# oscka/rag-llm-k8s

Measured on AMD Instinct MI355X. Metric: end-to-end RAG query p50 latency + gen tokens/sec, Llama-3.1-8B top-k=4, higher is better.
Workload: dtype bf16; 1 GPU; model=Llama-3.1-8B-Instruct, embedder=all-MiniLM-L6-v2, index=FlatL2 10000 vectors (HBM-resident; 10000 embedded chunks), retrieve_k=4, context_k=4, global_batch=32, seq_len=5192, parallelism=dp1

## Files before the change

csrc/kernels/gemm_w4.hip:

```cpp
#include <stdlib.h>

#include <utility>

#include "common.h"
using namespace ragk;

namespace {

constexpr int WBM = 256, WBN = 256, WBK = 64;
constexpr int W4_THREADS = 256;
constexpr int W_TILE_A = WBM * WBK * 2;
constexpr int W_TILE_B = WBN * WBK * 2;
constexpr int W_BUF = W_TILE_A + W_TILE_B;
constexpr int W4_LDS = 2 * W_BUF;
constexpr int WGROUP_M = 8;
constexpr int W4_MIN_KT = 3;

__device__ __forceinline__ int wswz(int row, int chunk) { return chunk ^ ((row >> 1) & 7); }

template <typename F, int... Ms>
__device__ __forceinline__ void static_for_impl(F&& f, std::integer_sequence<int, Ms...>) {
  (f(std::integral_constant<int, Ms>{}), ...);
}
template <int N, typename F>
__device__ __forceinline__ void static_for(F&& f) {
  static_for_impl(f, std::make_integer_sequence<int, N>{});
}

__device__ __forceinline__ int w4_perm(int q) {
  const int j = q >> 4, fh = (q >> 2) & 3, k = q & 3;
  return 32 * (j >> 1) + 8 * fh + 4 * (j & 1) + k;
}

template <bool PERM>
__device__ __forceinline__ void w4_offsets(int ld, int row0, int rows_valid, int wid, int lane, int (&off)[8]) {
#pragma unroll
  for (int i = 0; i < 8; ++i) {
    const int r = (wid * 8 + i) * 8 + (lane >> 3);
    const int c = wswz(r, lane & 7);
    int gr = row0 + (PERM ? (r & ~127) + w4_perm(r & 127) : r);
    gr = gr < rows_valid ? gr : rows_valid - 1;
    off[i] = gr * ld * 2 + c * 16;
  }
}

__device__ __forceinline__ void w4_stage(i32x4 srd, const int (&off)[8], int k0, char* lds, int wid) {
#pragma unroll
  for (int i = 0; i < 8; ++i) blds16(srd, off[i], k0 * 2, lds + (wid * 8 + i) * 1024);
}

__device__ __forceinline__ void w4_barrier() {
  __builtin_amdgcn_sched_barrier(0);
  __builtin_amdgcn_s_barrier();
  __builtin_amdgcn_sched_barrier(0);
}

__device__ __forceinline__ void w4_read(const char* buf, int s, int wr, int wc, int fr, int fh, bf16x8 (&a)[8],
                                        bf16x8 (&b)[8]) {
  const char* sa = buf;
  const char* sb = buf + W_TILE_A;
  const int c = 4 * s + fh;
#pragma unroll
  for (int i = 0; i < 8; ++i) {
    const int R = wr * 128 + 16 * i + fr;
    a[i] = *reinterpret_cast<const bf16x8*>(sa + R * 128 + 16 * wswz(R, c));
  }
#pragma unroll
  for (int j = 0; j < 8; ++j) {
    const int R = wc * 128 + 16 * j + fr;
    b[j] = *reinterpret_cast<const bf16x8*>(sb + R * 128 + 16 * wswz(R, c));
  }
}

__device__ __forceinline__ void w4_mfma(f32x4 (&acc)[8][8], const bf16x8 (&a)[8], const bf16x8 (&b)[8], int m) {
  asm volatile("v_mfma_f32_16x16x32_bf16 %0, %2, %1, %0"
               : "+a"(acc[m >> 3][m & 7])
               : "v"(a[m >> 3]), "v"(b[m & 7])
               : "memory");
}
__device__ __forceinline__ void w4_mfma0(f32x4 (&acc)[8][8], const bf16x8 (&a)[8], const bf16x8 (&b)[8], int m) {
  asm volatile("v_mfma_f32_16x16x32_bf16 %0, %2, %1, 0"
               : "=a"(acc[m >> 3][m & 7])
               : "v"(a[m >> 3]), "v"(b[m & 7])
               : "memory");
}

__device__ __forceinline__ void w4_pin_acc(f32x4 (&acc)[8][8]) {
  asm volatile("s_nop 7\n\ts_nop 7\n\ts_nop 1" ::: "memory");
#pragma unroll
  for (int i = 0; i < 8; ++i)
#pragma unroll
    for (int j = 0; j < 8; ++j) asm volatile("" : "+a"(acc[i][j])::"memory");
}

constexpr bool epi_res(int e) { return e == EPI_RESID || e == EPI_BIAS_RESID; }
constexpr bool epi_bias(int e) {
  return e == EPI_BIAS || e == EPI_BIAS_RESID || e == EPI_BIAS_GELU || e == EPI_BIAS_GELU_TANH;
}

template <int EPI, bool OUT_F32>
constexpr int w4_epi_vmem() {
  if constexpr (EPI == EPI_ROPE_KV) return 63;
  if constexpr (EPI == EPI_SILU_MUL) return 16;
  if constexpr (OUT_F32) return 64 + (epi_res(EPI) ? 64 : 0) + (epi_bias(EPI) ? 8 : 0);
  return 32 + (epi_res(EPI) ? 32 : 0) + (epi_bias(EPI) ? 4 : 0);
}

template <int EPI>
__device__ __forceinline__ float w4_act(float v) {
  if constexpr (EPI == EPI_BIAS_GELU || EPI == EPI_GELU) return gelu_erf(v);
  if constexpr (EPI == EPI_BIAS_GELU_TANH) return gelu_tanh(v);
  return v;
}

__device__ __forceinline__ void unpack4(uint2 v, float (&f)[4]) {
  f[0] = __uint_as_float(v.x << 16);
  f[1] = __uint_as_float(v.x & 0xffff0000u);
  f[2] = __uint_as_float(v.y << 16);
  f[3] = __uint_as_float(v.y & 0xffff0000u);
}

template <int EPI>
__device__ __forceinline__ void w4_epilogue_full_bf16(const f32x4 (&acc)[8][8], int wr, int wc, int fr, int fh,
                                                      int m0, int n0, void* C, int ldc,
                                                      const bf16_t* __restrict__ bias, const bf16_t* resid, int ldr) {
  const int row0 = m0 + wr * 128 + fr;
  bf16_t* Cb = reinterpret_cast<bf16_t*>(C);
  if constexpr (EPI == EPI_SILU_MUL) {
    const int colw = (n0 >> 1) + wc * 64 + 8 * fh;
#pragma unroll
    for (int i = 0; i < 8; ++i) {
#pragma unroll
      for (int p = 0; p < 2; ++p) {
        float o[8];
#pragma unroll
        for (int k = 0; k < 4; ++k) {
          o[k] = silu(acc[i][2 * p][k]) * acc[i][2 * p + 4][k];
          o[4 + k] = silu(acc[i][2 * p + 1][k]) * acc[i][2 * p + 5][k];
        }
        *reinterpret_cast<u32x4*>(Cb + (size_t)(row0 + 16 * i) * ldc + colw + 32 * p) = pack8(o);
        __builtin_amdgcn_sched_barrier(0);
      }
    }
  } else {
    constexpr bool RES = epi_res(EPI), BIAS = epi_bias(EPI);
    const int colw = n0 + wc * 128 + 8 * fh;
    u32x4 bv[BIAS ? 4 : 1];
    if constexpr (BIAS) {
#pragma unroll
      for (int p = 0; p < 4; ++p) bv[p] = *reinterpret_cast<const u32x4*>(bias + colw + 32 * p);
    }
    u32x4 rv[RES ? 32 : 1];
    if constexpr (RES) {
#pragma unroll
      for (int i = 0; i < 8; ++i)
#pragma unroll
        for (int p = 0; p < 4; ++p)
          rv[4 * i + p] = *reinterpret_cast<const u32x4*>(resid + (size_t)(row0 + 16 * i) * ldr + colw + 32 * p);
    }
#pragma unroll
    for (int i = 0; i < 8; ++i) {
#pragma unroll
      for (int p = 0; p < 4; ++p) {
        float o[8];
#pragma unroll
        for (int k = 0; k < 4; ++k) {
          o[k] = acc[i][2 * p][k];
          o[4 + k] = acc[i][2 * p + 1][k];
        }
        if constexpr (BIAS) {
          float b[8];
          unpack8(bv[p], b);
#pragma unroll
          for (int k = 0; k < 8; ++k) o[k] += b[k];
        }
        if constexpr (RES) {
          float r[8];
          unpack8(rv[4 * i + p], r);
#pragma unroll
          for (int k = 0; k < 8; ++k) o[k] += r[k];
        }
#pragma unroll
        for (int k = 0; k < 8; ++k) o[k] = w4_act<EPI>(o[k]);
        *reinterpret_cast<u32x4*>(Cb + (size_t)(row0 + 16 * i) * ldc + colw + 32 * p) = pack8(o);
      }
    }
  }
}

struct RopeKV {
  const int* pos;
  const int* slot;
  const float* cos_t;
  const float* sin_t;
  bf16_t* kc;
  bf16_t* vc;
  int Hq, Hkv, BS;
};

template <bool FULL>
__device__ __forceinline__ void w4_epilogue_rope(const f32x4 (&acc)[8][8], int wr, int wc, int fr, int fh, int m0,
                                                 int n0, bf16_t* C, int ldc, const RopeKV& rk, int M) {
  const int row0 = m0 + wr * 128 + fr;
  const int hd = (n0 + wc * 128) >> 7;
  const int d0 = 8 * fh;
  const bool isq = hd < rk.Hq, isk = !isq && hd < rk.Hq + rk.Hkv, rot = hd < rk.Hq + rk.Hkv;
  const int kvh = isk ? hd - rk.Hq : hd - rk.Hq - rk.Hkv;
  bf16_t* cache = isk ? rk.kc : rk.vc;
  int pos[8], slot[8];
#pragma unroll
  for (int i = 0; i < 8; ++i) {
    const int r = FULL ? row0 + 16 * i : min(row0 + 16 * i, M - 1);
    pos[i] = rk.pos[r];
    slot[i] = rk.slot[r];
  }
#pragma unroll
  for (int i2 = 0; i2 < 8; i2 += 2) {
    u32x4 cv[2][2][2], sv[2][2][2];
#pragma unroll
    for (int u = 0; u < 2; ++u)
#pragma unroll
      for (int p = 0; p < 2; ++p) {
        const float* ct = rk.cos_t + (size_t)pos[i2 + u] * 64 + d0 + 32 * p;
        const float* st = rk.sin_t + (size_t)pos[i2 + u] * 64 + d0 + 32 * p;
        cv[u][p][0] = *reinterpret_cast<const u32x4*>(ct);
        cv[u][p][1] = *reinterpret_cast<const u32x4*>(ct + 4);
        sv[u][p][0] = *reinterpret_cast<const u32x4*>(st);
        sv[u][p][1] = *reinterpret_cast<const u32x4*>(st + 4);
      }
#pragma unroll
    for (int u = 0; u < 2; ++u) {
      const int i = i2 + u;
      const int gr = row0 + 16 * i;
      float o[4][8];
#pragma unroll
      for (int p = 0; p < 4; ++p)
#pragma unroll
        for (int k = 0; k < 4; ++k) {
          o[p][k] = bf2f(f2bf(acc[i][2 * p][k]));
          o[p][4 + k] = bf2f(f2bf(acc[i][2 * p + 1][k]));
        }
      if (rot) {
#pragma unroll
        for (int p = 0; p < 2; ++p)
#pragma unroll
          for (int k = 0; k < 8; ++k) {
            const float c = __uint_as_float(cv[u][p][k >> 2][k & 3]), sn = __uint_as_float(sv[u][p][k >> 2][k & 3]);
            const float x1 = o[p][k], x2 = o[p + 2][k];
            o[p][k] = bf2f(f2bf(bf2f(f2bf(x1 * c)) + bf2f(f2bf(-x2 * sn))));
            o[p + 2][k] = bf2f(f2bf(bf2f(f2bf(x2 * c)) + bf2f(f2bf(x1 * sn))));
          }
      }
      if (FULL || gr < M) {
        bf16_t* crow = C + (size_t)gr * ldc + n0 + wc * 128 + d0;
#pragma unroll
        for (int p = 0; p < 4; ++p) *reinterpret_cast<u32x4*>(crow + 32 * p) = pack8(o[p]);
        const int sl = slot[i];
        if (!isq && sl >= 0) {
          bf16_t* dst = cache + (((size_t)(sl / rk.BS) * rk.Hkv + kvh) * rk.BS + (sl % rk.BS)) * 128 + d0;
#pragma unroll
          for (int p = 0; p < 4; ++p) *reinterpret_cast<u32x4*>(dst + 32 * p) = pack8(o[p]);
        }
      }
    }
  }
}

template <int EPI, bool OUT_F32, bool FULL>
__device__ __forceinline__ void w4_epilogue_reg(const f32x4 (&acc)[8][8], int wr, int wc, int fr, int fh, int m0,
                                                int n0, void* C, int ldc, const bf16_t* __restrict__ bias,
                                                const bf16_t* resid, int ldr, int M, int Nout) {
  const int row0 = m0 + wr * 128 + fr;
  if constexpr (EPI == EPI_SILU_MUL) {
    const int colw = (n0 >> 1) + wc * 64;
#pragma unroll
    for (int i = 0; i < 8; ++i) {
      const int gr = row0 + 16 * i;
#pragma unroll
      for (int j = 0; j < 4; ++j) {
        const int gc = colw + w4_perm(16 * j + 4 * fh);
        if (FULL || (gr < M && gc < Nout)) {
          float o[4];
#pragma unroll
          for (int k = 0; k < 4; ++k) o[k] = silu(acc[i][j][k]) * acc[i][j + 4][k];
          *reinterpret_cast<uint2*>(reinterpret_cast<bf16_t*>(C) + (size_t)gr * ldc + gc) =
              make_uint2(pk2bf(o[0], o[1]), pk2bf(o[2], o[3]));
        }
      }
    }
  } else {
    constexpr bool RES = epi_res(EPI), BIAS = epi_bias(EPI);
    const int colw = n0 + wc * 128;
    uint2 bv[BIAS ? 8 : 1];
    if constexpr (BIAS) {
#pragma unroll
      for (int j = 0; j < 8; ++j) {
        const int gc = colw + w4_perm(16 * j + 4 * fh);
        bv[j] = *reinterpret_cast<const uint2*>(bias + (FULL ? gc : min(gc, Nout - 4)));
      }
    }
    constexpr int RD = BIAS ? 1 : 8;
    uint2 rv[RES ? 8 * RD : 1];
#pragma unroll
    for (int i = 0; i < 8; ++i) {
      const int gr = row0 + 16 * i;
      if constexpr (RES) {
        if (i % RD == 0) {
#pragma unroll
          for (int g = 0; g < RD; ++g)
#pragma unroll
            for (int j = 0; j < 8; ++j) {
              const int grc = FULL ? gr + 16 * g : min(gr + 16 * g, M - 1);
              const int gc = colw + w4_perm(16 * j + 4 * fh);
              rv[8 * g + j] = *reinterpret_cast<const uint2*>(resid + (size_t)grc * ldr + (FULL ? gc : min(gc, Nout - 4)));
            }
        }
      }
#pragma unroll
      for (int j = 0; j < 8; ++j) {
        const int gc = colw + w4_perm(16 * j + 4 * fh);
        if (FULL || (gr < M && gc < Nout)) {
          float o[4];
#pragma unroll
          for (int k = 0; k < 4; ++k) o[k] = acc[i][j][k];
          if constexpr (BIAS) {
            float b[4];
            unpack4(bv[j], b);
#pragma unroll
            for (int k = 0; k < 4; ++k) o[k] += b[k];
          }
          if constexpr (RES) {
            float r[4];
            unpack4(rv[8 * (i % RD) + j], r);
#pragma unroll
            for (int k = 0; k < 4; ++k) o[k] += r[k];
          }
#pragma unroll
          for (int k = 0; k < 4; ++k) o[k] = w4_act<EPI>(o[k]);
          if constexpr (OUT_F32) {
            *reinterpret_cast<f32x4*>(reinterpret_cast<float*>(C) + (size_t)gr * ldc + gc) =
                (f32x4){o[0], o[1], o[2], o[3]};
          } else {
            *reinterpret_cast<uint2*>(reinterpret_cast<bf16_t*>(C) + (size_t)gr * ldc + gc) =
                make_uint2(pk2bf(o[0], o[1]), pk2bf(o[2], o[3]));
          }
        }
      }
    }
  }
}

__device__ __forceinline__ void h_read(bf16x8& d, unsigned addr, int off_imm) {
  asm volatile("ds_read_b128 %0, %1 offset:%2" : "=v"(d) : "v"(addr), "i"(off_imm) : "memory");
}
__device__ __forceinline__ void h_dma(i32x4 srd, int voff, int soff) {
  asm volatile("buffer_load_dwordx4 %0, %1, %2 offen lds" ::"v"(voff), "s"(srd), "s"(soff) : "memory");
}
__device__ __forceinline__ void h_m0_set(unsigned lds) { asm volatile("s_mov_b32 m0, %0" ::"s"(lds) : "memory"); }
__device__ __forceinline__ void h_m0_inc() { asm volatile("s_add_u32 m0, m0, 0x400" ::: "memory"); }

constexpr int H_DX[8] = {22, 25, 28, 31, 34, 52, 55, 58};
constexpr int H_DY[8] = {61, 64, 85, 87, 89, 96, 99, 125};
constexpr int H_RB1[8] = {0, 2, 4, 6, 8, 10, 12, 14};
constexpr int H_RA1[8] = {24, 27, 30, 33, 36, 38, 40, 42};
constexpr int H_RB0[8] = {93, 94, 95, 97, 98, 100, 101, 102};
constexpr int H_RA0[8] = {104, 107, 110, 113, 116, 119, 121, 123};
constexpr int H_VM = 13;

constexpr int h_find(const int (&s)[8], int m) {
  for (int q = 0; q < 8; ++q)
    if (s[q] == m) return q;
  return -1;
}

template <bool ZERO, int VMW, bool F0 = true>
__device__ __forceinline__ void w4_iter_h(char* smem, int g, i32x4 srd_a, i32x4 srd_b, const int (&sa)[8],
                                          const int (&sb)[8], int kst, int wid, const unsigned (&rbA)[2],
                                          const unsigned (&rbB)[2], f32x4 (&acc)[8][8], bf16x8 (&a0)[8],
                                          bf16x8 (&b0)[8], bf16x8 (&a1)[8], bf16x8 (&b1)[8]) {
  static_assert(VMW >= H_VM && VMW <= 63, "vmcnt bound");
  const unsigned cur = (unsigned)(g & 1) * W_BUF, nxt = (unsigned)((g + 1) & 1) * W_BUF;
  const unsigned lds_cur = (unsigned)(unsigned long long)(const __attribute__((address_space(3))) char*)smem + cur;
  const unsigned mX = __builtin_amdgcn_readfirstlane(lds_cur + W_TILE_A + wid * 8192);
  const unsigned mY = __builtin_amdgcn_readfirstlane(lds_cur + wid * 8192);
  const int kb = kst * WBK * 2;
  const unsigned rb1 = rbB[1] + cur, ra1 = rbA[1] + cur, rb0 = rbB[0] + nxt, ra0 = rbA[0] + nxt;
  static_for<128>([&](auto mc) __attribute__((always_inline)) {
    constexpr int m = decltype(mc)::value;
    if constexpr (m == 0) asm volatile("s_waitcnt lgkmcnt(7)" ::: "memory");
    if constexpr (m == 8) asm volatile("s_waitcnt lgkmcnt(10)" ::: "memory");
    if constexpr (m == 16) asm volatile("s_waitcnt lgkmcnt(13)" ::: "memory");
    if constexpr (m == 21 || m == 51) asm volatile("s_waitcnt lgkmcnt(0)" ::: "memory");
    if constexpr (m == 22 || m == 52) w4_barrier();
    if constexpr (m == 92) asm volatile("s_waitcnt vmcnt(%0)" ::"i"(VMW) : "memory");
    if constexpr (m == 93) w4_barrier();
    if constexpr (m < 64) {
      if constexpr (ZERO) w4_mfma0(acc, a0, b0, m);
      else w4_mfma(acc, a0, b0, m);
    } else {
      w4_mfma(acc, a1, b1, m - 64);
    }
    if constexpr (h_find(H_DX, m - 1) >= 0 || h_find(H_DY, m - 1) >= 0) h_m0_inc();
    if constexpr (m == 21) h_m0_set(mX);
    if constexpr (m == 59) h_m0_set(mY);
    constexpr int qx = h_find(H_DX, m), qy = h_find(H_DY, m);
    if constexpr (qx >= 0) h_dma(srd_b, sb[qx], kb);
    if constexpr (qy >= 0) h_dma(srd_a, sa[qy], kb);
    constexpr int r1b = h_find(H_RB1, m), r1a = h_find(H_RA1, m), r0b = h_find(H_RB0, m), r0a = h_find(H_RA0, m);
    if constexpr (r1b >= 0) h_read(b1[r1b], rb1, r1b * 2048);
    if constexpr (r1a >= 0) h_read(a1[r1a], ra1, r1a * 2048);
    if constexpr (F0 && r0b >= 0) h_read(b0[r0b], rb0, r0b * 2048);
    if constexpr (F0 && r0a >= 0) h_read(a0[r0a], ra0, r0a * 2048);
  });
}

__device__ __forceinline__ void w4_read_f0(int g, const unsigned (&rbA)[2], const unsigned (&rbB)[2],
                                           bf16x8 (&a0)[8], bf16x8 (&b0)[8]) {
  const unsigned buf = (unsigned)(g & 1) * W_BUF;
  const unsigned rb0 = rbB[0] + buf, ra0 = rbA[0] + buf;
  static_for<8>([&](auto jc) __attribute__((always_inline)) {
    constexpr int j = decltype(jc)::value;
    h_read(b0[j], rb0, j * 2048);
  });
  static_for<8>([&](auto ic) __attribute__((always_inline)) {
    constexpr int i = decltype(ic)::value;
    h_read(a0[i], ra0, i * 2048);
  });
}

template <bool MT = false>
__device__ __forceinline__ void w4_origin(int tile, int nwg, int tiles_m, int tiles_n, int& m0, int& n0,
                                          const int* __restrict__ mt = nullptr, int mt_max = 0) {
  const int logical = xcd_remap(tile, nwg);
  const int group = logical / (WGROUP_M * tiles_n);
  const int first_m = group * WGROUP_M;
  const int gm = min(tiles_m - first_m, WGROUP_M);
  const int in_group = logical % (WGROUP_M * tiles_n);
  int mi = first_m + in_group % gm;
  if constexpr (MT) mi = (int)min((unsigned)mt[__builtin_amdgcn_readfirstlane(mi)], (unsigned)mt_max);
  m0 = mi * WBM;
  n0 = (in_group / gm) * WBN;
}

template <int EPI, bool OUT_F32, bool KSPLIT = false, bool MT = false>
__global__ __launch_bounds__(W4_THREADS, 1) void gemm_w4_kernel(const bf16_t* __restrict__ A, int lda,
                                                                const bf16_t* __restrict__ B, int ldb, void* C,
                                                                int ldc, const bf16_t* __restrict__ bias,
                                                                const bf16_t* resid, int ldr, int M, int N, int K,
                                                                int nsplit, RopeKV rk,
                                                                const int* __restrict__ m_tiles, int n_m_tiles) {
  __shared__ __attribute__((aligned(16))) char smem[W4_LDS];
  const int tid = threadIdx.x, lane = tid & 63;
  const int wid = __builtin_amdgcn_readfirstlane(tid >> 6);
  const int wr = wid >> 1, wc = wid & 1;
  const int fr = lane & 15, fh = lane >> 4;
  const int tiles_m = MT ? n_m_tiles : (M + WBM - 1) / WBM, tiles_n = (N + WBN - 1) / WBN;
  const int mt_max = (M + WBM - 1) / WBM - 1;
  const int nwg = tiles_m * tiles_n;
  const int nwt = KSPLIT ? nwg * nsplit : nwg;
  const int nk = K / WBK;
  const int Nout = EPI == EPI_SILU_MUL ? N / 2 : N;
  const i32x4 srd_a = make_srd(A, (unsigned)M * (unsigned)lda * 2u);
  const i32x4 srd_b = make_srd(B, (unsigned)N * (unsigned)ldb * 2u);

  constexpr int EV = w4_epi_vmem<EPI, OUT_F32>();
  constexpr int VMH0 = H_VM + EV > 63 ? 63 : H_VM + EV;
  constexpr bool LATE_F0 = !(EPI == EPI_NONE || EPI == EPI_SILU_MUL || (EPI == EPI_RESID && !OUT_F32));
  static_assert(EPI != EPI_ROPE_KV || (!OUT_F32 && !KSPLIT), "rope epilogue: bf16 output, no split-K");
  static_assert(!MT || EPI == EPI_NONE || ((EPI == EPI_RESID || EPI == EPI_SILU_MUL) && !OUT_F32 && !KSPLIT),
                "M-tile list: none / residual / SiLU*up epilogues and the split-K slabs");

  int tile = blockIdx.x;
  int z = KSPLIT ? tile / nwg : 0;
  int m0, n0;
  w4_origin<MT>(tile - z * nwg, nwg, tiles_m, tiles_n, m0, n0, m_tiles, mt_max);
  int off_a[8], off_b[8];
  w4_offsets<false>(lda, m0, M, wid, lane, off_a);
  w4_offsets<true>(ldb, n0, N, wid, lane, off_b);
  if constexpr (KSPLIT) {
#pragma unroll
    for (int i = 0; i < 8; ++i) {
      off_a[i] += z * K * 2;
      off_b[i] += z * K * 2;
    }
  }
  w4_stage(srd_a, off_a, 0, smem, wid);
  w4_stage(srd_b, off_b, 0, smem + W_TILE_A, wid);
  w4_stage(srd_a, off_a, WBK, smem + W_BUF, wid);
  w4_stage(srd_b, off_b, WBK, smem + W_BUF + W_TILE_A, wid);
  __builtin_amdgcn_s_waitcnt(0x0F70);
  w4_barrier();
  bf16x8 a0[8], b0[8], a1[8], b1[8];
  w4_read(smem, 0, wr, wc, fr, fh, a0, b0);
  __builtin_amdgcn_s_waitcnt(0xC07F);
  __builtin_amdgcn_sched_barrier(0);

  unsigned rbA[2], rbB[2];
  {
    const unsigned l0 = (unsigned)(unsigned long long)(const __attribute__((address_space(3))) char*)smem;
#pragma unroll
    for (int s = 0; s < 2; ++s) {
      const unsigned cs = (unsigned)(((4 * s + fh) ^ ((fr >> 1) & 7)) * 16);
      rbA[s] = l0 + (unsigned)((wr * 128 + fr) * 128) + cs;
      rbB[s] = l0 + W_TILE_A + (unsigned)((wc * 128 + fr) * 128) + cs;
    }
  }

  f32x4 acc[8][8];
  int g = 0;
  for (;;) {
    const int next = tile + (int)gridDim.x;
    const bool has_next = next < nwt;
    w4_iter_h<true, VMH0>(smem, g, srd_a, srd_b, off_a, off_b, 2, wid, rbA, rbB, acc, a0, b0, a1, b1);
    ++g;
    for (int t = 1; t + 2 < nk; ++t, ++g)
      w4_iter_h<false, H_VM>(smem, g, srd_a, srd_b, off_a, off_b, t + 2, wid, rbA, rbB, acc, a0, b0, a1, b1);
    int nm0, nn0;
    const int ntile = has_next ? next : tile;
    const int nz = KSPLIT ? ntile / nwg : 0;
    w4_origin<MT>(ntile - nz * nwg, nwg, tiles_m, tiles_n, nm0, nn0, m_tiles, mt_max);
    {
      int ln;
      asm volatile("v_mbcnt_lo_u32_b32 %0, -1, 0\n\tv_mbcnt_hi_u32_b32 %0, -1, %0" : "=v"(ln));
      w4_offsets<false>(lda, nm0, M, wid, ln, off_a);
      w4_offsets<true>(ldb, nn0, N, wid, ln, off_b);
      if constexpr (KSPLIT) {
#pragma unroll
        for (int i = 0; i < 8; ++i) {
          off_a[i] += nz * K * 2;
          off_b[i] += nz * K * 2;
        }
      }
    }
    w4_iter_h<false, H_VM>(smem, g, srd_a, srd_b, off_a, off_b, 0, wid, rbA, rbB, acc, a0, b0, a1, b1);
    ++g;
    w4_iter_h<false, H_VM, !LATE_F0>(smem, g, srd_a, srd_b, off_a, off_b, 1, wid, rbA, rbB, acc, a0, b0, a1, b1);
    ++g;
    asm volatile("s_waitcnt lgkmcnt(0)" ::: "memory");
    w4_pin_acc(acc);
    void* Cz = KSPLIT ? (void*)(reinterpret_cast<float*>(C) + (size_t)z * M * ldc) : C;
    if constexpr (EPI == EPI_ROPE_KV) {
      if (m0 + WBM <= M) {
        w4_epilogue_rope<true>(acc, wr, wc, fr, fh, m0, n0, reinterpret_cast<bf16_t*>(Cz), ldc, rk, M);
      } else {
        w4_epilogue_rope<false>(acc, wr, wc, fr, fh, m0, n0, reinterpret_cast<bf16_t*>(Cz), ldc, rk, M);
        __builtin_amdgcn_s_waitcnt(0x0F70);
      }
    } else if (m0 + WBM <= M && n0 + WBN <= N) {
      if constexpr (OUT_F32)
        w4_epilogue_reg<EPI, true, true>(acc, wr, wc, fr, fh, m0, n0, Cz, ldc, bias, resid, ldr, M, Nout);
      else
        w4_epilogue_full_bf16<EPI>(acc, wr, wc, fr, fh, m0, n0, Cz, ldc, bias, resid, ldr);
    } else {
      w4_epilogue_reg<EPI, OUT_F32, false>(acc, wr, wc, fr, fh, m0, n0, Cz, ldc, bias, resid, ldr, M, Nout);
      __builtin_amdgcn_s_waitcnt(0x0F70);
    }
    asm volatile("s_nop 7" ::: "memory");
    if (!has_next) {
      __builtin_amdgcn_s_waitcnt(0x0F70);
      asm volatile("s_waitcnt lgkmcnt(0)" ::: "memory");
      break;
    }
    if constexpr (LATE_F0) w4_read_f0(g, rbA, rbB, a0, b0);
    tile = next;
    m0 = nm0;
    n0 = nn0;
    z = nz;
  }
}

static int g_w4_grid = -1;
static int w4_grid(int nwg) {
  if (g_w4_grid < 0) {
    int cus = 0, dev = 0;
    if (hipGetDevice(&dev) != hipSuccess ||
        hipDeviceGetAttribute(&cus, hipDeviceAttributeMultiprocessorCount, dev) != hipSuccess)
      cus = 256;
    g_w4_grid = (cus / 8) * 8;
  }
  return (g_w4_grid == 0 || g_w4_grid >= nwg) ? nwg : g_w4_grid;
}

constexpr bool w4_mt_epi(int e) { return e == EPI_NONE || e == EPI_RESID || e == EPI_SILU_MUL; }

template <int EPI, bool F32>
int launch_w4(const void* A, int lda, const void* B, int ldb, void* C, int ldc, const void* bias, const void* resid,
              int ldr, int M, int N, int K, const int* m_tiles, int n_m_tiles, hipStream_t st) {
  const int tiles_n = (N + WBN - 1) / WBN;
  if (m_tiles) {
    if constexpr (w4_mt_epi(EPI) && !F32) {
      hipLaunchKernelGGL((gemm_w4_kernel<EPI, F32, false, true>), dim3(w4_grid(n_m_tiles * tiles_n)),
                         dim3(W4_THREADS), 0, st, (const bf16_t*)A, lda, (const bf16_t*)B, ldb, C, ldc,
                         (const bf16_t*)bias, (const bf16_t*)resid, ldr, M, N, K, 1, RopeKV{}, m_tiles, n_m_tiles);
      return (int)hipGetLastError();
    } else {
      return (int)hipErrorInvalidValue;
    }
  }
  const int nwg = ((M + WBM - 1) / WBM) * tiles_n;
  hipLaunchKernelGGL((gemm_w4_kernel<EPI, F32>), dim3(w4_grid(nwg)), dim3(W4_THREADS), 0, st, (const bf16_t*)A, lda,
                     (const bf16_t*)B, ldb, C, ldc, (const bf16_t*)bias, (const bf16_t*)resid, ldr, M, N, K, 1,
                     RopeKV{}, nullptr, 0);
  return (int)hipGetLastError();
}

static bool w4_mt_ok(const int* m_tiles, int n_m_tiles, int M) {
  return !m_tiles || (n_m_tiles >= 1 && n_m_tiles <= (M + WBM - 1) / WBM);
}

}

RAGK_API int ragk_gemm_w4_set_grid(int g) {
  g_w4_grid = g < 0 ? -1 : g;
  return 0;
}

RAGK_API int ragk_gemm_w4(const void* A, int lda, const void* B, int ldb, void* C, int ldc, const void* bias,
                          const void* resid, int ldr, int M, int N, int K, int epi, int out_f32, const int* m_tiles,
                          int n_m_tiles, hipStream_t st) {
  if (M <= 0 || N <= 0 || K <= 0 || (m_tiles && n_m_tiles == 0)) return 0;
  if (!w4_mt_ok(m_tiles, n_m_tiles, M)) return (int)hipErrorInvalidValue;
  if (K % WBK != 0 || K / WBK < W4_MIN_KT) return (int)hipErrorInvalidValue;
  const long long rows_b = (epi == EPI_SILU_MUL) ? 2LL * N : (long long)N;
  if ((long long)M * lda * 2 >= (1LL << 31) || rows_b * ldb * 2 >= (1LL << 31))
    return (int)hipErrorInvalidValue;
  if (epi == EPI_SILU_MUL) {
    if (N % 128 != 0 || out_f32) return (int)hipErrorInvalidValue;
    return launch_w4<EPI_SILU_MUL, false>(A, lda, B, ldb, C, ldc, bias, resid, ldr, M, 2 * N, K, m_tiles, n_m_tiles,
                                          st);
  }
  if (N % 8 != 0) return (int)hipErrorInvalidValue;
#define RAGK_W4_CASE(E) \
  case E:               \
    return out_f32 ? launch_w4<E, true>(A, lda, B, ldb, C, ldc, bias, resid, ldr, M, N, K, m_tiles, n_m_tiles, st) \
                   : launch_w4<E, false>(A, lda, B, ldb, C, ldc, bias, resid, ldr, M, N, K, m_tiles, n_m_tiles, st);
  switch (epi) {
    RAGK_W4_CASE(EPI_NONE)
    RAGK_W4_CASE(EPI_BIAS)
    RAGK_W4_CASE(EPI_RESID)
    RAGK_W4_CASE(EPI_BIAS_RESID)
    RAGK_W4_CASE(EPI_BIAS_GELU)
    RAGK_W4_CASE(EPI_GELU)
    RAGK_W4_CASE(EPI_BIAS_GELU_TANH)
    default:
      return (int)hipErrorInvalidValue;
  }
#undef RAGK_W4_CASE
}

RAGK_API int ragk_gemm_w4_splitk(const void* A, int lda, const void* B, int ldb, float* P, int M, int N, int K,
                                 int nsplit, const int* m_tiles, int n_m_tiles, hipStream_t st) {
  if (M <= 0 || N <= 0 || K <= 0 || (m_tiles && n_m_tiles == 0)) return 0;
  if (!w4_mt_ok(m_tiles, n_m_tiles, M)) return (int)hipErrorInvalidValue;
  if (nsplit < 1 || K % nsplit || (K / nsplit) % WBK || (K / nsplit) / WBK < W4_MIN_KT || N % 8 || !P)
    return (int)hipErrorInvalidValue;
  if ((long long)M * lda * 2 >= (1LL << 31) || (long long)N * ldb * 2 >= (1LL << 31)) return (int)hipErrorInvalidValue;
  if (m_tiles) {
    const int nwt = n_m_tiles * ((N + WBN - 1) / WBN) * nsplit;
    hipLaunchKernelGGL((gemm_w4_kernel<EPI_NONE, true, true, true>), dim3(w4_grid(nwt)), dim3(W4_THREADS), 0, st,
                       (const bf16_t*)A, lda, (const bf16_t*)B, ldb, (void*)P, N, nullptr, nullptr, 0, M, N,
                       K / nsplit, nsplit, RopeKV{}, m_tiles, n_m_tiles);
    return (int)hipGetLastError();
  }
  const int nwg = ((M + WBM - 1) / WBM) * ((N + WBN - 1) / WBN);
  hipLaunchKernelGGL((gemm_w4_kernel<EPI_NONE, true, true>), dim3(w4_grid(nwg * nsplit)), dim3(W4_THREADS), 0, st,
                     (const bf16_t*)A, lda, (const bf16_t*)B, ldb, (void*)P, N, nullptr, nullptr, 0, M, N, K / nsplit,
                     nsplit, RopeKV{}, nullptr, 0);
  return (int)hipGetLastError();
}

RAGK_API int ragk_gemm_w4_rope_kv(const void* A, int lda, const void* B, int ldb, void* C, int ldc, int M, int K,
                                  const int* pos, const int* slot, const float* cos_t, const float* sin_t, void* kc,
                                  void* vc, int Hq, int Hkv, int BS, hipStream_t st) {
  if (M <= 0) return 0;
  const int N = (Hq + 2 * Hkv) * 128;
  if (K % WBK != 0 || K / WBK < W4_MIN_KT || Hq < 1 || Hkv < 1 || BS < 1 || N % WBN != 0) return (int)hipErrorInvalidValue;
  if (!pos || !slot || !cos_t || !sin_t || !kc || !vc || ldc % 8 != 0) return (int)hipErrorInvalidValue;
  if ((long long)M * lda * 2 >= (1LL << 31) || (long long)N * ldb * 2 >= (1LL << 31)) return (int)hipErrorInvalidValue;
  const int nwg = ((M + WBM - 1) / WBM) * (N / WBN);
  const RopeKV rk{pos, slot, cos_t, sin_t, (bf16_t*)kc, (bf16_t*)vc, Hq, Hkv, BS};
  hipLaunchKernelGGL((gemm_w4_kernel<EPI_ROPE_KV, false>), dim3(w4_grid(nwg)), dim3(W4_THREADS), 0, st,
                     (const bf16_t*)A, lda, (const bf16_t*)B, ldb, C, ldc, nullptr, nullptr, 0, M, N, K, 1, rk, nullptr, 0);
  return (int)hipGetLastError();
}
```

csrc/kernels/norm.hip:

```cpp
#include <algorithm>

#include "common.h"
#include "kv_fp8.h"
using namespace ragk;

namespace {

constexpr int NT = 256;

__global__ __launch_bounds__(NT) void rmsnorm_kernel(const bf16_t* x, int ldx, bf16_t* resid, int ldr,
                                                     const bf16_t* __restrict__ w, bf16_t* out, int ldo,
                                                     int H, float eps) {
  __shared__ float red[NT / 64];
  const int row = blockIdx.x;
  const bf16_t* xr = x + (size_t)row * ldx;
  bf16_t* rr = resid ? resid + (size_t)row * ldr : nullptr;
  bf16_t* orow = out + (size_t)row * ldo;
  constexpr int MAXV = 4;
  float v[MAXV][8];
  const int nvec = H >> 3;
  float ss = 0.f;
#pragma unroll
  for (int i = 0; i < MAXV; ++i) {
    const int vi = threadIdx.x + i * NT;
    if (vi < nvec) {
      unpack8(*reinterpret_cast<const u32x4*>(xr + vi * 8), v[i]);
      if (rr) {
        float r8[8];
        unpack8(*reinterpret_cast<const u32x4*>(rr + vi * 8), r8);
#pragma unroll
        for (int e = 0; e < 8; ++e) v[i][e] = bf2f(f2bf(v[i][e] + r8[e]));
        *reinterpret_cast<u32x4*>(rr + vi * 8) = pack8(v[i]);
      }
#pragma unroll
      for (int e = 0; e < 8; ++e) ss += v[i][e] * v[i][e];
    }
  }
  ss = block_sum(ss, red);
  const float inv = rsqrtf(ss / (float)H + eps);
#pragma unroll
  for (int i = 0; i < MAXV; ++i) {
    const int vi = threadIdx.x + i * NT;
    if (vi < nvec) {
      float wv[8], o[8];
      unpack8(*reinterpret_cast<const u32x4*>(w + vi * 8), wv);
#pragma unroll
      for (int e = 0; e < 8; ++e) o[e] = wv[e] * bf2f(f2bf(v[i][e] * inv));
      *reinterpret_cast<u32x4*>(orow + vi * 8) = pack8(o);
    }
  }
}

__global__ __launch_bounds__(NT) void layernorm_kernel(const bf16_t* x, int ldx, const bf16_t* resid, int ldr,
                                                       const bf16_t* __restrict__ g, const bf16_t* __restrict__ b,
                                                       bf16_t* out, int ldo, int H, float eps) {
  __shared__ float red[NT / 64];
  const int row = blockIdx.x;
  const bf16_t* xr = x + (size_t)row * ldx;
  constexpr int MAXV = 4;
  float v[MAXV][8];
  const int nvec = H >> 3;
  float s = 0.f;
#pragma unroll
  for (int i = 0; i < MAXV; ++i) {
    const int vi = threadIdx.x + i * NT;
    if (vi < nvec) {
      unpack8(*reinterpret_cast<const u32x4*>(xr + vi * 8), v[i]);
      if (resid) {
        float r8[8];
        unpack8(*reinterpret_cast<const u32x4*>(resid + (size_t)row * ldr + vi * 8), r8);
#pragma unroll
        for (int e = 0; e < 8; ++e) v[i][e] += r8[e];
      }
#pragma unroll
      for (int e = 0; e < 8; ++e) s += v[i][e];
    }
  }
  const float mean = block_sum(s, red) / (float)H;
  float sq = 0.f;
#pragma unroll
  for (int i = 0; i < MAXV; ++i) {
    const int vi = threadIdx.x + i * NT;
    if (vi < nvec)
#pragma unroll
      for (int e = 0; e < 8; ++e) {
        const float d = v[i][e] - mean;
        sq += d * d;
      }
  }
  const float inv = rsqrtf(block_sum(sq, red) / (float)H + eps);
#pragma unroll
  for (int i = 0; i < MAXV; ++i) {
    const int vi = threadIdx.x + i * NT;
    if (vi < nvec) {
      float gv[8], bv[8], o[8];
      unpack8(*reinterpret_cast<const u32x4*>(g + vi * 8), gv);
      unpack8(*reinterpret_cast<const u32x4*>(b + vi * 8), bv);
#pragma unroll
      for (int e = 0; e < 8; ++e) o[e] = (v[i][e] - mean) * inv * gv[e] + bv[e];
      *reinterpret_cast<u32x4*>(out + (size_t)row * ldo + vi * 8) = pack8(o);
    }
  }
}

__global__ __launch_bounds__(NT) void embed_kernel(int* __restrict__ ids, const bf16_t* __restrict__ table,
                                                   bf16_t* out, int H, int vocab, const int* __restrict__ carry,
                                                   const int* __restrict__ prev) {
  const int t = blockIdx.x;
  int id = ids[t];
  if (carry != nullptr) {
    const int c = carry[t];
    if (c >= 0) {
      id = prev[c];
      __syncthreads();
      if (threadIdx.x == 0) ids[t] = id;
    }
  }
  id = id < 0 ? 0 : (id >= vocab ? vocab - 1 : id);
  const u32x4* src = reinterpret_cast<const u32x4*>(table + (size_t)id * H);
  u32x4* dst = reinterpret_cast<u32x4*>(out + (size_t)t * H);
  for (int i = threadIdx.x; i < (H >> 3); i += NT) dst[i] = src[i];
}

__global__ __launch_bounds__(NT) void embed_ln_kernel(const int* __restrict__ ids, const int* __restrict__ pos_ids,
                                                      const bf16_t* __restrict__ word, const bf16_t* __restrict__ pos,
                                                      const bf16_t* __restrict__ type, const bf16_t* __restrict__ g,
                                                      const bf16_t* __restrict__ b, bf16_t* out, int H, float eps,
                                                      int do_ln) {
  __shared__ float red[NT / 64];
  const int t = blockIdx.x;
  const bf16_t* wr = word + (size_t)ids[t] * H;
  const bf16_t* pr = pos + (size_t)pos_ids[t] * H;
  constexpr int MAXV = 4;
  float v[MAXV][8];
  const int nvec = H >> 3;
  float s = 0.f;
#pragma unroll
  for (int i = 0; i < MAXV; ++i) {
    const int vi = threadIdx.x + i * NT;
    if (vi < nvec) {
      float a[8], p[8];
      unpack8(*reinterpret_cast<const u32x4*>(wr + vi * 8), a);
      unpack8(*reinterpret_cast<const u32x4*>(pr + vi * 8), p);
#pragma unroll
      for (int e = 0; e < 8; ++e) v[i][e] = a[e] + p[e];
      if (type) {
        float ty[8];
        unpack8(*reinterpret_cast<const u32x4*>(type + vi * 8), ty);
#pragma unroll
        for (int e = 0; e < 8; ++e) v[i][e] += ty[e];
      }
#pragma unroll
      for (int e = 0; e < 8; ++e) s += v[i][e];
    }
  }
  if (!do_ln) {
#pragma unroll
    for (int i = 0; i < MAXV; ++i) {
      const int vi = threadIdx.x + i * NT;
      if (vi < nvec) *reinterpret_cast<u32x4*>(out + (size_t)t * H + vi * 8) = pack8(v[i]);
    }
    return;
  }
  const float mean = block_sum(s, red) / (float)H;
  float sq = 0.f;
#pragma unroll
  for (int i = 0; i < MAXV; ++i) {
    const int vi = threadIdx.x + i * NT;
    if (vi < nvec)
#pragma unroll
      for (int e = 0; e < 8; ++e) {
        const float d = v[i][e] - mean;
        sq += d * d;
      }
  }
  const float inv = rsqrtf(block_sum(sq, red) / (float)H + eps);
#pragma unroll
  for (int i = 0; i < MAXV; ++i) {
    const int vi = threadIdx.x + i * NT;
    if (vi < nvec) {
      float gv[8], bv[8], o[8];
      unpack8(*reinterpret_cast<const u32x4*>(g + vi * 8), gv);
      unpack8(*reinterpret_cast<const u32x4*>(b + vi * 8), bv);
#pragma unroll
      for (int e = 0; e < 8; ++e) o[e] = (v[i][e] - mean) * inv * gv[e] + bv[e];
      *reinterpret_cast<u32x4*>(out + (size_t)t * H + vi * 8) = pack8(o);
    }
  }
}

__global__ __launch_bounds__(NT) void rope_kv_kernel(bf16_t* qkv, int ld, const int* __restrict__ positions,
                                                     const float* __restrict__ cos_t, const float* __restrict__ sin_t,
                                                     const int* __restrict__ slots, bf16_t* kc, bf16_t* vc, int Hq,
                                                     int Hkv, int D, int BS, int apply_rope) {
  const int t = blockIdx.x;
  const int pos = positions[t];
  const int slot = slots ? slots[t] : -1;
  bf16_t* row = qkv + (size_t)t * ld;
  const int half = D >> 1;
  const int vpr = half >> 3;
  const float* ct = cos_t + (size_t)pos * half;
  const float* st = sin_t + (size_t)pos * half;
  const int nrot = (Hq + Hkv) * vpr;
  for (int i = threadIdx.x; i < nrot; i += NT) {
    const int h = i / vpr, v = i % vpr;
    bf16_t* hp = row + h * D;
    float x1[8], x2[8], o1[8], o2[8];
    unpack8(*reinterpret_cast<const u32x4*>(hp + v * 8), x1);
    unpack8(*reinterpret_cast<const u32x4*>(hp + half + v * 8), x2);
    if (apply_rope) {
#pragma unroll
      for (int e = 0; e < 8; ++e) {
        const float c = ct[v * 8 + e], s = st[v * 8 + e];
        o1[e] = bf2f(f2bf(bf2f(f2bf(x1[e] * c)) + bf2f(f2bf(-x2[e] * s))));
        o2[e] = bf2f(f2bf(bf2f(f2bf(x2[e] * c)) + bf2f(f2bf(x1[e] * s))));
      }
    } else {
#pragma unroll
      for (int e = 0; e < 8; ++e) { o1[e] = x1[e]; o2[e] = x2[e]; }
    }
    const u32x4 p1 = pack8(o1), p2 = pack8(o2);
    if (h < Hq) {
      *reinterpret_cast<u32x4*>(hp + v * 8) = p1;
      *reinterpret_cast<u32x4*>(hp + half + v * 8) = p2;
    } else if (slot >= 0) {
      const int kh = h - Hq;
      bf16_t* dst = kc + (((size_t)(slot / BS) * Hkv + kh) * BS + (slot % BS)) * D;
      *reinterpret_cast<u32x4*>(dst + v * 8) = p1;
      *reinterpret_cast<u32x4*>(dst + half + v * 8) = p2;
      *reinterpret_cast<u32x4*>(hp + v * 8) = p1;
      *reinterpret_cast<u32x4*>(hp + half + v * 8) = p2;
    } else {
      *reinterpret_cast<u32x4*>(hp + v * 8) = p1;
      *reinterpret_cast<u32x4*>(hp + half + v * 8) = p2;
    }
  }
  if (slot >= 0) {
    const int vpd = D >> 3;
    for (int i = threadIdx.x; i < Hkv * vpd; i += NT) {
      const int kh = i / vpd, v = i % vpd;
      const bf16_t* src = row + (Hq + Hkv + kh) * D + v * 8;
      bf16_t* dst = vc + (((size_t)(slot / BS) * Hkv + kh) * BS + (slot % BS)) * D + v * 8;
      *reinterpret_cast<u32x4*>(dst) = *reinterpret_cast<const u32x4*>(src);
    }
  }
}

__global__ __launch_bounds__(NT) void pool_l2norm_kernel(const bf16_t* __restrict__ hidden, int ld,
                                                         const int* __restrict__ cu, float* out, int H, int mode,
                                                         int normalize) {
  __shared__ float red[NT / 64];
  const int b = blockIdx.x;
  const int s0 = cu[b], s1 = cu[b + 1];
  const int len = s1 - s0;
  float ss = 0.f;
  constexpr int MAXC = 8;
  float acc[MAXC];
#pragma unroll
  for (int k = 0; k < MAXC; ++k) acc[k] = 0.f;
  if (mode == 1) {
    for (int t = s0; t < s1; ++t)
#pragma unroll
      for (int k = 0; k < MAXC; ++k) {
        const int c = threadIdx.x + k * NT;
        if (c < H) acc[k] += bf2f(hidden[(size_t)t * ld + c]);
      }
    const float inv = len > 0 ? 1.f / (float)len : 0.f;
#pragma unroll
    for (int k = 0; k < MAXC; ++k) acc[k] *= inv;
  } else {
    const int t = mode == 0 ? s0 : s1 - 1;
#pragma unroll
    for (int k = 0; k < MAXC; ++k) {
      const int c = threadIdx.x + k * NT;
      if (c < H) acc[k] = bf2f(hidden[(size_t)t * ld + c]);
    }
  }
#pragma unroll
  for (int k = 0; k < MAXC; ++k) ss += acc[k] * acc[k];
  float scale = 1.f;
  if (normalize) {
    ss = block_sum(ss, red);
    scale = 1.f / fmaxf(sqrtf(ss), 1e-12f);
  }
#pragma unroll
  for (int k = 0; k < MAXC; ++k) {
    const int c = threadIdx.x + k * NT;
    if (c < H) out[(size_t)b * H + c] = acc[k] * scale;
  }
}

__global__ __launch_bounds__(NT) void silu_mul_kernel(const bf16_t* x, int ldx, bf16_t* out, int ldo, int I) {
  const int t = blockIdx.x;
  for (int v = threadIdx.x; v < (I >> 3); v += NT) {
    float g[8], u[8], o[8];
    unpack8(*reinterpret_cast<const u32x4*>(x + (size_t)t * ldx + v * 8), g);
    unpack8(*reinterpret_cast<const u32x4*>(x + (size_t)t * ldx + I + v * 8), u);
#pragma unroll
    for (int e = 0; e < 8; ++e) o[e] = silu(g[e]) * u[e];
    *reinterpret_cast<u32x4*>(out + (size_t)t * ldo + v * 8) = pack8(o);
  }
}

__global__ __launch_bounds__(NT) void gather_rows_kernel(const bf16_t* x, int ldx, const int* __restrict__ idx,
                                                         bf16_t* out, int ldo, int H) {
  const int i = blockIdx.x;
  const bf16_t* src = x + (size_t)idx[i] * ldx;
  for (int v = threadIdx.x; v < (H >> 3); v += NT)
    *reinterpret_cast<u32x4*>(out + (size_t)i * ldo + v * 8) = *reinterpret_cast<const u32x4*>(src + v * 8);
}



constexpr int PNT = 512;
__global__ __launch_bounds__(PNT) void add_partials_rmsnorm_kernel(const float* __restrict__ P, int S, int M,
                                                                   bf16_t* h, int ldh,
                                                                   const bf16_t* __restrict__ w, bf16_t* out,
                                                                   int ldo, int H, float eps) {
  __shared__ float red[PNT / 64];
  const int row = blockIdx.x;
  bf16_t* hr = h + (size_t)row * ldh;
  constexpr int MAXV = 2;
  float v[MAXV][8];
  const int nvec = H >> 3;
  float ss = 0.f;
  f32x4 pv[MAXV][PSU][2];
  u32x4 hv[MAXV], gv[MAXV];
#pragma unroll
  for (int i = 0; i < MAXV; ++i) {
    const int vi = min((int)threadIdx.x + i * PNT, nvec - 1);
    if (i * PNT < nvec) {
      load_slabs8(P + (size_t)row * H + vi * 8, S, (size_t)M * H, pv[i]);
      hv[i] = *reinterpret_cast<const u32x4*>(hr + vi * 8);
      gv[i] = *reinterpret_cast<const u32x4*>(w + vi * 8);
    }
  }
#pragma unroll
  for (int i = 0; i < MAXV; ++i) {
    const int vi = threadIdx.x + i * PNT;
    if (vi < nvec) {
      float a[8];
      add_slabs8(pv[i], P + (size_t)row * H + vi * 8, S, (size_t)M * H, a);
      unpack8(hv[i], v[i]);
#pragma unroll
      for (int e = 0; e < 8; ++e) v[i][e] = bf2f(f2bf(v[i][e] + bf2f(f2bf(a[e]))));
      *reinterpret_cast<u32x4*>(hr + vi * 8) = pack8(v[i]);
#pragma unroll
      for (int e = 0; e < 8; ++e) ss += v[i][e] * v[i][e];
    }
  }
  ss = block_sum(ss, red);
  const float inv = rsqrtf(ss / (float)H + eps);
#pragma unroll
  for (int i = 0; i < MAXV; ++i) {
    const int vi = threadIdx.x + i * PNT;
    if (vi < nvec) {
      float wv[8], o[8];
      unpack8(gv[i], wv);
#pragma unroll
      for (int e = 0; e < 8; ++e) o[e] = wv[e] * bf2f(f2bf(v[i][e] * inv));
      *reinterpret_cast<u32x4*>(out + (size_t)row * ldo + vi * 8) = pack8(o);
    }
  }
}


__global__ __launch_bounds__(NT) void rope_kv_partials_kernel(const float* __restrict__ P, int S, int T, int ldp,
                                                              bf16_t* q_out, int ldq,
                                                              const int* __restrict__ positions,
                                                              const float* __restrict__ cos_t,
                                                              const float* __restrict__ sin_t,
                                                              const int* __restrict__ slots, bf16_t* kc, bf16_t* vc,
                                                              int Hq, int Hkv, int D, int BS) {
  const int t = blockIdx.x, hg = blockIdx.y, ngroups = gridDim.y;
  const int pos = positions[t];
  const int slot = slots ? slots[t] : -1;
  const size_t slab = (size_t)T * ldp;
  const float* prow = P + (size_t)t * ldp;
  const int half = D >> 1;
  const int vpr = half >> 3;
  const float* ct = cos_t + (size_t)pos * half;
  const float* st = sin_t + (size_t)pos * half;
  const int nh = Hq + 2 * Hkv;
  for (int i = threadIdx.x + hg * NT; i < nh * vpr; i += NT * ngroups) {
    const int hd = i / vpr, v = i % vpr;
    float x1[8], x2[8];
    sum_partials8(prow + hd * D + v * 8, S, slab, x1);
    sum_partials8(prow + hd * D + half + v * 8, S, slab, x2);
    if (hd >= Hq + Hkv) {
      if (slot >= 0) {
        bf16_t* dst = vc + (((size_t)(slot / BS) * Hkv + (hd - Hq - Hkv)) * BS + (slot % BS)) * D;
        *reinterpret_cast<u32x4*>(dst + v * 8) = pack8(x1);
        *reinterpret_cast<u32x4*>(dst + half + v * 8) = pack8(x2);
      }
      continue;
    }
    float o1[8], o2[8];
    rope8(x1, x2, ct + v * 8, st + v * 8, o1, o2);
    if (hd < Hq) {
      bf16_t* qp = q_out + (size_t)t * ldq + hd * D;
      *reinterpret_cast<u32x4*>(qp + v * 8) = pack8(o1);
      *reinterpret_cast<u32x4*>(qp + half + v * 8) = pack8(o2);
    } else if (slot >= 0) {
      bf16_t* dst = kc + (((size_t)(slot / BS) * Hkv + (hd - Hq)) * BS + (slot % BS)) * D;
      *reinterpret_cast<u32x4*>(dst + v * 8) = pack8(o1);
      *reinterpret_cast<u32x4*>(dst + half + v * 8) = pack8(o2);
    }
  }
}

__device__ __forceinline__ size_t kv8_row(int slot, int kh, int Hkv, int BS) {
  return ((size_t)(slot / BS) * Hkv + kh) * BS + (slot % BS);
}

__global__ __launch_bounds__(NT) void rope_kv_fp8_kernel(bf16_t* qkv, int ld, const int* __restrict__ positions,
                                                         const float* __restrict__ cos_t,
                                                         const float* __restrict__ sin_t,
                                                         const int* __restrict__ slots, unsigned char* k8,
                                                         unsigned char* v8, float* ks, float* vs, int Hq, int Hkv,
                                                         int BS) {
  constexpr int D = 128, half = 64, vpr = 8;
  const int t = blockIdx.x;
  const int pos = positions[t];
  const int slot = slots ? slots[t] : -1;
  bf16_t* row = qkv + (size_t)t * ld;
  const float* ct = cos_t + (size_t)pos * half;
  const float* st = sin_t + (size_t)pos * half;
  const int nh = Hq + 2 * Hkv;
  for (int i = threadIdx.x; i < nh * vpr; i += NT) {
    const int h = i / vpr, v = i % vpr;
    bf16_t* hp = row + h * D;
    float x1[8], x2[8], o1[8], o2[8];
    unpack8(*reinterpret_cast<const u32x4*>(hp + v * 8), x1);
    unpack8(*reinterpret_cast<const u32x4*>(hp + half + v * 8), x2);
    if (h >= Hq + Hkv) {
      if (slot >= 0) {
        const size_t r = kv8_row(slot, h - Hq - Hkv, Hkv, BS);
        kv8_store_row128(x1, x2, v, v8 + r * D, vs + r);
      }
      continue;
    }
    rope8(x1, x2, ct + v * 8, st + v * 8, o1, o2);
    *reinterpret_cast<u32x4*>(hp + v * 8) = pack8(o1);
    *reinterpret_cast<u32x4*>(hp + half + v * 8) = pack8(o2);
    if (h >= Hq && slot >= 0) {
      const size_t r = kv8_row(slot, h - Hq, Hkv, BS);
      kv8_store_row128(o1, o2, v, k8 + r * D, ks + r);
    }
  }
}

__global__ __launch_bounds__(NT) void rope_kv_partials_fp8_kernel(const float* __restrict__ P, int S, int T, int ldp,
                                                                  bf16_t* q_out, int ldq,
                                                                  const int* __restrict__ positions,
                                                                  const float* __restrict__ cos_t,
                                                                  const float* __restrict__ sin_t,
                                                                  const int* __restrict__ slots, unsigned char* k8,
                                                                  unsigned char* v8, float* ks, float* vs, int Hq,
                                                                  int Hkv, int BS) {
  constexpr int D = 128, half = 64, vpr = 8;
  const int t = blockIdx.x, hg = blockIdx.y, ngroups = gridDim.y;
  const int pos = positions[t];
  const int slot = slots[t];
  const size_t slab = (size_t)T * ldp;
  const float* prow = P + (size_t)t * ldp;
  const float* ct = cos_t + (size_t)pos * half;
  const float* st = sin_t + (size_t)pos * half;
  const int nh = Hq + 2 * Hkv;
  for (int i = threadIdx.x + hg * NT; i < nh * vpr; i += NT * ngroups) {
    const int hd = i / vpr, v = i % vpr;
    float x1[8], x2[8];
    sum_partials8(prow + hd * D + v * 8, S, slab, x1);
    sum_partials8(prow + hd * D + half + v * 8, S, slab, x2);
    if (hd >= Hq + Hkv) {
      if (slot >= 0) {
        const size_t r = kv8_row(slot, hd - Hq - Hkv, Hkv, BS);
        kv8_store_row128(x1, x2, v, v8 + r * D, vs + r);
      }
      continue;
    }
    float o1[8], o2[8];
    rope8(x1, x2, ct + v * 8, st + v * 8, o1, o2);
    if (hd < Hq) {
      bf16_t* qp = q_out + (size_t)t * ldq + hd * D;
      *reinterpret_cast<u32x4*>(qp + v * 8) = pack8(o1);
      *reinterpret_cast<u32x4*>(qp + half + v * 8) = pack8(o2);
    } else if (slot >= 0) {
      const size_t r = kv8_row(slot, hd - Hq, Hkv, BS);
      kv8_store_row128(o1, o2, v, k8 + r * D, ks + r);
    }
  }
}

}

RAGK_API int ragk_rmsnorm(const void* x, int ldx, void* resid, int ldr, const void* w, void* out, int ldo, int rows,
                          int H, float eps, hipStream_t st) {
  if (rows <= 0) return 0;
  if (H % 8 || H > 8 * NT * 4) return (int)hipErrorInvalidValue;
  hipLaunchKernelGGL(rmsnorm_kernel, dim3(rows), dim3(NT), 0, st, (const bf16_t*)x, ldx, (bf16_t*)resid, ldr,
                     (const bf16_t*)w, (bf16_t*)out, ldo, H, eps);
  return (int)hipGetLastError();
}

RAGK_API int ragk_layernorm(const void* x, int ldx, const void* resid, int ldr, const void* g, const void* b,
                            void* out, int ldo, int rows, int H, float eps, hipStream_t st) {
  if (rows <= 0) return 0;
  if (H % 8 || H > 8 * NT * 4) return (int)hipErrorInvalidValue;
  hipLaunchKernelGGL(layernorm_kernel, dim3(rows), dim3(NT), 0, st, (const bf16_t*)x, ldx, (const bf16_t*)resid,
                     ldr, (const bf16_t*)g, (const bf16_t*)b, (bf16_t*)out, ldo, H, eps);
  return (int)hipGetLastError();
}

RAGK_API int ragk_embed(const int* ids, const void* table, void* out, int T, int H, int vocab, hipStream_t st) {
  if (T <= 0) return 0;
  if (H % 8) return (int)hipErrorInvalidValue;
  hipLaunchKernelGGL(embed_kernel, dim3(T), dim3(NT), 0, st, const_cast<int*>(ids), (const bf16_t*)table,
                     (bf16_t*)out, H, vocab, (const int*)nullptr, (const int*)nullptr);
  return (int)hipGetLastError();
}

RAGK_API int ragk_embed_carry(int* ids, const int* carry, const int* prev, const void* table, void* out, int T,
                              int H, int vocab, hipStream_t st) {
  if (T <= 0) return 0;
  if (H % 8 || !carry || !prev) return (int)hipErrorInvalidValue;
  hipLaunchKernelGGL(embed_kernel, dim3(T), dim3(NT), 0, st, ids, (const bf16_t*)table, (bf16_t*)out, H, vocab,
                     carry, prev);
  return (int)hipGetLastError();
}

RAGK_API int ragk_embed_ln(const int* ids, const int* pos_ids, const void* word, const void* pos, const void* type,
                           const void* g, const void* b, void* out, int T, int H, float eps, int do_ln,
                           hipStream_t st) {
  if (T <= 0) return 0;
  if (H % 8 || H > 8 * NT * 4) return (int)hipErrorInvalidValue;
  hipLaunchKernelGGL(embed_ln_kernel, dim3(T), dim3(NT), 0, st, ids, pos_ids, (const bf16_t*)word,
                     (const bf16_t*)pos, (const bf16_t*)type, (const bf16_t*)g, (const bf16_t*)b, (bf16_t*)out, H,
                     eps, do_ln);
  return (int)hipGetLastError();
}

RAGK_API int ragk_rope_kv(void* qkv, int ld, const int* positions, const float* cos_t, const float* sin_t,
                          const int* slots, void* kc, void* vc, int T, int Hq, int Hkv, int D, int BS,
                          int apply_rope, hipStream_t st) {
  if (T <= 0) return 0;
  if (D % 16) return (int)hipErrorInvalidValue;
  hipLaunchKernelGGL(rope_kv_kernel, dim3(T), dim3(NT), 0, st, (bf16_t*)qkv, ld, positions, cos_t, sin_t, slots,
                     (bf16_t*)kc, (bf16_t*)vc, Hq, Hkv, D, BS, apply_rope);
  return (int)hipGetLastError();
}

RAGK_API int ragk_pool_l2norm(const void* hidden, int ld, const int* cu, float* out, int B, int H, int mode,
                              int normalize, hipStream_t st) {
  if (B <= 0) return 0;
  if (H > 8 * NT) return (int)hipErrorInvalidValue;
  hipLaunchKernelGGL(pool_l2norm_kernel, dim3(B), dim3(NT), 0, st, (const bf16_t*)hidden, ld, cu, out, H, mode,
                     normalize);
  return (int)hipGetLastError();
}

RAGK_API int ragk_silu_mul(const void* x, int ldx, void* out, int ldo, int T, int I, hipStream_t st) {
  if (T <= 0) return 0;
  if (I % 8) return (int)hipErrorInvalidValue;
  hipLaunchKernelGGL(silu_mul_kernel, dim3(T), dim3(NT), 0, st, (const bf16_t*)x, ldx, (bf16_t*)out, ldo, I);
  return (int)hipGetLastError();
}

RAGK_API int ragk_gather_rows(const void* x, int ldx, const int* idx, void* out, int ldo, int n, int H,
                              hipStream_t st) {
  if (n <= 0) return 0;
  if (H % 8) return (int)hipErrorInvalidValue;
  hipLaunchKernelGGL(gather_rows_kernel, dim3(n), dim3(NT), 0, st, (const bf16_t*)x, ldx, idx, (bf16_t*)out, ldo, H);
  return (int)hipGetLastError();
}

RAGK_API int ragk_add_partials_rmsnorm(const float* P, int S, int M, void* h, int ldh, const void* w, void* out,
                                       int ldo, int H, float eps, hipStream_t st) {
  if (M <= 0) return 0;
  if (H % 8 || H > 8 * PNT * 2 || S < 1) return (int)hipErrorInvalidValue;
  hipLaunchKernelGGL(add_partials_rmsnorm_kernel, dim3(M), dim3(PNT), 0, st, P, S, M, (bf16_t*)h, ldh,
                     (const bf16_t*)w, (bf16_t*)out, ldo, H, eps);
  return (int)hipGetLastError();
}

RAGK_API int ragk_rope_kv_partials(const float* P, int S, int T, int ldp, void* q_out, int ldq,
                                   const int* positions, const float* cos_t, const float* sin_t, const int* slots,
                                   void* kc, void* vc, int Hq, int Hkv, int D, int BS, hipStream_t st) {
  if (T <= 0) return 0;
  if (D % 16 || S < 1) return (int)hipErrorInvalidValue;
  const int items = (Hq + 2 * Hkv) * (D / 16);
  const int groups = std::max(1, std::min((items + 63) / 64, std::max(4, (512 + T - 1) / T)));
  hipLaunchKernelGGL(rope_kv_partials_kernel, dim3(T, groups), dim3(NT), 0, st, P, S, T, ldp, (bf16_t*)q_out,
                     ldq, positions, cos_t, sin_t, slots, (bf16_t*)kc, (bf16_t*)vc, Hq, Hkv, D, BS);
  return (int)hipGetLastError();
}

RAGK_API int ragk_rope_kv_fp8(void* qkv, int ld, const int* positions, const float* cos_t, const float* sin_t,
                              const int* slots, void* k8, void* v8, float* ks, float* vs, int T, int Hq, int Hkv,
                              int D, int BS, hipStream_t st) {
  if (T <= 0) return 0;
  if (D != 128 || !positions || !cos_t || !sin_t || (slots && (!k8 || !v8 || !ks || !vs)))
    return (int)hipErrorInvalidValue;
  hipLaunchKernelGGL(rope_kv_fp8_kernel, dim3(T), dim3(NT), 0, st, (bf16_t*)qkv, ld, positions, cos_t, sin_t, slots,
                     (unsigned char*)k8, (unsigned char*)v8, ks, vs, Hq, Hkv, BS);
  return (int)hipGetLastError();
}

RAGK_API int ragk_rope_kv_partials_fp8(const float* P, int S, int T, int ldp, void* q_out, int ldq,
                                       const int* positions, const float* cos_t, const float* sin_t,
                                       const int* slots, void* k8, void* v8, float* ks, float* vs, int Hq, int Hkv,
                                       int D, int BS, hipStream_t st) {
  if (T <= 0) return 0;
  if (D != 128 || S < 1 || !positions || !cos_t || !sin_t || !slots || !k8 || !v8 || !ks || !vs)
    return (int)hipErrorInvalidValue;
  const int items = (Hq + 2 * Hkv) * (D / 16);
  const int groups = std::max(1, std::min((items + 63) / 64, std::max(4, (512 + T - 1) / T)));
  hipLaunchKernelGGL(rope_kv_partials_fp8_kernel, dim3(T, groups), dim3(NT), 0, st, P, S, T, ldp, (bf16_t*)q_out,
                     ldq, positions, cos_t, sin_t, slots, (unsigned char*)k8, (unsigned char*)v8, ks, vs, Hq, Hkv,
                     BS);
  return (int)hipGetLastError();
}
```

rag_llm_k8s_amd/models/llama.py:

```python
from __future__ import annotations

import json
import math
import os
from dataclasses import dataclass, field
from typing import List, Optional

import torch

from ..ops.backend import AttnMeta, get_backend
from ..ops.fp8 import FP8, alloc_fp8_kv, check_fp8_kv_head_dim, kv_cache_torch_dtype
from ..ops.reference import pack_gate_up, rope_tables

DECODE_DOWN_SKINNY_MAX_M = 4
DECODE_OPROJ_MERGE_MAX_M = 2


@dataclass
class LlamaConfig:
    vocab_size: int = 128256
    hidden_size: int = 4096
    intermediate_size: int = 14336
    num_hidden_layers: int = 32
    num_attention_heads: int = 32
    num_key_value_heads: int = 8
    head_dim: int = 128
    rms_norm_eps: float = 1e-5
    rope_theta: float = 500000.0
    rope_scaling: Optional[dict] = field(default_factory=lambda: {
        "rope_type": "llama3", "factor": 8.0, "low_freq_factor": 1.0, "high_freq_factor": 4.0,
        "original_max_position_embeddings": 8192})
    max_position_embeddings: int = 131072
    tie_word_embeddings: bool = False
    bos_token_id: int = 128000
    eos_token_id: List[int] = field(default_factory=lambda: [128001, 128008, 128009])
    model_type: str = "llama"

    @classmethod
    def from_dict(cls, d):
        c = cls()
        for k in ("vocab_size", "hidden_size", "intermediate_size", "num_hidden_layers", "num_attention_heads",
                  "rms_norm_eps", "rope_theta", "max_position_embeddings", "tie_word_embeddings", "bos_token_id",
                  "model_type"):
            if k in d and d[k] is not None:
                setattr(c, k, d[k])
        c.num_key_value_heads = d.get("num_key_value_heads") or c.num_attention_heads
        c.head_dim = d.get("head_dim") or c.hidden_size // c.num_attention_heads
        c.rope_scaling = d.get("rope_scaling")
        eos = d.get("eos_token_id")
        if eos is not None:
            c.eos_token_id = eos if isinstance(eos, list) else [eos]
        return c

    @classmethod
    def from_json(cls, path):
        with open(path) as f:
            return cls.from_dict(json.load(f))

    def to_hf_dict(self):
        return {
            "architectures": ["LlamaForCausalLM"], "model_type": "llama", "vocab_size": self.vocab_size,
            "hidden_size": self.hidden_size, "intermediate_size": self.intermediate_size,
            "num_hidden_layers": self.num_hidden_layers, "num_attention_heads": self.num_attention_heads,
            "num_key_value_heads": self.num_key_value_heads, "head_dim": self.head_dim,
            "rms_norm_eps": self.rms_norm_eps, "rope_theta": self.rope_theta, "rope_scaling": self.rope_scaling,
            "max_position_embeddings": self.max_position_embeddings,
            "tie_word_embeddings": self.tie_word_embeddings, "bos_token_id": self.bos_token_id,
            "eos_token_id": self.eos_token_id, "hidden_act": "silu", "attention_bias": False, "mlp_bias": False,
            "torch_dtype": "bfloat16",
        }


def llama31_8b():
    return LlamaConfig()


def llama31_70b():
    return LlamaConfig(hidden_size=8192, intermediate_size=28672, num_hidden_layers=80, num_attention_heads=64,
                       num_key_value_heads=8)


def llama_tiny(vocab=512, layers=2, hidden=256, heads=4, kv_heads=2, inter=512):
    return LlamaConfig(vocab_size=vocab, hidden_size=hidden, intermediate_size=inter, num_hidden_layers=layers,
                       num_attention_heads=heads, num_key_value_heads=kv_heads, head_dim=hidden // heads,
                       max_position_embeddings=4096, bos_token_id=1, eos_token_id=[2])


class LlamaWeights:

    def __init__(self, cfg: LlamaConfig, tp_rank=0, tp_size=1):
        self.cfg, self.tp_rank, self.tp_size = cfg, tp_rank, tp_size
        self.layers = []
        self.embed = self.norm = self.lm_head = None

    def geom(self):
        c, tp = self.cfg, self.tp_size
        assert c.num_attention_heads % tp == 0 and c.num_key_value_heads % tp == 0, "heads % tp"
        assert c.intermediate_size % tp == 0 and (c.intermediate_size // tp) % 64 == 0, "intermediate % (64*tp)"
        return dict(Hq=c.num_attention_heads // tp, Hkv=c.num_key_value_heads // tp, D=c.head_dim,
                    I=c.intermediate_size // tp, V=-(-c.vocab_size // tp))

    @classmethod
    def from_hf(cls, cfg, get, device, tp_rank=0, tp_size=1, dtype=torch.bfloat16):
        w = cls(cfg, tp_rank, tp_size)
        g = w.geom()
        r = tp_rank
        D, Hq, Hkv, I, Vl = g["D"], g["Hq"], g["Hkv"], g["I"], g["V"]

        def dev(t):
            return t.to(device=device, dtype=dtype, non_blocking=False).contiguous()

        w.embed = dev(get("model.embed_tokens.weight"))
        for i in range(cfg.num_hidden_layers):
            p = "model.layers.%d." % i
            q = get(p + "self_attn.q_proj.weight", rows=(r * Hq * D, (r + 1) * Hq * D))
            k = get(p + "self_attn.k_proj.weight", rows=(r * Hkv * D, (r + 1) * Hkv * D))
            v = get(p + "self_attn.v_proj.weight", rows=(r * Hkv * D, (r + 1) * Hkv * D))
            o = get(p + "self_attn.o_proj.weight", cols=(r * Hq * D, (r + 1) * Hq * D))
            gt = get(p + "mlp.gate_proj.weight", rows=(r * I, (r + 1) * I))
            up = get(p + "mlp.up_proj.weight", rows=(r * I, (r + 1) * I))
            dn = get(p + "mlp.down_proj.weight", cols=(r * I, (r + 1) * I))
            w.layers.append(dict(
                ln_in=dev(get(p + "input_layernorm.weight")), ln_post=dev(get(p + "post_attention_layernorm.weight")),
                wqkv=dev(torch.cat([q, k, v], 0)), wo=dev(o), wgu=dev(pack_gate_up(gt, up)), wdown=dev(dn)))
        w.norm = dev(get("model.norm.weight"))
        V = cfg.vocab_size
        lo, hi = r * Vl, min(V, (r + 1) * Vl)
        name = "model.embed_tokens.weight" if cfg.tie_word_embeddings else "lm_head.weight"
        lm = get(name, rows=(lo, hi))
        if lm.shape[0] < Vl:
            lm = torch.cat([lm, torch.zeros(Vl - lm.shape[0], lm.shape[1], dtype=lm.dtype, device=lm.device)], 0)
        w.lm_head = dev(lm)
        w.vocab_offset = lo
        w.vocab_valid = hi - lo
        return w

    @classmethod
    def from_checkpoint(cls, path, cfg, device, tp_rank=0, tp_size=1):
        from ..runtime.safetensors_io import CheckpointReader

        rd = CheckpointReader(path)
        try:
            return cls.from_hf(cfg, rd.get, device, tp_rank, tp_size)
        finally:
            rd.close()

    @classmethod
    def from_state_dict(cls, cfg, sd, device, tp_rank=0, tp_size=1):
        def get(name, rows=None, cols=None):
            t = sd[name]
            if rows is not None:
                t = t[rows[0]:rows[1]]
            if cols is not None:
                t = t[:, cols[0]:cols[1]]
            return t

        return cls.from_hf(cfg, get, device, tp_rank, tp_size)

    @classmethod
    def random(cls, cfg, device, tp_rank=0, tp_size=1, seed=0, dtype=torch.bfloat16):
        w = cls(cfg, tp_rank, tp_size)
        g = w.geom()
        D, Hq, Hkv, I, Vl = g["D"], g["Hq"], g["Hkv"], g["I"], g["V"]
        H = cfg.hidden_size
        gen = torch.Generator(device=device).manual_seed(seed * 1000 + tp_rank)

        def rnd(*shape, std=0.02):
            return (torch.randn(*shape, device=device, generator=gen, dtype=torch.float32) * std).to(dtype)

        def ones(n):
            return (1.0 + 0.1 * torch.randn(n, device=device, generator=gen)).to(dtype)

        w.embed = rnd(cfg.vocab_size, H)
        for _ in range(cfg.num_hidden_layers):
            w.layers.append(dict(ln_in=ones(H), ln_post=ones(H), wqkv=rnd((Hq + 2 * Hkv) * D, H),
                                 wo=rnd(H, Hq * D), wgu=rnd(2 * I, H), wdown=rnd(H, I)))
        w.norm = ones(H)
        w.lm_head = rnd(Vl, H)
        w.vocab_offset = tp_rank * Vl
        w.vocab_valid = min(cfg.vocab_size - tp_rank * Vl, Vl)
        return w

    def quantize_fp8(self, lm_head=False):
        from ..ops.fp8 import quantize_weight

        for L in self.layers:
            for k in ("wqkv", "wo", "wgu", "wdown"):
                L[k] = quantize_weight(L[k])
        if lm_head:
            self.lm_head = quantize_weight(self.lm_head)
        self.dtype = "fp8"
        return self

    def quantize_mxfp4(self, lm_head=False):
        from ..ops.mxfp4 import quantize_weight

        for L in self.layers:
            for k in ("wqkv", "wo", "wgu", "wdown"):
                L[k] = quantize_weight(L[k])
        if lm_head:
            self.lm_head = quantize_weight(self.lm_head)
        self.dtype = "mxfp4"
        return self

    def nbytes(self):
        t = [self.embed, self.norm, self.lm_head] + [v for l in self.layers for v in l.values()]
        return sum(x.nbytes() if hasattr(x, "dequant") else x.numel() * x.element_size() for x in t)


@dataclass
class StepInput:
    ids: torch.Tensor
    positions: torch.Tensor
    slots: torch.Tensor
    meta: AttnMeta
    logits_idx: Optional[torch.Tensor] = None
    m_tiles: Optional[torch.Tensor] = None
    carry: Optional[torch.Tensor] = None
    carry_src: Optional[torch.Tensor] = None


class LlamaModel:
    def __init__(self, cfg: LlamaConfig, weights: LlamaWeights, device, comm=None, max_positions=None):
        self.cfg, self.w, self.device = cfg, weights, torch.device(device)
        self.be = get_backend(self.device)
        g = weights.geom()
        self.Hq, self.Hkv, self.D, self.I, self.Vl = g["Hq"], g["Hkv"], g["D"], g["I"], g["V"]
        self.comm = comm
        self.tp_rank = weights.tp_rank
        mp = max_positions or cfg.max_position_embeddings
        cos, sin = rope_tables(self.D, mp, cfg.rope_theta, cfg.rope_scaling)
        self.cos, self.sin = cos.to(self.device), sin.to(self.device)
        self.kv_cache = None
        self.seq_parallel = os.environ.get("RAGK_SEQ_PARALLEL", "0") == "1"
        self.sp_min_tokens = int(os.environ.get("RAGK_SP_MIN_TOKENS", "256"))

    def allocate_kv_cache(self, num_blocks, dtype=torch.bfloat16):
        dtype = kv_cache_torch_dtype(dtype)
        if dtype == FP8:
            check_fp8_kv_head_dim(self.D)
            self.kv_cache = [(alloc_fp8_kv(num_blocks, self.Hkv, 64, self.D, self.device),
                              alloc_fp8_kv(num_blocks, self.Hkv, 64, self.D, self.device))
                             for _ in range(self.cfg.num_hidden_layers)]
            return self.kv_cache
        self.kv_cache = [(torch.zeros(num_blocks, self.Hkv, 64, self.D, dtype=dtype, device=self.device),
                          torch.zeros(num_blocks, self.Hkv, 64, self.D, dtype=dtype, device=self.device))
                         for _ in range(self.cfg.num_hidden_layers)]
        return self.kv_cache

    def kv_bytes_per_block(self, dtype=torch.bfloat16):
        dtype = kv_cache_torch_dtype(dtype)
        if dtype == FP8:
            return 2 * self.cfg.num_hidden_layers * self.Hkv * 64 * (self.D + 4)
        return 2 * self.cfg.num_hidden_layers * self.Hkv * 64 * self.D * torch.tensor([], dtype=dtype).element_size()

    def _allreduce(self, x):
        if self.comm is not None:
            self.comm.all_reduce(x)

    def _attn_block(self, li, L, h, inp: StepInput, attn):
        be, c = self.be, self.cfg
        Hq, Hkv, D = self.Hq, self.Hkv, self.D
        kc, vc = self.kv_cache[li]
        xn = be.rmsnorm(h, L["ln_in"], c.rms_norm_eps)
        qkv = be.gemm_rope_kv(xn, L["wqkv"], inp.positions, self.cos, self.sin, inp.slots, kc, vc, Hq, Hkv, D)
        if inp.meta.kind == "decode":
            be.attn_decode(qkv, kc, vc, inp.meta, attn, Hq, Hkv, D)
        else:
            be.attn_prefill(qkv, kc, vc, inp.meta, attn, Hq, Hkv, D)
        if self.tp_rank == 0:
            be.gemm(attn, L["wo"], resid=h, epi="resid", out=h)
        else:
            be.gemm(attn, L["wo"], out=h)

    def _mlp_block(self, L, h):
        be, c = self.be, self.cfg
        xn = be.rmsnorm(h, L["ln_post"], c.rms_norm_eps)
        a = be.gemm(xn, L["wgu"], epi="silu_mul")
        if self.tp_rank == 0:
            be.gemm(a, L["wdown"], resid=h, epi="resid", out=h)
        else:
            be.gemm(a, L["wdown"], out=h)

    def _final(self, h, inp: StepInput):
        if inp.logits_idx is not None:
            h = self.be.gather_rows(h, inp.logits_idx)
            if h.shape[0] == 0:
                return h
        return self.be.rmsnorm(h, self.w.norm, self.cfg.rms_norm_eps)

    @staticmethod
    def prefill_last_rows_enabled():
        return os.environ.get("RAGK_PREFILL_LAST_ROWS", "1") != "0"

    def _last_rows(self, inp: StepInput, M):
        if (self.comm is not None or inp.meta is None or inp.meta.kind == "decode" or inp.logits_idx is None
                or not self.prefill_last_rows_enabled()):
            return None
        if inp.logits_idx.numel() == 0:
            return "skip"
        if inp.m_tiles is None or inp.meta.tiles_last is None:
            return None
        L, be = self.w.layers[-1], self.be
        if not (be.m_tiles_ok(M, L["wo"], "resid") and be.m_tiles_ok(M, L["wgu"], "silu_mul")
                and be.m_tiles_ok(M, L["wdown"], "resid")):
            return None
        return "tiles"

    def _tp(self):
        return self.comm is not None and self.comm.size > 1

    def _decode_part_ok(self, inp: StepInput, h):
        if inp.meta is None or inp.meta.kind != "decode" or inp.slots is None:
            return False
        L, M = self.w.layers[0], h.shape[0]
        if self._tp() and not self.comm.fused_decode_ok(M, h.shape[1]):
            return False
        return self.be.part_ok(M, L["wqkv"]) and self.be.part_ok(M, L["wo"]) and self.be.part_ok(M, L["wdown"])

    def hidden_states_decode_part(self, inp: StepInput, h):
        be, w, c = self.be, self.w, self.cfg
        Hq, Hkv, D = self.Hq, self.Hkv, self.D
        M = h.shape[0]
        tp = self._tp()

        def reduce_norm(P, gamma):
            if tp:
                return self.comm.add_partials_rmsnorm(P, h, gamma, c.rms_norm_eps, be)
            return be.add_partials_rmsnorm(P, h, gamma, c.rms_norm_eps)

        attn = torch.empty((M, Hq * D), dtype=h.dtype, device=h.device)
        layers = w.layers
        fuse_norm = M <= DECODE_DOWN_SKINNY_MAX_M and not tp and be.part_norm_ok(M, layers[0]["wqkv"])
        silu_fused = tp and be.part_silu_ok(M, layers[0]["wgu"], layers[0]["wdown"])
        xn = None if fuse_norm else be.rmsnorm(h, layers[0]["ln_in"], c.rms_norm_eps)
        merge = M <= DECODE_OPROJ_MERGE_MAX_M and be.part_merge_ok(M, inp.meta, layers[0]["wo"], Hq, D)
        mlp_eng = M == 1 and not tp and be.mlp_engine_ok(M, layers[0]["wgu"], layers[0]["wdown"])
        for li, L in enumerate(layers):
            kc, vc = self.kv_cache[li]
            P = be.gemm_part_norm(h, L["ln_in"], c.rms_norm_eps, L["wqkv"]) if fuse_norm else be.gemm_part(xn, L["wqkv"])
            be.attn_decode_rope(P, inp.positions, self.cos, self.sin, inp.slots, kc, vc, inp.meta, attn, Hq, Hkv, D,
                                defer_merge=merge)
            P = be.gemm_part_merge(attn, inp.meta, L["wo"], Hq) if merge else be.gemm_part(attn, L["wo"])
            nxt = layers[li + 1]["ln_in"] if li + 1 < len(layers) else w.norm
            if mlp_eng:
                be.mlp_engine_tail(P, h, L["ln_post"], c.rms_norm_eps, L["wgu"], L["wdown"])
                if not fuse_norm or li + 1 == len(layers):
                    xn = be.rmsnorm(h, nxt, c.rms_norm_eps)
                continue
            xn = reduce_norm(P, L["ln_post"])
            if silu_fused:
                P = be.gemm_part_silu(be.gemm_part_gu(xn, L["wgu"]), L["wdown"])
                xn = reduce_norm(P, nxt)
                continue
            a = be.gemm(xn, L["wgu"], epi="silu_mul")
            if M <= DECODE_DOWN_SKINNY_MAX_M and not tp:
                be.gemm(a, L["wdown"], resid=h, epi="resid", out=h)
                if not fuse_norm or li + 1 == len(layers):
                    xn = be.rmsnorm(h, nxt, c.rms_norm_eps)
                continue
            P = be.gemm_part(a, L["wdown"])
            xn = reduce_norm(P, nxt)
        if inp.logits_idx is not None:
            xn = be.gather_rows(xn, inp.logits_idx)
        return xn

    def hidden_states(self, inp: StepInput):
        be, w = self.be, self.w
        h = be.embed(inp.ids, w.embed, carry=inp.carry, prev=inp.carry_src)
        if self._decode_part_ok(inp, h):
            return self.hidden_states_decode_part(inp, h)
        attn = torch.empty((h.shape[0], self.Hq * self.D), dtype=h.dtype, device=h.device)
        if self.comm is None and inp.meta is not None and inp.meta.kind != "decode":
            L0 = w.layers[0]
            ns = (be.prefill_nsplit(h.shape[0], L0["wo"]), be.prefill_nsplit(h.shape[0], L0["wdown"]))
            if max(ns) > 1:
                return self.hidden_states_splitk(inp, h, attn, *ns)
        last = self._last_rows(inp, h.shape[0])
        for li, L in enumerate(w.layers):
            if last is not None and li + 1 == len(w.layers):
                self._last_layer_rows(li, L, h, inp, attn, last)
                break
            self._attn_block(li, L, h, inp, attn)
            self._allreduce(h)
            self._mlp_block(L, h)
            self._allreduce(h)
        return self._final(h, inp)

    def _last_layer_rows(self, li, L, h, inp: StepInput, attn, mode):
        be, c = self.be, self.cfg
        Hq, Hkv, D = self.Hq, self.Hkv, self.D
        kc, vc = self.kv_cache[li]
        xn = be.rmsnorm(h, L["ln_in"], c.rms_norm_eps)
        qkv = be.gemm_rope_kv(xn, L["wqkv"], inp.positions, self.cos, self.sin, inp.slots, kc, vc, Hq, Hkv, D)
        if mode == "skip":
            return
        mt = inp.m_tiles
        be.attn_prefill(qkv, kc, vc, inp.meta, attn, Hq, Hkv, D, tiles=inp.meta.tiles_last)
        be.gemm(attn, L["wo"], resid=h, epi="resid", out=h, m_tiles=mt)
        xn = be.rmsnorm(h, L["ln_post"], c.rms_norm_eps)
        a = be.gemm(xn, L["wgu"], epi="silu_mul", m_tiles=mt)
        be.gemm(a, L["wdown"], resid=h, epi="resid", out=h, m_tiles=mt)

    def hidden_states_splitk(self, inp: StepInput, h, attn, ns_o, ns_d):
        be, w, c = self.be, self.w, self.cfg
        Hq, Hkv, D = self.Hq, self.Hkv, self.D
        layers = w.layers
        last = self._last_rows(inp, h.shape[0])
        xn = be.rmsnorm(h, layers[0]["ln_in"], c.rms_norm_eps)
        for li, L in enumerate(layers):
            kc, vc = self.kv_cache[li]
            cut = last if li + 1 == len(layers) else None
            rows = {"m_tiles": inp.m_tiles} if cut == "tiles" else {}
            blocks = {"tiles": inp.meta.tiles_last} if cut == "tiles" else {}
            qkv = be.gemm_rope_kv(xn, L["wqkv"], inp.positions, self.cos, self.sin, inp.slots, kc, vc, Hq, Hkv, D)
            if cut == "skip":
                return h.new_empty((0, h.shape[1]))
            be.attn_prefill(qkv, kc, vc, inp.meta, attn, Hq, Hkv, D, **blocks)
            if ns_o > 1:
                xn = be.add_partials_rmsnorm(be.gemm_splitk(attn, L["wo"], ns_o, **rows), h, L["ln_post"],
                                             c.rms_norm_eps)
            else:
                be.gemm(attn, L["wo"], resid=h, epi="resid", out=h, **rows)
                xn = be.rmsnorm(h, L["ln_post"], c.rms_norm_eps)
            a = be.gemm(xn, L["wgu"], epi="silu_mul", **rows)
            nxt = layers[li + 1]["ln_in"] if li + 1 < len(layers) else w.norm
            if ns_d > 1:
                xn = be.add_partials_rmsnorm(be.gemm_splitk(a, L["wdown"], ns_d, **rows), h, nxt, c.rms_norm_eps)
            else:
                be.gemm(a, L["wdown"], resid=h, epi="resid", out=h, **rows)
                xn = be.rmsnorm(h, nxt, c.rms_norm_eps)
        if inp.logits_idx is not None:
            xn = be.gather_rows(xn, inp.logits_idx)
        return xn

    def hidden_states_sp(self, inp: StepInput):
        be, w, c, comm = self.be, self.w, self.cfg, self.comm
        tp, r = comm.size, comm.rank
        Hq, Hkv, D, H = self.Hq, self.Hkv, self.D, c.hidden_size
        T = inp.ids.shape[0]
        S = -(-T // tp)
        Tp = S * tp
        ids = inp.ids
        if Tp != T:
            ids = torch.cat([ids, ids.new_zeros(Tp - T)])
        h = be.embed(ids[r * S:(r + 1) * S].contiguous(), w.embed)
        dev, dt = h.device, h.dtype
        xg = torch.empty((Tp, H), dtype=dt, device=dev)
        part = torch.zeros((Tp, H), dtype=dt, device=dev)
        attn = torch.empty((T, Hq * D), dtype=dt, device=dev)
        rs = torch.empty((S, H), dtype=dt, device=dev)
        for li, L in enumerate(w.layers):
            kc, vc = self.kv_cache[li]
            comm.all_gather_into(xg, be.rmsnorm(h, L["ln_in"], c.rms_norm_eps))
            qkv = be.gemm_rope_kv(xg[:T], L["wqkv"], inp.positions, self.cos, self.sin, inp.slots, kc, vc, Hq, Hkv, D)
            be.attn_prefill(qkv, kc, vc, inp.meta, attn, Hq, Hkv, D)
            be.gemm(attn, L["wo"], out=part[:T])
            h += comm.reduce_scatter(part, rs)
            comm.all_gather_into(xg, be.rmsnorm(h, L["ln_post"], c.rms_norm_eps))
            a = be.gemm(xg[:T], L["wgu"], epi="silu_mul")
            be.gemm(a, L["wdown"], out=part[:T])
            h += comm.reduce_scatter(part, rs)
        comm.all_gather_into(xg, be.rmsnorm(h, w.norm, c.rms_norm_eps))
        x = xg[:T]
        return be.gather_rows(x, inp.logits_idx) if inp.logits_idx is not None else x

    def hidden_states_microbatched(self, inps):
        be, w = self.be, self.w
        hs = [be.embed(i.ids, w.embed) for i in inps]
        attn = [torch.empty((h.shape[0], self.Hq * self.D), dtype=h.dtype, device=h.device) for h in hs]
        pend = [None] * len(hs)
        for li, L in enumerate(w.layers):
            for m, inp in enumerate(inps):
                if pend[m] is not None:
                    pend[m].wait()
                self._attn_block(li, L, hs[m], inp, attn[m])
                pend[m] = self.comm.all_reduce_async(hs[m])
            for m in range(len(inps)):
                pend[m].wait()
                self._mlp_block(L, hs[m])
                pend[m] = self.comm.all_reduce_async(hs[m])
        for p in pend:
            p.wait()
        return [self._final(h, inp) for h, inp in zip(hs, inps)]

    def logits(self, hs):
        return self.be.gemm(hs, self.w.lm_head, out_f32=True)

    def forward(self, inp: StepInput):
        if self.use_sp(inp):
            return self.logits(self.hidden_states_sp(inp))
        return self.logits(self.hidden_states(inp))

    def use_sp(self, inp: StepInput):
        return (self.seq_parallel and self.comm is not None and self.comm.size > 1 and inp.meta is not None
                and inp.meta.kind == "prefill" and inp.ids.shape[0] >= self.sp_min_tokens)
```

rag_llm_k8s_amd/ops/_lib.py:

```python
from __future__ import annotations

import ctypes
import os
import threading

import torch

_HERE = os.path.dirname(os.path.abspath(__file__))
LIB_PATH = os.path.join(os.path.dirname(_HERE), "_lib", "libragk_hip.so")

P, I, F, S, U64 = ctypes.c_void_p, ctypes.c_int, ctypes.c_float, ctypes.c_void_p, ctypes.c_uint64

_SIGS = {
    "ragk_gemm": [P, I, P, I, P, I, P, P, I, I, I, I, I, I, S],
    "ragk_gemm_path": [I, P, I, P, I, P, I, P, P, I, I, I, I, I, S],
    "ragk_gemm_pp": [P, I, P, I, P, I, P, P, I, I, I, I, I, I, S],
    "ragk_gemm_w4_set_grid": [I],
    "ragk_gemm_stream_set_diag": [I],
    "ragk_gemm_stream_set_pair_rows": [I],
    "ragk_gemm_w4": [P, I, P, I, P, I, P, P, I, I, I, I, I, I, P, I, S],
    "ragk_gemm_w4_rope_kv": [P, I, P, I, P, I, I, I, P, P, P, P, P, P, I, I, I, S],
    "ragk_gemm_w4_splitk": [P, I, P, I, P, I, I, I, I, P, I, S],
    "ragk_gemm_part": [P, I, P, I, P, I, I, I, I, S],
    "ragk_gemm_part_norm": [P, I, P, F, P, I, P, I, I, I, I, S],
    "ragk_gemm_part_fp8": [P, I, P, I, P, P, I, I, I, I, S],
    "ragk_gemm_part_merge": [P, P, P, I, P, I, I, I, P, I, P, P, I, I, I, I, S],
    "ragk_gemm_part_merge_ok": [I, I, I, I, I],
    "ragk_gemm_stream_part": [P, I, P, I, P, I, I, I, I, I, S],
    "ragk_gemm_part_silu": [P, I, P, I, P, I, I, I, I, S],
    "ragk_gemm_part_silu_ok": [I, I, I, I],
    "ragk_mlp_engine_ok": [I, I, I, I],
    "ragk_mlp_engine_set_nt": [I],
    "ragk_mlp_engine_set_stamps": [P],
    "ragk_mlp_engine_set_xcd_weights": [I, I],
    "ragk_mlp_engine": [P, P, I, P, F, P, P, P, P, P, P, P, P, I, I, I, I, S],
    "ragk_host_word_alloc": [],
    "ragk_host_word_dev": [P],
    "ragk_host_word_free": [P],
    "ragk_mlp_engine_ctr_bytes": [],
    "ragk_mlp_engine_split": [I, I, I, I, P],
    "ragk_gemm_part_ksteps": [I, I, I, I],
    "ragk_add_partials_rmsnorm": [P, I, I, P, I, P, P, I, I, F, S],
    "ragk_rope_kv_partials": [P, I, I, I, P, I, P, P, P, P, P, P, I, I, I, I, S],
    "ragk_gemm_dec": [P, I, P, I, P, I, P, P, I, I, I, I, I, I, I, P, P, S],
    "ragk_gemm_dec_splits": [I, I, I],
    "ragk_rmsnorm": [P, I, P, I, P, P, I, I, I, F, S],
    "ragk_layernorm": [P, I, P, I, P, P, P, I, I, I, F, S],
    "ragk_embed": [P, P, P, I, I, I, S],
    "ragk_embed_carry": [P, P, P, P, P, I, I, I, S],
    "ragk_embed_ln": [P, P, P, P, P, P, P, P, I, I, F, I, S],
    "ragk_embed_ln_tt": [P, P, P, P, P, P, I, P, P, P, I, I, F, S],
    "ragk_cls_head": [P, I, I, P, P, P, P, F, P, I, I, S],
    "ragk_rerank_select": [P, P, P, P, P, P, P, I, I, I, S],
    "ragk_rope_kv": [P, I, P, P, P, P, P, P, I, I, I, I, I, I, S],
    "ragk_pool_l2norm": [P, I, P, P, I, I, I, I, S],
    "ragk_silu_mul": [P, I, P, I, I, I, S],
    "ragk_gather_rows": [P, I, P, P, I, I, I, S],
    "ragk_attn_prefill_qtile": [I, I],
    "ragk_attn_prefill": [P, I, P, P, P, P, I, P, I, P, P, P, P, I, P, I, I, I, I, I, I, F, S],
    "ragk_attn_decode": [P, I, P, I, I, P, P, P, P, P, P, P, P, P, I, P, P, P, P, I, I, I, I, I, I, I, F,
                         ctypes.c_uint, S],
    "ragk_rope_kv_fp8": [P, I, P, P, P, P, P, P, P, P, I, I, I, I, I, S],
    "ragk_rope_kv_partials_fp8": [P, I, I, I, P, I, P, P, P, P, P, P, P, P, I, I, I, I, S],
    "ragk_topk_candidates": [P, I, I, I, I, I, I, P, P, S],
    "ragk_sample_candidates": [P, P, I, I, P, P, P, P, P, P, P, S],
    "ragk_sample_candidates_lists": [P, P, I, I, I, P, P, P, P, P, P, P, S],
    "ragk_logits_proc_max_hist": [],
    "ragk_hist_write": [P, P, P, P, I, I, I, S],
    "ragk_logits_process": [P, I, I, I, I, P, P, P, P, I, I, P, P, P, I, P, S],
    "ragk_logprobs_max": [],
    "ragk_lse_partials": [P, I, I, I, I, P, S],
    "ragk_logprobs_finish": [P, I, P, P, I, I, I, P, P, P, P, P, P, S],
    "ragk_l2_scan_groups": [I, I, I],
    "ragk_l2_search_groups": [I, I, I, I, I],
    "ragk_l2_search_set_mfma_min_nq": [I],
    "ragk_l2_search": [P, I, I, I, I, P, I, I, P, P, P, P, P, S],
    "ragk_ivf_search": [P, I, I, P, I, P, I, P, P, P, I, P, P, P, P, S],
    "ragk_l2_search_masked": [P, I, I, I, I, P, I, I, P, P, I, I, P, P, P, P, P, S],
    "ragk_ivf_search_masked": [P, I, I, P, I, P, I, P, P, P, I, P, I, I, P, P, P, P, P, S],
    "ragk_kmeans_assign": [P, I, I, P, P, I, P, P, P, S],
    "ragk_l2_scatter": [P, I, I, P, P, I, S],
    "ragk_l2_append": [P, I, I, I, P, I, S],
    "ragk_l2_gather": [P, I, I, P, I, P, S],
    "ragk_gemm_stream": [P, I, P, I, P, P, I, P, P, I, I, I, I, I, I, I, P, P, S],
    "ragk_gemm_stream_splits": [I, I, I, I],
    "ragk_quant_fp8_rows": [P, I, P, I, P, I, I, S],
    "ragk_gemm_fp8": [P, I, P, I, P, P, I, P, P, I, P, P, I, I, I, I, I, I, S],
    "ragk_gemm_mxfp4": [P, I, P, I, P, P, I, P, I, P, I, P, P, I, I, I, I, I, I, S],
    "ragk_ar_create": [I, I, ctypes.c_long, I, I, I],
    "ragk_ar_add_rmsnorm": [P, P, I, I, P, I, P, P, I, I, F, I, S],
    "ragk_ar_fused_rows": [P],
    "ragk_ar_ipc_handle": [P, P],
    "ragk_ar_handle_size": [],
    "ragk_ar_open_peers": [P, P],
    "ragk_ar_max_bytes": [P],
    "ragk_ar_allreduce": [P, P, P, ctypes.c_long, I, S],
    "ragk_ar_error": [P],
    "ragk_ar_set_spin_limit": [P, ctypes.c_uint],
    "ragk_ar_error_host_ptr": [P],
    "ragk_ar_allgather": [P, P, P, ctypes.c_long, S],
    "ragk_ar_destroy": [P],
    "ragk_ar_set_fences": [P, I],
    "ragk_ar_get_fences": [P],
}
_RESTYPES = {"ragk_host_word_alloc": ctypes.c_void_p, "ragk_host_word_dev": ctypes.c_void_p,
             "ragk_ar_create": ctypes.c_void_p, "ragk_ar_error_host_ptr": ctypes.c_void_p, "ragk_ar_max_bytes": ctypes.c_long, "ragk_ar_destroy": None}

_lib = None
_lock = threading.Lock()


class NativeLibraryError(RuntimeError):
    pass


def available() -> bool:
    return os.path.exists(LIB_PATH)


def lib():
    global _lib
    if _lib is not None:
        return _lib
    with _lock:
        if _lib is not None:
            return _lib
        if not os.path.exists(LIB_PATH):
            raise NativeLibraryError(
                "gfx950 kernel library not built (%s). Run `python -m rag_llm_k8s_amd._build` "
                "or __graft_entry__.build()." % LIB_PATH)
        h = ctypes.CDLL(LIB_PATH, mode=ctypes.RTLD_GLOBAL)
        _check_stamp(h)
        for name, args in _SIGS.items():
            fn = getattr(h, name)
            fn.argtypes = args
            fn.restype = _RESTYPES.get(name, ctypes.c_int)
        _lib = h
        return h


def _check_stamp(h):
    if os.environ.get("RAGK_ALLOW_STALE_LIB") == "1":
        return
    from .. import _build

    srcs, _ = _build.hip_sources()
    if not srcs:
        return
    if not hasattr(h, "ragk_build_stamp"):
        raise NativeLibraryError("%s has no build stamp: rebuild it (python -m rag_llm_k8s_amd._build)" % LIB_PATH)
    f = h.ragk_build_stamp
    f.restype = ctypes.c_char_p
    f.argtypes = []
    got, want = f().decode(), _build.source_hash()
    if got != want:
        raise NativeLibraryError("%s was built from other kernel sources (stamp %s, tree %s): rebuild it "
                                 "(python -m rag_llm_k8s_amd._build)" % (LIB_PATH, got, want))


def build_stamp():
    h = lib()
    f = h.ragk_build_stamp
    f.restype = ctypes.c_char_p
    return f().decode()


def has_symbol(name: str) -> bool:
    try:
        return hasattr(lib(), name)
    except NativeLibraryError:
        return False


def stream_ptr(device=None) -> int:
    return torch.cuda.current_stream(device).cuda_stream


def check(rc: int, what: str):
    if rc != 0:
        raise NativeLibraryError("%s failed with hipError %d" % (what, rc))


def ptr(t):
    return None if t is None else t.data_ptr()
```

rag_llm_k8s_amd/ops/backend.py:

```python
from __future__ import annotations

import math
from dataclasses import dataclass, field
from typing import List, Optional

import torch

from . import reference as R
from . import mxfp4
from .fp8 import Fp8KV, Fp8Weight, reference_linear
from .mxfp4 import Mxfp4Weight

KV_BLOCK = 64
_QUANT = (Fp8Weight, Mxfp4Weight)


@dataclass
class AttnMeta:
    kind: str
    kv_lens: torch.Tensor
    block_tables: torch.Tensor
    cu_q: Optional[torch.Tensor] = None
    tiles: Optional[torch.Tensor] = None
    tiles_last: Optional[torch.Tensor] = None
    part_tiles: int = 4
    max_parts: int = 1
    ws_o: Optional[torch.Tensor] = None
    ws_ml: Optional[torch.Tensor] = None
    host_kv_lens: List[int] = field(default_factory=list)
    host_q_lens: List[int] = field(default_factory=list)


class TorchBackend:
    name = "torch"

    def __init__(self, device="cpu"):
        self.device = torch.device(device)

    def gemm(self, x, w, bias=None, resid=None, epi="none", out=None, out_f32=False):
        if isinstance(w, Fp8Weight):
            y = reference_linear(x, w, bias, resid, epi=epi, out_f32=out_f32)
        elif isinstance(w, Mxfp4Weight):
            y = mxfp4.reference_linear(x, w, bias, resid, epi=epi, out_f32=out_f32)
        else:
            y = R.linear(x, w, bias, resid, epi=epi, out_f32=out_f32)
        if out is not None:
            out.copy_(y)
            return out
        return y

    def rmsnorm(self, x, w, eps, out=None):
        y = R.rmsnorm(x, w, eps)
        if out is not None:
            out.copy_(y)
            return out
        return y

    def layernorm(self, x, g, b, eps, out=None, resid=None):
        y = R.layernorm(x, g, b, eps, resid=resid)
        if out is not None:
            out.copy_(y)
            return out
        return y

    def embed(self, ids, table, out=None, carry=None, prev=None):
        if carry is not None:
            c = carry[:ids.numel()].long()
            ids.copy_(torch.where(c >= 0, prev.long()[c.clamp(min=0)], ids.long()).to(ids.dtype))
        y = table[ids.long()]
        if out is not None:
            out.copy_(y)
            return out
        return y

    def embed_ln(self, ids, pos_ids, word, pos, type_row, g, b, eps, do_ln=True):
        h = word[ids.long()].float() + pos[pos_ids.long()].float()
        if type_row is not None:
            h = h + type_row.float().reshape(1, -1)
        if do_ln:
            h = torch.nn.functional.layer_norm(h, (h.shape[-1],), g.float(), b.float(), eps)
        return h.to(word.dtype)

    def gather_rows(self, x, idx):
        return x[idx.long()]

    def silu_mul(self, x):
        I = x.shape[1] // 2
        return (torch.nn.functional.silu(x[:, :I].float()) * x[:, I:].float()).to(x.dtype)

    def rope_kv(self, qkv, positions, cos_t, sin_t, slots, kc, vc, Hq, Hkv, D, apply_rope=True):
        T = qkv.shape[0]
        q = qkv[:, :Hq * D].reshape(T, Hq, D)
        k = qkv[:, Hq * D:(Hq + Hkv) * D].reshape(T, Hkv, D)
        v = qkv[:, (Hq + Hkv) * D:(Hq + 2 * Hkv) * D].reshape(T, Hkv, D)
        if apply_rope:
            p = positions.long()
            q.copy_(R.apply_rope(q, p, cos_t, sin_t))
            k.copy_(R.apply_rope(k, p, cos_t, sin_t))
        if slots is not None and kc is not None:
            s = slots.long()
            ok = s >= 0
            s = s[ok]
            for cache, rows in ((kc, k[ok]), (vc, v[ok])):
                if isinstance(cache, Fp8KV):
                    cache.write_rows(s // KV_BLOCK, s % KV_BLOCK, rows)
                else:
                    cache[s // KV_BLOCK, :, s % KV_BLOCK] = rows

    def gemm_rope_kv(self, x, w, positions, cos_t, sin_t, slots, kc, vc, Hq, Hkv, D):
        qkv = self.gemm(x, w)
        self.rope_kv(qkv, positions, cos_t, sin_t, slots, kc, vc, Hq, Hkv, D)
        return qkv


    enable_part = False

    def part_ok(self, M, w):
        return self.enable_part and M <= 64 and not isinstance(w, Mxfp4Weight)

    def gemm_part(self, x, w):
        wf = w.dequant() if isinstance(w, (Fp8Weight, Mxfp4Weight)) else w.float()
        return (x.float() @ wf.t()).unsqueeze(0)

    def part_norm_ok(self, M, w):
        return self.enable_part and M <= 4 and not isinstance(w, _QUANT) and w.shape[1] <= 8192

    def part_silu_ok(self, M, w_gu, w_down):
        return (self.enable_part and M <= 4 and not isinstance(w_gu, _QUANT) and not isinstance(w_down, _QUANT)
                and w_down.shape[1] % 64 == 0)

    def gemm_part_gu(self, x, w):
        return self.gemm_part(x, w)

    def gemm_part_silu(self, pgu, w):
        gu = pgu.float().sum(0)
        M, K2 = gu.shape
        t = gu.view(M, K2 // 128, 2, 64)
        a = (torch.nn.functional.silu(t[:, :, 0, :]) * t[:, :, 1, :]).reshape(M, K2 // 2).to(torch.bfloat16)
        return self.gemm_part(a, w)

    def gemm_part_norm(self, h, gamma, eps, w):
        return self.gemm_part(R.rmsnorm(h, gamma, eps), w)

    def mlp_engine_ok(self, M, w_gu, w_down):
        return (self.enable_part and M == 1 and not isinstance(w_gu, _QUANT) and not isinstance(w_down, _QUANT)
                and w_down.shape[1] % 64 == 0)

    def mlp_engine(self, xn, w_gu, w_down, h):
        t = (xn.float() @ w_gu.float().t()).view(xn.shape[0], -1, 2, 64)
        a = (torch.nn.functional.silu(t[:, :, 0, :]) * t[:, :, 1, :]).reshape(xn.shape[0], -1).to(torch.bfloat16)
        h.copy_((h.float() + a.float() @ w_down.float().t()).to(h.dtype))
        return h

    def mlp_engine_tail(self, P, h, gamma, eps, w_gu, w_down):
        return self.mlp_engine(self.add_partials_rmsnorm(P, h, gamma, eps), w_gu, w_down, h)

    def add_partials_rmsnorm(self, P, h, w, eps):
        h.copy_((h.float() + P.sum(0).to(h.dtype).float()).to(h.dtype))
        return R.rmsnorm(h, w, eps)

    def rope_kv_partials(self, P, q_out, positions, cos_t, sin_t, slots, kc, vc, Hq, Hkv, D):
        qkv = P.sum(0).to(q_out.dtype)
        self.rope_kv(qkv, positions, cos_t, sin_t, slots, kc, vc, Hq, Hkv, D)
        q_out[:, :Hq * D].copy_(qkv[:, :Hq * D])

    def attn_prefill(self, q, kc, vc, meta: AttnMeta, out, Hq, Hkv, D):
        T = q.shape[0]
        qq = q[:, :Hq * D].reshape(T, Hq, D)
        bt = meta.block_tables.cpu()
        lens = meta.host_kv_lens

        def view(cache, s):
            if isinstance(cache, Fp8KV):
                return (R.paged_kv_view(cache.data.view(torch.uint8), bt[s], lens[s], KV_BLOCK).view(cache.data.dtype).float()
                        * _paged_scale_view(cache.scale, bt[s], lens[s])[..., None])
            return R.paged_kv_view(cache, bt[s], lens[s], KV_BLOCK)

        o = R.attention_varlen(qq, None, None, meta.cu_q.cpu(), lens, True, 1.0 / math.sqrt(D),
                               k_full=lambda s: view(kc, s), v_full=lambda s: view(vc, s))
        out.copy_(o.reshape(T, Hq * D))
        return out

    def attn_decode_rope(self, P, positions, cos_t, sin_t, slots, kc, vc, meta: AttnMeta, out, Hq, Hkv, D,
                         defer_merge=False):
        q = torch.empty((P.shape[1], Hq * D), dtype=out.dtype, device=out.device)
        self.rope_kv_partials(P, q, positions, cos_t, sin_t, slots, kc, vc, Hq, Hkv, D)
        return self.attn_decode(q, kc, vc, meta, out, Hq, Hkv, D)

    def part_merge_ok(self, M, meta: AttnMeta, w, Hq, D):
        return False

    def prefill_nsplit(self, M, w):
        return 1

    def m_tiles_ok(self, M, w, epi="none"):
        return False

    def attn_decode(self, q, kc, vc, meta: AttnMeta, out, Hq, Hkv, D):
        B = q.shape[0]
        cu = torch.arange(B + 1, dtype=torch.int32)
        m = AttnMeta("prefill", meta.kv_lens, meta.block_tables, cu_q=cu, host_kv_lens=meta.host_kv_lens)
        return self.attn_prefill(q, kc, vc, m, out, Hq, Hkv, D)

    def attn_encoder(self, qkv, cu, lens_host, tiles, out, H, D):
        T = qkv.shape[0]
        q = qkv[:, :H * D].reshape(T, H, D)
        k = qkv[:, H * D:2 * H * D].reshape(T, H, D)
        v = qkv[:, 2 * H * D:3 * H * D].reshape(T, H, D)
        o = R.attention_varlen(q, k, v, cu.cpu(), lens_host, False, 1.0 / math.sqrt(D), cu_kv=cu.cpu())
        out.copy_(o.reshape(T, H * D))
        return out

    def pool_l2norm(self, hidden, cu, mode="cls", normalize=True):
        return R.pool_l2norm(hidden, cu.cpu(), mode=mode, normalize=normalize)

    def embed_ln_tt(self, ids, pos_ids, type_ids, word, pos, type_table, g, b, eps):
        return R.embed_ln_tt(ids, pos_ids, type_ids, word, pos, type_table, g, b, eps)

    def cls_head(self, h, cu, w1, b1, w2, b2):
        return R.cls_head(h, cu, w1, b1, w2, b2)

    def rerank_select(self, scores, cand_ids, cand_dist, n_valid, k):
        if not 1 <= scores.shape[1] <= R.SELECT_MAX_N or not 1 <= k <= scores.shape[1]:
            raise ValueError("rerank_select: need 1 <= k <= N <= %d" % R.SELECT_MAX_N)
        return R.rerank_select(scores, cand_ids, cand_dist, n_valid, k)

    def topk_candidates(self, logits, K, vocab_offset=0, max_cand=512, chunks=None):
        k = min(K, logits.shape[1])
        v, i = torch.topk(logits.float(), k, dim=-1)
        if k < K:
            v = torch.cat([v, torch.full((v.shape[0], K - k), float("-inf"))], 1)
            i = torch.cat([i, torch.full((i.shape[0], K - k), -1)], 1)
        return v, (i + vocab_offset).int()

    def hist_write(self, ids, rows, pos, hist):
        return R.hist_write(ids, rows, pos, hist)

    def logits_process(self, logits, vocab_offset, ids, rows, pos, hist, penalty, ngram, ban_ids, ban_count):
        return R.logits_process(logits, vocab_offset, ids, rows, pos, hist, penalty, ngram, ban_ids, ban_count)

    def lse_partials(self, logits, chunks, out=None):
        return R.lse_partials(logits, chunks, out=out)

    def logprobs_finish(self, part, cand_v, cand_i, list_len, tok, nlp, out_lse=None, out_tok_lp=None,
                        out_top_lp=None, out_top_id=None):
        return R.logprobs_finish(part, cand_v, cand_i, list_len, tok, nlp, out_lse, out_tok_lp, out_top_lp,
                                 out_top_id)

    def sample_candidates(self, cand_v, cand_i, temps, top_ks, top_ps, seeds, steps, list_len=None):
        out = torch.empty(cand_v.shape[0], dtype=torch.int32)
        for b in range(cand_v.shape[0]):
            order = torch.argsort(cand_v[b], descending=True, stable=True)
            v, i = cand_v[b][order], cand_i[b][order]
            k = int(top_ks[b])
            k = len(v) if k <= 0 or k > len(v) else k
            v, i = v[:k], i[:k]
            t = float(temps[b])
            if t <= 0:
                out[b] = int(i[0])
                continue
            g = torch.Generator().manual_seed((int(seeds[b]) * 1000003 + int(steps[b])) & 0x7FFFFFFFFFFFFFFF)
            u = float(torch.rand(1, generator=g))
            _, _, pick = R.sample_from_logits_candidates(v, i, t, float(top_ps[b]), u)
            out[b] = pick
        return out


class NativeBackend(TorchBackend):
    name = "native"

    def __init__(self, device="cuda"):
        super().__init__(device)
        from . import native

        self.n = native
        native._lib.lib()

    def gemm(self, x, w, bias=None, resid=None, epi="none", out=None, out_f32=False, m_tiles=None):
        if m_tiles is not None and isinstance(w, _QUANT):
            raise ValueError("m_tiles: bf16 weights only")
        if isinstance(w, Fp8Weight):
            return self.n.gemm_fp8(x, w, bias=bias, resid=resid, epi=epi, out=out, out_f32=out_f32)
        if isinstance(w, Mxfp4Weight):
            return self.n.gemm_mxfp4(x, w, bias=bias, resid=resid, epi=epi, out=out, out_f32=out_f32)
        return self.n.gemm(x, w, bias=bias, resid=resid, epi=epi, out=out, out_f32=out_f32, m_tiles=m_tiles)

    def m_tiles_ok(self, M, w, epi="none"):
        if isinstance(w, _QUANT):
            return False
        N = w.shape[0] // 2 if epi == "silu_mul" else w.shape[0]
        return self.n.gemm_m_tiles_ok(M, N, w.shape[1], epi, ldb=w.stride(0))

    def rmsnorm(self, x, w, eps, out=None):
        return self.n.rmsnorm(x, w, eps, out=out)

    def layernorm(self, x, g, b, eps, out=None, resid=None):
        return self.n.layernorm(x, g, b, eps, out=out, resid=resid)

    def embed(self, ids, table, out=None, carry=None, prev=None):
        return self.n.embed(ids, table, out=out, carry=carry, prev=prev)

    def embed_ln(self, ids, pos_ids, word, pos, type_row, g, b, eps, do_ln=True):
        return self.n.embed_ln(ids, pos_ids, word, pos, type_row, g, b, eps, do_ln=do_ln)

    def gather_rows(self, x, idx):
        return self.n.gather_rows(x, idx)

    def silu_mul(self, x):
        return self.n.silu_mul(x)

    def rope_kv(self, qkv, positions, cos_t, sin_t, slots, kc, vc, Hq, Hkv, D, apply_rope=True):
        self.n.rope_kv(qkv, positions, cos_t, sin_t, slots, kc, vc, Hq, Hkv, D, apply_rope=apply_rope)

    def gemm_rope_kv(self, x, w, positions, cos_t, sin_t, slots, kc, vc, Hq, Hkv, D):
        if self.n.gemm_rope_kv_ok(x, w, positions, cos_t, sin_t, slots, kc, vc, Hq, Hkv, D):
            return self.n.gemm_rope_kv(x, w, positions, cos_t, sin_t, slots, kc, vc, Hq, Hkv, D)
        qkv = self.gemm(x, w)
        self.rope_kv(qkv, positions, cos_t, sin_t, slots, kc, vc, Hq, Hkv, D)
        return qkv

    enable_part = __import__("os").environ.get("RAGK_DECODE_PART", "1") == "1"

    def part_ok(self, M, w):
        if not self.enable_part or M > 64 or isinstance(w, Mxfp4Weight):
            return False
        return self.n.gemm_part_slabs(M, w.shape[0], w.shape[1])[1] > 0

    def gemm_part(self, x, w):
        return self.n.gemm_part(x, w)

    def part_norm_ok(self, M, w):
        return self.enable_part and M <= 4 and not isinstance(w, _QUANT) and w.shape[1] in (4096, 8192)

    def gemm_part_norm(self, h, gamma, eps, w):
        return self.n.gemm_part_norm(h, gamma, eps, w)

    def part_silu_ok(self, M, w_gu, w_down):
        return self.enable_part and self.n.gemm_part_silu_ok(M, w_gu, w_down)

    def gemm_part_gu(self, x, w):
        return self.n.gemm_part_gu(x, w)

    def gemm_part_silu(self, pgu, w):
        return self.n.gemm_part_silu(pgu, w)

    def add_partials_rmsnorm(self, P, h, w, eps):
        return self.n.add_partials_rmsnorm(P, h, w, eps)

    def mlp_engine_ok(self, M, w_gu, w_down):
        return self.n.mlp_engine_ok(M, w_gu, w_down)

    def mlp_engine(self, xn, w_gu, w_down, h):
        return self.n.mlp_engine(xn, w_gu, w_down, h)

    def mlp_engine_tail(self, P, h, gamma, eps, w_gu, w_down):
        return self.n.mlp_engine_tail(P, h, gamma, eps, w_gu, w_down)

    def rope_kv_partials(self, P, q_out, positions, cos_t, sin_t, slots, kc, vc, Hq, Hkv, D):
        self.n.rope_kv_partials(P, q_out, positions, cos_t, sin_t, slots, kc, vc, Hq, Hkv, D)

    def attn_prefill(self, q, kc, vc, meta: AttnMeta, out, Hq, Hkv, D, tiles=None):
        return self.n.attn_prefill(q, kc, vc, meta.cu_q, meta.kv_lens, meta.tiles if tiles is None else tiles, out,
                                   Hq, Hkv, D, causal=True, paged=True, block_tables=meta.block_tables)

    def attn_decode_rope(self, P, positions, cos_t, sin_t, slots, kc, vc, meta: AttnMeta, out, Hq, Hkv, D,
                         defer_merge=False):
        return self.n.attn_decode_rope(P, positions, cos_t, sin_t, slots, kc, vc, meta.block_tables, meta.kv_lens, out,
                                       Hq, Hkv, D, meta.part_tiles, meta.max_parts, meta.ws_o, meta.ws_ml,
                                       defer_merge=defer_merge)

    def prefill_nsplit(self, M, w):
        if isinstance(w, _QUANT):
            return 1
        return self.n.prefill_nsplit(M, w.shape[0], w.shape[1])

    def gemm_splitk(self, x, w, nsplit, m_tiles=None):
        return self.n.gemm_splitk(x, w, nsplit, m_tiles=m_tiles)

    def part_merge_ok(self, M, meta: AttnMeta, w, Hq, D):
        return (self.enable_part and D == 128 and not isinstance(w, Mxfp4Weight)
                and self.n.gemm_part_merge_ok(M, w, Hq, meta.max_parts, meta.ws_o))

    def gemm_part_merge(self, attn_out, meta: AttnMeta, w, Hq):
        return self.n.gemm_part_merge(attn_out, meta.kv_lens, meta.part_tiles, meta.max_parts, meta.ws_o, meta.ws_ml,
                                      Hq, w)

    def attn_decode(self, q, kc, vc, meta: AttnMeta, out, Hq, Hkv, D):
        return self.n.attn_decode(q, kc, vc, meta.block_tables, meta.kv_lens, out, Hq, Hkv, D, meta.part_tiles,
                                  meta.max_parts, meta.ws_o, meta.ws_ml)

    def attn_encoder(self, qkv, cu, lens_host, tiles, out, H, D):
        return self.n.attn_prefill(qkv, qkv[:, H * D:], qkv[:, 2 * H * D:], cu, _lens_dev(cu), tiles, out, H, H, D,
                                   causal=False, paged=False, cu_kv=cu, kv_stride=qkv.stride(0))

    def pool_l2norm(self, hidden, cu, mode="cls", normalize=True):
        return self.n.pool_l2norm(hidden, cu, mode=mode, normalize=normalize)

    def embed_ln_tt(self, ids, pos_ids, type_ids, word, pos, type_table, g, b, eps):
        return self.n.embed_ln_tt(ids, pos_ids, type_ids, word, pos, type_table, g, b, eps)

    def cls_head(self, h, cu, w1, b1, w2, b2):
        return self.n.cls_head(h, cu, w1, b1, w2, b2)

    def rerank_select(self, scores, cand_ids, cand_dist, n_valid, k):
        return self.n.rerank_select(scores, cand_ids, cand_dist, n_valid, k)

    def topk_candidates(self, logits, K, vocab_offset=0, max_cand=512, chunks=None):
        return self.n.topk_candidates(logits, K, vocab_offset=vocab_offset, max_cand=max_cand, chunks=chunks)

    def hist_write(self, ids, rows, pos, hist):
        return self.n.hist_write(ids, rows, pos, hist)

    def logits_process(self, logits, vocab_offset, ids, rows, pos, hist, penalty, ngram, ban_ids, ban_count):
        return self.n.logits_process(logits, vocab_offset, ids, rows, pos, hist, penalty, ngram, ban_ids, ban_count)

    def lse_partials(self, logits, chunks, out=None):
        return self.n.lse_partials(logits, chunks, out=out)

    def logprobs_finish(self, part, cand_v, cand_i, list_len, tok, nlp, out_lse=None, out_tok_lp=None,
                        out_top_lp=None, out_top_id=None):
        return self.n.logprobs_finish(part, cand_v, cand_i, list_len, tok, nlp, out_lse, out_tok_lp, out_top_lp,
                                      out_top_id)

    def sample_candidates(self, cand_v, cand_i, temps, top_ks, top_ps, seeds, steps, list_len=None):
        return self.n.sample_candidates(cand_v, cand_i, temps, top_ks, top_ps, seeds, steps, list_len=list_len)


def _paged_scale_view(scale, block_table, L):
    nb = (L + KV_BLOCK - 1) // KV_BLOCK
    return scale[block_table[:nb].long()].permute(0, 2, 1).reshape(nb * KV_BLOCK, scale.shape[1])[:L]


def _lens_dev(cu):
    return (cu[1:] - cu[:-1]).contiguous()


def get_backend(device) -> TorchBackend:
    dev = torch.device(device)
    return NativeBackend(dev) if dev.type == "cuda" else TorchBackend(dev)
```

rag_llm_k8s_amd/ops/native.py:

```python
from __future__ import annotations

import math
import os
import threading

import torch

from . import _lib
from ._lib import check, ptr, stream_ptr
from .fp8 import FP8, Fp8KV
from .reference import EPI


def _req(cond, msg):
    if not cond:
        raise ValueError(msg)


def _kv8(k_cache, v_cache, Hkv, D, dev):
    _req(isinstance(k_cache, Fp8KV) and isinstance(v_cache, Fp8KV), "fp8 KV cache: both k and v must be Fp8KV")
    _req(D == 128, "fp8 KV cache needs head_dim 128")
    kd = k_cache.data
    _req(kd.dim() == 4 and kd.shape[1] == Hkv and kd.shape[2] == 64 and kd.shape[3] == D, "fp8 cache [nb,Hkv,64,128]")
    for side, c in (("k", k_cache), ("v", v_cache)):
        _req(c.data.dtype == FP8 and c.data.shape == kd.shape and c.data.is_contiguous() and c.data.is_cuda
             and c.data.device == dev, "%s cache data must be contiguous e4m3fn on the launch device" % side)
        _req(c.scale.dtype == torch.float32 and c.scale.shape == kd.shape[:3] and c.scale.is_contiguous()
             and c.scale.device == dev, "%s cache scales must be contiguous fp32 [nb,Hkv,64] on the cache's device" % side)
    return kd.shape[0]


def _bf16_2d(t, name):
    _req(t.is_cuda and t.dtype == torch.bfloat16 and t.dim() == 2, "%s must be a 2-D bf16 GPU tensor" % name)
    _req(t.stride(1) == 1, "%s must be row-contiguous" % name)


def _al16(t, name):
    if t is None:
        return
    _req(t.data_ptr() % 16 == 0, "%s: base pointer must be 16-byte aligned (column offset of a view?)" % name)
    _req(t.dim() < 2 or t.shape[0] <= 1 or (t.stride(0) * t.element_size()) % 16 == 0,
         "%s: row pitch must be a multiple of 16 bytes (got %d elements)" % (name, t.stride(0) if t.dim() > 1 else 0))


PP_MIN_M = 1024


def set_w4_grid(g):
    check(_lib.lib().ragk_gemm_w4_set_grid(int(g)), "ragk_gemm_w4_set_grid")




DEC_DEFAULT = True
DEC_WS_BYTES = 96 << 20
_dec_ws = {}


def dec_workspace(device):
    key = str(device)
    if key not in _dec_ws:
        _dec_ws[key] = (torch.empty(DEC_WS_BYTES // 4, dtype=torch.float32, device=device),
                        torch.zeros(65536, dtype=torch.int32, device=device))
    return _dec_ws[key]


def use_dec(M, N, K, epi):
    return 16 < M <= 64 and N >= 32768 and K % 256 == 0 and epi != "silu_mul"


STREAM_DEFAULT = True
STREAM_MIN_ROWS = 16384
STREAM_MAX_ROWS = 262144
STREAM_VOCAB_MIN_M = 17


def use_stream(M, N, K, epi, fp8=False):
    rows = 2 * N if epi == "silu_mul" else N
    if M > 64 or not (STREAM_MIN_ROWS <= rows < STREAM_MAX_ROWS) or K % 128:
        return False
    if rows >= 32768 and M < STREAM_VOCAB_MIN_M:
        return False
    return M > 16 if fp8 else True


def use_pp(M, N, K, epi):
    if M < PP_MIN_M or K % 64 or K < 192:
        return False
    return N % 128 == 0 if epi == "silu_mul" else N % 8 == 0


PREFILL_BLAS = os.environ.get("RAGK_PREFILL_BLAS", "none")


PREFILL_ROPE_FUSED = os.environ.get("RAGK_PREFILL_ROPE", "1") != "0"


def gemm_rope_kv_ok(x, w, positions, cos_t, sin_t, slots, k_cache, v_cache, Hq, Hkv, D):
    if not PREFILL_ROPE_FUSED or D != 128 or slots is None or k_cache is None or v_cache is None:
        return False
    if isinstance(k_cache, Fp8KV) or isinstance(v_cache, Fp8KV):
        return False
    if not (isinstance(x, torch.Tensor) and isinstance(w, torch.Tensor) and x.is_cuda and w.dim() == 2):
        return False
    M, K = x.shape
    N = w.shape[0]
    if N != (Hq + 2 * Hkv) * D or N % 256 or w.shape[1] != K or not use_pp(M, N, K, "none"):
        return False
    if PREFILL_BLAS in ("plain", "all"):
        return False
    if x.dtype != torch.bfloat16 or w.dtype != torch.bfloat16 or x.stride(1) != 1 or w.stride(1) != 1:
        return False
    if x.stride(0) * M * 2 >= 2 ** 31 or w.stride(0) * N * 2 >= 2 ** 31:
        return False
    if not (k_cache.is_contiguous() and v_cache.is_contiguous() and k_cache.dim() == 4 and k_cache.shape[1] == Hkv
            and k_cache.shape[3] == D and v_cache.shape == k_cache.shape and k_cache.dtype == torch.bfloat16):
        return False
    if not (cos_t.dtype == torch.float32 and sin_t.dtype == torch.float32 and cos_t.is_contiguous()
            and sin_t.is_contiguous() and cos_t.shape[-1] == D // 2):
        return False
    return (positions.dtype == torch.int32 and slots.dtype == torch.int32 and positions.is_contiguous()
            and slots.is_contiguous() and positions.numel() == M and slots.numel() == M)


def gemm_rope_kv(x, w, positions, cos_t, sin_t, slots, k_cache, v_cache, Hq, Hkv, D, out=None):
    _req(gemm_rope_kv_ok(x, w, positions, cos_t, sin_t, slots, k_cache, v_cache, Hq, Hkv, D), "gemm_rope_kv operands")
    M, K = x.shape
    N = w.shape[0]
    if out is None:
        out = torch.empty((M, N), dtype=torch.bfloat16, device=x.device)
    _req(out.shape == (M, N) and out.stride(1) == 1 and out.stride(0) % 8 == 0, "gemm_rope_kv out")
    check(_lib.lib().ragk_gemm_w4_rope_kv(x.data_ptr(), x.stride(0), w.data_ptr(), w.stride(0), out.data_ptr(),
                                          out.stride(0), M, K, positions.data_ptr(), slots.data_ptr(),
                                          cos_t.data_ptr(), sin_t.data_ptr(), k_cache.data_ptr(), v_cache.data_ptr(),
                                          Hq, Hkv, k_cache.shape[2], stream_ptr()), "ragk_gemm_w4_rope_kv")
    return out


def _gemm_blas(x, w, resid, out, epi):
    if epi == "resid":
        if out.data_ptr() == resid.data_ptr() and out.stride() == resid.stride():
            return out.addmm_(x, w.t())
        return torch.addmm(resid, x, w.t(), out=out)
    return torch.mm(x, w.t(), out=out)


def _m_tiles_arg(m_tiles, M, dev):
    _req(isinstance(m_tiles, torch.Tensor) and m_tiles.dtype == torch.int32 and m_tiles.dim() == 1
         and m_tiles.is_contiguous() and m_tiles.is_cuda and m_tiles.device == dev, "m_tiles: int32 [n] on the GPU")
    _req(m_tiles.numel() <= -(-M // 256), "m_tiles: more entries than 256-row tiles")
    return m_tiles.data_ptr(), m_tiles.numel()


def gemm_m_tiles_ok(M, N, K, epi="none", lda=None, ldb=None):
    if epi not in ("none", "resid", "silu_mul") or PREFILL_BLAS != "none" or not use_pp(M, N, K, epi):
        return False
    rows = 2 * N if epi == "silu_mul" else N
    return (lda or K) * M * 2 < 2 ** 31 and (ldb or K) * rows * 2 < 2 ** 31


def gemm(x, w, bias=None, resid=None, epi="none", out=None, out_f32=False, path=None, m_tiles=None):
    _bf16_2d(x, "x")
    _bf16_2d(w, "w")
    M, K = x.shape
    e = EPI[epi]
    N = w.shape[0] // 2 if epi == "silu_mul" else w.shape[0]
    _req(w.shape[1] == K, "K mismatch %s vs %s" % (tuple(x.shape), tuple(w.shape)))
    _req(K % 128 == 0, "K must be a multiple of 128 (got %d)" % K)
    if epi == "silu_mul":
        _req(N % 64 == 0, "silu_mul needs N % 64 == 0")
    if "bias" in epi:
        _req(bias is not None and bias.is_cuda and bias.dtype == torch.bfloat16 and bias.numel() == N
             and bias.is_contiguous(), "bias must be bf16[N]")
    if "resid" in epi:
        _bf16_2d(resid, "resid")
        _req(resid.shape == (M, N), "resid shape")
    odt = torch.float32 if out_f32 else torch.bfloat16
    if out is None:
        out = torch.empty((M, N), dtype=odt, device=x.device)
    _req(out.dtype == odt and out.shape == (M, N) and out.stride(1) == 1, "out shape/dtype")
    if M > 64 and N % 8 != 0 and epi != "silu_mul":
        raise ValueError("tile GEMM needs N % 8 == 0")
    if M == 0:
        return out
    _al16(x, "x")
    _al16(w, "w")
    L = _lib.lib()
    ldr = resid.stride(0) if resid is not None else 0
    mt_ptr, mt_n = None, 0
    if m_tiles is not None:
        _req(path in (None, 6), "m_tiles: only the gemm_w4 path takes an M-tile list")
        _req(epi in ("none", "resid", "silu_mul") and not out_f32, "m_tiles: epi none / resid / silu_mul, bf16 out")
        _req(K % 64 == 0 and K >= 192 and (N % 128 == 0 if epi == "silu_mul" else N % 8 == 0), "m_tiles: gemm_w4 shape")
        _req(x.stride(0) * M * 2 < 2 ** 31 and w.stride(0) * w.shape[0] * 2 < 2 ** 31, "m_tiles: operand past 2 GiB")
        mt_ptr, mt_n = _m_tiles_arg(m_tiles, M, x.device)
        if mt_n == 0:
            return out
        path = 6
    if (path is None and PREFILL_BLAS != "none" and not out_f32 and bias is None and use_pp(M, N, K, epi)
            and ((epi == "none" and PREFILL_BLAS in ("plain", "all"))
                 or (epi == "resid" and PREFILL_BLAS in ("resid", "all")))):
        return _gemm_blas(x, w, resid, out, epi)
    if path is None and use_pp(M, N, K, epi):
        rows = w.shape[0]
        fits = x.stride(0) * M * 2 < 2 ** 31 and w.stride(0) * rows * 2 < 2 ** 31
        path = 6 if fits else 2
    if path is None and STREAM_DEFAULT and use_stream(M, N, K, epi):
        path = 5
    if path is None and DEC_DEFAULT and use_dec(M, N, K, epi):
        path = 4
    _req(path in (None, 0, 1, 2, 3, 4, 5, 6), "unknown GEMM path %r" % (path,))
    if path in (0, 2, 6) or (path is None and M > 64):
        _al16(out, "out")
        if "bias" in epi:
            _al16(bias, "bias")
        if "resid" in epi:
            _al16(resid, "resid")
    if path == 5:
        rc = _gemm_stream(x, w, None, out, bias, resid, ldr, M, N, K, epi, e, out_f32)
    elif path == 4:
        ws, cnt = dec_workspace(x.device)
        S = L.ragk_gemm_dec_splits(N, K, e)
        need = S * (2 if epi == "silu_mul" else 1) * M * N
        _req(S == 1 or need <= ws.numel(), "decode GEMM workspace too small (%d > %d floats)" % (need, ws.numel()))
        _req(-(-N // 128) <= cnt.numel(), "too many n-tiles for the counter buffer")
        rc = L.ragk_gemm_dec(x.data_ptr(), x.stride(0), w.data_ptr(), w.stride(0), out.data_ptr(), out.stride(0),
                             ptr(bias), ptr(resid), ldr, M, N, K, e, int(out_f32), S, ws.data_ptr(), cnt.data_ptr(),
                             stream_ptr())
    elif path == 2:
        rc = L.ragk_gemm_pp(x.data_ptr(), x.stride(0), w.data_ptr(), w.stride(0), out.data_ptr(), out.stride(0),
                            ptr(bias), ptr(resid), ldr, M, N, K, e, int(out_f32), stream_ptr())
    elif path == 6:
        rc = L.ragk_gemm_w4(x.data_ptr(), x.stride(0), w.data_ptr(), w.stride(0), out.data_ptr(), out.stride(0),
                            ptr(bias), ptr(resid), ldr, M, N, K, e, int(out_f32), mt_ptr, mt_n, stream_ptr())
    elif path is None:
        rc = L.ragk_gemm(x.data_ptr(), x.stride(0), w.data_ptr(), w.stride(0), out.data_ptr(), out.stride(0),
                         ptr(bias), ptr(resid), ldr, M, N, K, e, int(out_f32), stream_ptr())
    else:
        rc = L.ragk_gemm_path(path, x.data_ptr(), x.stride(0), w.data_ptr(), w.stride(0), out.data_ptr(),
                              out.stride(0), ptr(bias), ptr(resid), ldr, M, N, K, e, stream_ptr())
    check(rc, "ragk_gemm")
    return out


PART_MIN_BLOCKS = 512


def gemm_part_slabs(M, N, K, ks=None):
    ks = ks or _lib.lib().ragk_gemm_part_ksteps(M, N, K, PART_MIN_BLOCKS)
    if ks <= 0 or K % (64 * ks):
        return 0, 0
    return ks, K // (64 * ks)


def gemm_part_norm(h, gamma, eps, w, out=None, ks=None):
    _bf16_2d(h, "h")
    _bf16_2d(w, "w")
    M, K = h.shape
    N = w.shape[0]
    _req(w.shape[1] == K and M <= 4 and K <= 8192 and gamma.numel() == K and gamma.dtype == torch.bfloat16
         and gamma.is_contiguous(), "gemm_part_norm shape")
    ks, S = gemm_part_slabs(1, N, K, ks)
    if ks not in (8, 16):
        ks, S = gemm_part_slabs(1, N, K, 16)
    _req(S > 0 and K in (4096, 8192), "gemm_part_norm: unsupported K=%d" % K)
    _al16(h, "h")
    _al16(w, "w")
    _al16(gamma, "gamma")
    if out is None:
        out = torch.empty((S, M, N), dtype=torch.float32, device=h.device)
    check(_lib.lib().ragk_gemm_part_norm(h.data_ptr(), h.stride(0), gamma.data_ptr(), float(eps), w.data_ptr(),
                                         w.stride(0), out.data_ptr(), M, N, K, ks, stream_ptr()),
          "ragk_gemm_part_norm")
    return out


STREAM_PART = True
STREAM_PART_MIN_M = 5
STREAM_PART_ROWS = 0
STREAM_PART_MAX_S = 64


def stream_part_cfg(M, N, K):
    cus = _cu_count()
    steps = K // 64
    best = (0, 0, 0)
    for rows, per_cu in ((128, 1), (64, 2)):
        if STREAM_PART_ROWS and rows != STREAM_PART_ROWS:
            continue
        tiles = -(-N // rows)
        S = 1
        while (tiles * S * 2 <= per_cu * cus and steps % (S * 2) == 0 and steps // (S * 2) >= 8
               and S * 2 <= STREAM_PART_MAX_S):
            S *= 2
        blocks = tiles * S
        if blocks <= per_cu * cus and (blocks / per_cu, rows) > (best[2], best[0]):
            best = (rows, S, blocks / per_cu)
    if best[2] < 0.5 * cus:
        return 0, 0
    return best[0], best[1]


def gemm_stream_part(x, w, out=None, rows=None, S=None):
    _bf16_2d(x, "x")
    _bf16_2d(w, "w")
    M, K = x.shape
    N = w.shape[0]
    _req(w.shape[1] == K and M <= 64 and K % 64 == 0 and N % 4 == 0, "gemm_stream_part shape")
    r0, s0 = stream_part_cfg(M, N, K)
    rows, S = rows or r0, S or s0
    _req(rows in (64, 128) and S >= 1 and (K // 64) % S == 0, "gemm_stream_part config")
    _al16(x, "x")
    _al16(w, "w")
    if out is None:
        out = torch.empty((S, M, N), dtype=torch.float32, device=x.device)
    _req(out.dtype == torch.float32 and out.is_contiguous() and out.numel() >= S * M * N and out.data_ptr() % 16 == 0,
         "gemm_stream_part out: contiguous fp32 [S, M, N], 16-byte aligned")
    check(_lib.lib().ragk_gemm_stream_part(x.data_ptr(), x.stride(0), w.data_ptr(), w.stride(0), out.data_ptr(), M, N,
                                           K, S, rows, stream_ptr()), "ragk_gemm_stream_part")
    return out


def gemm_part(x, w, out=None, ks=None):
    from .fp8 import Fp8Weight

    _bf16_2d(x, "x")
    fp8 = isinstance(w, Fp8Weight)
    wt = w.w8 if fp8 else w
    if fp8:
        _req(wt.is_cuda and wt.dim() == 2 and wt.stride(1) == 1 and wt.element_size() == 1, "fp8 weight rows")
        _req(w.scale.dtype == torch.float32 and w.scale.is_contiguous(), "fp8 weight scales fp32")
    else:
        _bf16_2d(wt, "w")
    M, K = x.shape
    N = wt.shape[0]
    _req(wt.shape[1] == K and M <= 64, "gemm_part shape %s x %s" % (tuple(x.shape), tuple(wt.shape)))
    _al16(x, "x")
    _al16(wt, "w")
    if (STREAM_PART and not fp8 and ks is None and out is None and M >= STREAM_PART_MIN_M and K % 64 == 0
            and N % 4 == 0 and stream_part_cfg(M, N, K)[1] > 0):
        return gemm_stream_part(x, wt)
    ks, S = gemm_part_slabs(M, N, K, ks)
    _req(S > 0, "gemm_part: unsupported K=%d" % K)
    if out is None:
        out = torch.empty((S, M, N), dtype=torch.float32, device=x.device)
    _req(out.dtype == torch.float32 and out.is_contiguous() and out.numel() >= S * M * N, "gemm_part out")
    if fp8:
        check(_lib.lib().ragk_gemm_part_fp8(x.data_ptr(), x.stride(0), wt.data_ptr(), wt.stride(0),
                                            w.scale.data_ptr(), out.data_ptr(), M, N, K, ks, stream_ptr()),
              "ragk_gemm_part_fp8")
    else:
        check(_lib.lib().ragk_gemm_part(x.data_ptr(), x.stride(0), wt.data_ptr(), wt.stride(0), out.data_ptr(), M, N,
                                        K, ks, stream_ptr()), "ragk_gemm_part")
    return out[:S] if out.dim() == 3 else out


PREFILL_SPLITK = True
PREFILL_SPLITK_MIN_M = 4096
_n_cus = [0]


def _cu_count():
    if not _n_cus[0]:
        try:
            _n_cus[0] = torch.cuda.get_device_properties(torch.cuda.current_device()).multi_processor_count
        except Exception:
            _n_cus[0] = 256
    return _n_cus[0]


def prefill_nsplit(M, N, K):
    if not PREFILL_SPLITK or M < PREFILL_SPLITK_MIN_M:
        return 1
    cus = _cu_count()
    tiles = -(-M // 256) * -(-N // 256)
    best, best_s = 0.0, 1
    for s in (1, 2):
        if K % (64 * s) or K // s < 4 * 64:
            continue
        wt = tiles * s
        eff = wt / (-(-wt // cus) * cus) - 0.02 * (s - 1)
        if eff > best + 1e-9:
            best, best_s = eff, s
    return best_s


def gemm_splitk(x, w, nsplit, out=None, m_tiles=None):
    _bf16_2d(x, "x")
    _bf16_2d(w, "w")
    M, K = x.shape
    N = w.shape[0]
    _req(w.shape[1] == K and K % (64 * nsplit) == 0 and K // nsplit >= 256 and N % 8 == 0, "gemm_splitk shape")
    if out is None:
        out = torch.empty((nsplit, M, N), dtype=torch.float32, device=x.device)
    _req(out.dtype == torch.float32 and out.is_contiguous() and out.numel() >= nsplit * M * N
         and out.data_ptr() % 16 == 0, "gemm_splitk out: contiguous fp32 slabs, 16-byte aligned")
    _al16(x, "x")
    _al16(w, "w")
    mt_ptr, mt_n = _m_tiles_arg(m_tiles, M, x.device) if m_tiles is not None else (None, 0)
    if m_tiles is not None and mt_n == 0:
        return out
    check(_lib.lib().ragk_gemm_w4_splitk(x.data_ptr(), x.stride(0), w.data_ptr(), w.stride(0), out.data_ptr(), M, N, K,
                                         nsplit, mt_ptr, mt_n, stream_ptr()), "ragk_gemm_w4_splitk")
    return out


def gemm_part_merge_ok(M, w, Hq, max_parts, ws_o):
    from .fp8 import Fp8Weight

    if ws_o is None or max_parts < 2:
        return False
    wt = w.w8 if isinstance(w, Fp8Weight) else w
    N, K = wt.shape
    ks, S = gemm_part_slabs(M, N, K)
    return S > 0 and bool(_lib.lib().ragk_gemm_part_merge_ok(M, K, Hq, max_parts, ks))


def gemm_part_merge(attn_out, kv_lens, part_tiles, max_parts, ws_o, ws_ml, Hq, w, out=None):
    from .fp8 import Fp8Weight

    fp8 = isinstance(w, Fp8Weight)
    wt = w.w8 if fp8 else w
    M = kv_lens.numel()
    N, K = wt.shape
    _req(attn_out.dtype == torch.bfloat16 and attn_out.stride(1) == 1 and attn_out.shape[0] >= M
         and attn_out.shape[1] == K, "attention output rows")
    _req(ws_o is not None and ws_o.dtype == torch.float32 and ws_o.numel() >= M * Hq * max_parts * 128
         and ws_ml.numel() >= M * Hq * max_parts * 2, "partition workspace")
    ks, S = gemm_part_slabs(M, N, K)
    _req(S > 0 and _lib.lib().ragk_gemm_part_merge_ok(M, K, Hq, max_parts, ks), "gemm_part_merge shape")
    if out is None:
        out = torch.empty((S, M, N), dtype=torch.float32, device=attn_out.device)
    check(_lib.lib().ragk_gemm_part_merge(
        ws_o.data_ptr(), ws_ml.data_ptr(), attn_out.data_ptr(), attn_out.stride(0), kv_lens.data_ptr(), Hq,
        part_tiles, max_parts, wt.data_ptr(), wt.stride(0), w.scale.data_ptr() if fp8 else None, out.data_ptr(), M, N,
        K, ks, stream_ptr()), "ragk_gemm_part_merge")
    return out

# ... 25 lines not shown
    if w_gu.shape[0] != 2 * K or K % 64 or ks_gu == 0 or M > 4:
        return False
    S1 = w_gu.shape[1] // (64 * ks_gu)
    ks = _silu_ks(M, N, K)
    return ks > 0 and bool(_lib.lib().ragk_gemm_part_silu_ok(M, S1, K, ks))


def gemm_part_gu(x, w_gu):
    return gemm_part(x, w_gu, ks=gemm_part_gu_ks(x.shape[1]))


def gemm_part_silu(pgu, w, out=None):
    _bf16_2d(w, "w")
    _req(pgu.dtype == torch.float32 and pgu.is_cuda and pgu.is_contiguous() and pgu.dim() == 3, "pgu fp32 [S1, M, 2K]")
    S1, M, K2 = pgu.shape
    N, K = w.shape
    _req(K2 == 2 * K, "pgu holds packed gate/up columns of width 2K")
    ks = _silu_ks(M, N, K)
    _req(ks > 0 and _lib.lib().ragk_gemm_part_silu_ok(M, S1, K, ks), "gemm_part_silu shape")
    S = K // (64 * ks)
    if out is None:
        out = torch.empty((S, M, N), dtype=torch.float32, device=pgu.device)
    _req(out.shape == (S, M, N) and out.dtype == torch.float32, "out [S, M, N] fp32")
    check(_lib.lib().ragk_gemm_part_silu(pgu.data_ptr(), S1, w.data_ptr(), w.stride(0), out.data_ptr(), M, N, K, ks,
                                         stream_ptr()), "ragk_gemm_part_silu")
    return out


MLP_ENGINE = os.environ.get("RAGK_MLP_ENGINE", "1") != "0"
_me_ws = {}


class _MeWorkspace:

    def __init__(self, dev, I):
        L = _lib.lib()
        self.nb = int(L.ragk_mlp_engine_ctr_bytes())
        self.words = torch.zeros(self.nb // 8 + 2, dtype=torch.int64, device=dev)
        self.act = torch.zeros(I, dtype=torch.bfloat16, device=dev)
        self.host = L.ragk_host_word_alloc()
        _req(bool(self.host), "mlp_engine: hipHostMalloc of the host error word failed")
        self.host_dev = L.ragk_host_word_dev(self.host)
        _req(bool(self.host_dev), "mlp_engine: no device address for the host error word")
        import ctypes

        self._host_word = ctypes.c_uint.from_address(self.host)

    @property
    def err_ptr(self):
        return self.words.data_ptr() + self.nb

    @property
    def tmo_ptr(self):
        return self.words.data_ptr() + self.nb + 8

    def fault(self) -> int:
        return int(self._host_word.value)

    def rearm(self):
        self.words[: self.nb // 8 + 1].zero_()
        self._host_word.value = 0

    def __del__(self):
        try:
            if self.host:
                _lib.lib().ragk_host_word_free(self.host)
                self.host = None
        except Exception:
            pass


def _me_workspace(dev, I):
    key = (str(dev), stream_ptr(), I)
    ws = _me_ws.get(key)
    if ws is None:
        _req(not torch.cuda.is_current_stream_capturing(),
             "mlp_engine workspace: run one eager step on the capture stream before capture")
        ws = _me_ws[key] = _MeWorkspace(dev, I)
    return ws


def mlp_engine_ok(M, w_gu, w_down):
    if not MLP_ENGINE or not (isinstance(w_gu, torch.Tensor) and isinstance(w_down, torch.Tensor)):
        return False
    if w_gu.dtype != torch.bfloat16 or w_down.dtype != torch.bfloat16 or not w_gu.is_cuda:
        return False
    H, I = w_down.shape
    if w_gu.shape != (2 * I, H) or not (w_gu.is_contiguous() and w_down.is_contiguous()):
        return False
    return bool(_lib.lib().ragk_mlp_engine_ok(M, H, I, _cu_count()))


def mlp_engine(xn, w_gu, w_down, h):
    _bf16_2d(xn, "xn")
    _req(xn.shape == (1, w_down.shape[0]) and xn.is_contiguous(), "xn [1, H]")
    return _mlp_engine_launch(xn.data_ptr(), None, 0, None, 0.0, w_gu, w_down, h)


def mlp_engine_tail(P, h, gamma, eps, w_gu, w_down):
    H = w_down.shape[0]
    _req(P.dtype == torch.float32 and P.is_cuda and P.is_contiguous() and P.dim() == 3 and P.shape[1:] == (1, H),
         "P [S, 1, H] fp32")
    _req(gamma.dtype == torch.bfloat16 and gamma.is_contiguous() and gamma.numel() == H, "gamma [H] bf16")
    return _mlp_engine_launch(None, P.data_ptr(), P.shape[0], gamma.data_ptr(), float(eps), w_gu, w_down, h)


def _mlp_engine_launch(xn_ptr, P_ptr, S, g_ptr, eps, w_gu, w_down, h):
    _bf16_2d(h, "h")
    H, I = w_down.shape
    _req(h.shape == (1, H) and h.is_contiguous(), "h [1, H]")
    _req(mlp_engine_ok(1, w_gu, w_down), "mlp_engine shape")
    ws = _me_workspace(h.device, I)
    check(_lib.lib().ragk_mlp_engine(xn_ptr, P_ptr, S, g_ptr, eps, w_gu.data_ptr(), w_down.data_ptr(), h.data_ptr(),
                                     ws.act.data_ptr(), ws.words.data_ptr(), ws.err_ptr, ws.host_dev, ws.tmo_ptr, 1,
                                     H, I, _cu_count(), stream_ptr()),
          "ragk_mlp_engine")
    return h


def mlp_engine_fault(dev=None) -> int:
    d = torch.device(dev) if dev is not None else None
    for key, ws in list(_me_ws.items()):
        if d is not None and d.index is not None and torch.device(key[0]) != d:
            continue
        e = ws.fault()
        if e:
            return e
    return 0


def mlp_engine_rearm(dev=None):
    d = torch.device(dev) if dev is not None else None
    for key, ws in list(_me_ws.items()):
        if d is None or d.index is None or torch.device(key[0]) == d:
            ws.rearm()


def mlp_engine_check(dev=None):
    if not _me_ws:
        return
    torch.cuda.synchronize(dev)
    e = mlp_engine_fault(dev)
    if e:
        mlp_engine_rearm(dev)
        raise RuntimeError("persistent decode MLP: wait timed out (code %d); counters reset" % e)


def mlp_engine_force_timeout(ticks, dev=None):
    d = torch.device(dev) if dev is not None else None
    for key, ws in list(_me_ws.items()):
        if d is None or d.index is None or torch.device(key[0]) == d:
            ws.words[ws.nb // 8 + 1].fill_(int(ticks))


def set_mlp_engine_nt(nt):
    check(_lib.lib().ragk_mlp_engine_set_nt(int(nt)), "ragk_mlp_engine_set_nt")


STREAM_S_OVERRIDE = 0


def _gemm_stream(x, w, wscale, out, bias, resid, ldr, M, N, K, epi, e, out_f32):
    L = _lib.lib()
    fp8 = wscale is not None
    S = STREAM_S_OVERRIDE or L.ragk_gemm_stream_splits(N, K, e, int(fp8))
    ws, cnt = dec_workspace(x.device)
    rows = 2 * N if epi == "silu_mul" else N
    _req(S == 1 or S * M * (-(-rows // 128) * 128) <= ws.numel(), "stream GEMM workspace too small")
    _req(-(-rows // 64) <= cnt.numel(), "too many n-tiles for the counter buffer")
    return L.ragk_gemm_stream(x.data_ptr(), x.stride(0), w.data_ptr(), w.stride(0), ptr(wscale), out.data_ptr(),
                              out.stride(0), ptr(bias), ptr(resid), ldr, M, N, K, e, int(out_f32), S, ws.data_ptr(),
                              cnt.data_ptr(), stream_ptr())


def quant_fp8_rows(x, q=None, scale=None):
    _bf16_2d(x, "x")
    M, K = x.shape
    _req(K % 8 == 0, "K % 8")
    q = torch.empty((M, K), dtype=torch.float8_e4m3fn, device=x.device) if q is None else q
    scale = torch.empty(M, dtype=torch.float32, device=x.device) if scale is None else scale
    _req(q.shape == (M, K) and q.is_contiguous() and scale.numel() == M, "quant buffers")
    _al16(x, "x")
    _req(q.data_ptr() % 8 == 0, "q: base pointer must be 8-byte aligned")
    check(_lib.lib().ragk_quant_fp8_rows(x.data_ptr(), x.stride(0), q.data_ptr(), q.stride(0), scale.data_ptr(), M, K,
                                         stream_ptr()), "ragk_quant_fp8_rows")
    return q, scale


FP8_DEC_STREAM = True


def gemm_fp8(x, w, bias=None, resid=None, epi="none", out=None, out_f32=False, act=None):
    from .fp8 import DEC_MAX_M

    if act is None:
        _bf16_2d(x, "x")
        _al16(x, "x")
        M, K = x.shape
        dev = x.device
    else:
        q, sa = act
        _req(q.dtype == torch.float8_e4m3fn and q.is_cuda and q.dim() == 2 and q.stride(1) == 1
             and q.stride(0) % 16 == 0 and q.data_ptr() % 16 == 0, "act q e4m3 [M,K], 16-byte aligned rows")
        M, K = q.shape
        _req(sa.dtype == torch.float32 and sa.is_cuda and sa.is_contiguous() and sa.numel() == M, "act scale fp32[M]")
        dev = q.device
    w8, sw = w.w8, w.scale
    _req(w8.dtype == torch.float8_e4m3fn and w8.is_cuda and w8.is_contiguous() and w8.shape[1] == K
         and w8.data_ptr() % 16 == 0, "fp8 weight: contiguous e4m3 [rows, K], 16-byte aligned")
    _req(sw.dtype == torch.float32 and sw.is_cuda and sw.is_contiguous() and sw.numel() == w8.shape[0], "fp8 scale")
    _req(K % 128 == 0, "K must be a multiple of 128")
    e = EPI[epi]
    N = w8.shape[0] // 2 if epi == "silu_mul" else w8.shape[0]
    dec = act is None and M <= DEC_MAX_M
    if epi == "silu_mul":
        _req(N % 64 == 0 and not out_f32, "silu_mul needs N % 64 == 0, bf16 out")
    elif not dec:
        _req(N % 8 == 0, "N % 8")
    if "bias" in epi:
        _req(bias is not None and bias.is_cuda and bias.dtype == torch.bfloat16 and bias.numel() == N
             and bias.is_contiguous(), "bias bf16[N]")
    if "resid" in epi:
        _bf16_2d(resid, "resid")
        _req(resid.shape == (M, N), "resid shape")
    odt = torch.float32 if out_f32 else torch.bfloat16
    out = torch.empty((M, N), dtype=odt, device=dev) if out is None else out
    _req(out.dtype == odt and out.shape == (M, N) and out.stride(1) == 1, "out shape/dtype")
    if not dec:
        _al16(out, "out")
        if "bias" in epi:
            _al16(bias, "bias")
        if "resid" in epi:
            _al16(resid, "resid")
    if M == 0:
        return out
    ldr = resid.stride(0) if resid is not None else 0
    if dec and FP8_DEC_STREAM and use_stream(M, N, K, epi, fp8=True):
        rc = _gemm_stream(x, w8, sw, out, bias, resid, ldr, M, N, K, epi, e, out_f32)
    elif dec:
        rc = _lib.lib().ragk_gemm_fp8(x.data_ptr(), x.stride(0), None, 0, None, w8.data_ptr(), w8.stride(0),
                                      sw.data_ptr(), out.data_ptr(), out.stride(0), ptr(bias), ptr(resid), ldr, M, N,
                                      K, e, int(out_f32), stream_ptr())
    else:
        q, sa = quant_fp8_rows(x) if act is None else act
        rc = _lib.lib().ragk_gemm_fp8(None, 0, q.data_ptr(), q.stride(0), sa.data_ptr(), w8.data_ptr(), w8.stride(0),
                                      sw.data_ptr(), out.data_ptr(), out.stride(0), ptr(bias), ptr(resid), ldr, M, N,
                                      K, e, int(out_f32), stream_ptr())
    check(rc, "ragk_gemm_fp8")
    return out


def gemm_mxfp4(x, w, bias=None, resid=None, epi="none", out=None, out_f32=False, act=None):
    from .fp8 import DEC_MAX_M

    if act is None:
        _bf16_2d(x, "x")
        M, K = x.shape
        dev = x.device
    else:
        q, sa = act
        _req(q.dtype == torch.float8_e4m3fn and q.is_cuda and q.dim() == 2 and q.stride(1) == 1
             and q.stride(0) % 16 == 0 and q.data_ptr() % 16 == 0, "act q e4m3 [M,K], 16-byte aligned rows")
        M, K = q.shape
        _req(sa.dtype == torch.float32 and sa.is_cuda and sa.is_contiguous() and sa.numel() == M, "act scale fp32[M]")
        dev = q.device
    w4, sw = w.packed, w.scale
    _req(w4.dtype == torch.uint8 and w4.is_cuda and w4.is_contiguous() and w4.shape[1] * 2 == K, "mxfp4 weight")
    _req(sw.dtype == torch.uint8 and sw.is_cuda and sw.is_contiguous() and sw.shape == (w4.shape[0], K // 32),
         "mxfp4 scale")
    _req(K % 128 == 0, "K must be a multiple of 128")
    e = EPI[epi]
    N = w4.shape[0] // 2 if epi == "silu_mul" else w4.shape[0]
    dec = act is None and M <= DEC_MAX_M
    if epi == "silu_mul":
        _req(N % 64 == 0 and not out_f32, "silu_mul needs N % 64 == 0, bf16 out")
    elif not dec:
        _req(N % 8 == 0, "N % 8")
    if "bias" in epi:
        _req(bias is not None and bias.dtype == torch.bfloat16 and bias.numel() == N, "bias bf16[N]")
    if "resid" in epi:
        _bf16_2d(resid, "resid")
        _req(resid.shape == (M, N), "resid shape")
    odt = torch.float32 if out_f32 else torch.bfloat16
    out = torch.empty((M, N), dtype=odt, device=dev) if out is None else out
    _req(out.dtype == odt and out.shape == (M, N) and out.stride(1) == 1, "out shape/dtype")
    if not dec:
        _req(out.stride(0) % 8 == 0 and out.data_ptr() % 16 == 0, "out rows 16-byte aligned")
    if M == 0:
        return out
    ldr = resid.stride(0) if resid is not None else 0
    if dec:
        rc = _lib.lib().ragk_gemm_mxfp4(x.data_ptr(), x.stride(0), None, 0, None, w4.data_ptr(), w4.stride(0),
                                        sw.data_ptr(), sw.stride(0), out.data_ptr(), out.stride(0), ptr(bias),
                                        ptr(resid), ldr, M, N, K, e, int(out_f32), stream_ptr())
    else:
        q, sa = quant_fp8_rows(x) if act is None else act
        rc = _lib.lib().ragk_gemm_mxfp4(None, 0, q.data_ptr(), q.stride(0), sa.data_ptr(), w4.data_ptr(),
                                        w4.stride(0), sw.data_ptr(), sw.stride(0), out.data_ptr(), out.stride(0),
                                        ptr(bias), ptr(resid), ldr, M, N, K, e, int(out_f32), stream_ptr())
    check(rc, "ragk_gemm_mxfp4")
    return out


def rmsnorm(x, w, eps, out=None, resid=None):
    _bf16_2d(x, "x")
    T, H = x.shape
    _req(w.numel() == H and w.dtype == torch.bfloat16, "weight")
    _req(H % 8 == 0 and H <= 8192, "H must be a multiple of 8, <= 8192")
    if resid is not None:
        _bf16_2d(resid, "resid")
        _req(resid.shape == x.shape, "resid shape")
    out = torch.empty_like(x) if out is None else out
    _req(out.is_cuda and out.dtype == torch.bfloat16 and out.shape == x.shape and out.stride(1) == 1, "out shape/dtype")
    _al16(x, "x")
    _al16(resid, "resid")
    _al16(w, "weight")
    _al16(out, "out")
    check(_lib.lib().ragk_rmsnorm(x.data_ptr(), x.stride(0), ptr(resid), resid.stride(0) if resid is not None else 0,
                                  w.data_ptr(), out.data_ptr(), out.stride(0), T, H, float(eps), stream_ptr()),
          "ragk_rmsnorm")
    return out


def layernorm(x, g, b, eps, out=None, resid=None):
    _bf16_2d(x, "x")
    T, H = x.shape
    _req(H % 8 == 0 and H <= 8192, "H")
    out = torch.empty_like(x) if out is None else out
    check(_lib.lib().ragk_layernorm(x.data_ptr(), x.stride(0), ptr(resid), resid.stride(0) if resid is not None else 0,
                                    g.data_ptr(), b.data_ptr(), out.data_ptr(), out.stride(0), T, H, float(eps),
                                    stream_ptr()), "ragk_layernorm")
    return out


def embed(ids, table, out=None, carry=None, prev=None):
    _req(ids.dtype == torch.int32 and ids.is_cuda and ids.is_contiguous(), "ids int32")
    V, H = table.shape
    out = torch.empty((ids.numel(), H), dtype=table.dtype, device=table.device) if out is None else out
    if carry is None:
        check(_lib.lib().ragk_embed(ids.data_ptr(), table.data_ptr(), out.data_ptr(), ids.numel(), H, V,
                                    stream_ptr()), "ragk_embed")
        return out
    _req(carry.dtype == torch.int32 and prev.dtype == torch.int32 and carry.numel() >= ids.numel(), "carry int32")
    check(_lib.lib().ragk_embed_carry(ids.data_ptr(), carry.data_ptr(), prev.data_ptr(), table.data_ptr(),
                                      out.data_ptr(), ids.numel(), H, V, stream_ptr()), "ragk_embed_carry")
    return out


def embed_ln(ids, pos_ids, word, pos, type_row, g, b, eps, do_ln=True, out=None):
    _req(ids.dtype == torch.int32 and pos_ids.dtype == torch.int32, "int32 ids")
    _req(int(ids.numel()) == int(pos_ids.numel()), "ids/pos_ids")
    H = word.shape[1]
    out = torch.empty((ids.numel(), H), dtype=word.dtype, device=word.device) if out is None else out
    check(_lib.lib().ragk_embed_ln(ids.data_ptr(), pos_ids.data_ptr(), word.data_ptr(), pos.data_ptr(),
                                   ptr(type_row), ptr(g), ptr(b), out.data_ptr(), ids.numel(), H, float(eps),
                                   int(do_ln), stream_ptr()), "ragk_embed_ln")
    return out


def embed_ln_tt(ids, pos_ids, type_ids, word, pos, type_table, g, b, eps, out=None):
    T = int(ids.numel())
    for t, name in ((ids, "ids"), (pos_ids, "pos_ids"), (type_ids, "type_ids")):
        _req(t.is_cuda and t.dtype == torch.int32 and t.is_contiguous() and int(t.numel()) == T, "%s: int32 [T]" % name)
    _bf16_2d(word, "word")
    _bf16_2d(pos, "pos")
    _bf16_2d(type_table, "type_table")
    H = word.shape[1]
    _req(H % 8 == 0 and H <= 8192, "H must be a multiple of 8, at most 8192")
    _req(pos.shape[1] == H and type_table.shape[1] == H and type_table.shape[0] >= 1, "table widths")
    _req(word.is_contiguous() and pos.is_contiguous() and type_table.is_contiguous(), "contiguous tables")
    _req(g.dtype == torch.bfloat16 and b.dtype == torch.bfloat16 and g.numel() == H and b.numel() == H, "LN weights")
    out = torch.empty((T, H), dtype=word.dtype, device=word.device) if out is None else out
    _req(out.shape == (T, H) and out.is_contiguous(), "out")
    for t, name in ((word, "word"), (pos, "pos"), (type_table, "type_table"), (g, "g"), (b, "b"), (out, "out")):
        _al16(t, name)
    check(_lib.lib().ragk_embed_ln_tt(ids.data_ptr(), pos_ids.data_ptr(), type_ids.data_ptr(), word.data_ptr(),
                                      pos.data_ptr(), type_table.data_ptr(), type_table.shape[0], g.data_ptr(),
                                      b.data_ptr(), out.data_ptr(), T, H, float(eps), stream_ptr()), "ragk_embed_ln_tt")
    return out


CLS_HEAD_MAX_H = 1024


def cls_head(h, cu, w1, b1, w2, b2, out=None):
    _bf16_2d(h, "h")
    T, H = h.shape
    _req(H % 64 == 0 and 64 <= H <= CLS_HEAD_MAX_H,
         "cls_head: H must be a multiple of 64 in 64..%d (got %d)" % (CLS_HEAD_MAX_H, H))
    _req(T >= 1, "cls_head: empty hidden states")
    _req(cu.is_cuda and cu.dtype == torch.int32 and cu.is_contiguous() and cu.numel() >= 1, "cu: int32 [B + 1]")
    B = cu.numel() - 1
    _bf16_2d(w1, "w1")
    _req(tuple(w1.shape) == (H, H) and w1.is_contiguous(), "w1: [H, H]")
    for t, name in ((b1, "b1"), (w2, "w2")):
        _req(t.is_cuda and t.dtype == torch.bfloat16 and t.numel() == H and t.is_contiguous(), "%s: bf16 [H]" % name)
    _al16(h, "h")
    _al16(w1, "w1")
    out = torch.empty((B,), dtype=torch.float32, device=h.device) if out is None else out
    _req(out.dtype == torch.float32 and out.is_contiguous() and out.numel() >= B, "out: fp32 [B]")
    check(_lib.lib().ragk_cls_head(h.data_ptr(), h.stride(0), T, cu.data_ptr(), w1.data_ptr(), b1.data_ptr(),
                                   w2.data_ptr(), float(b2), out.data_ptr(), B, H, stream_ptr()), "ragk_cls_head")
    return out


def rerank_select(scores, cand_ids, cand_dist, n_valid, k, out=None):
    _req(scores.is_cuda and scores.dtype == torch.float32 and scores.dim() == 2 and scores.is_contiguous(), "scores")
    Q, N = scores.shape
    _req(1 <= N <= 64, "rerank_select: N must be in 1..64 (got %d)" % N)
    _req(1 <= k <= N, "rerank_select: k must be in 1..N (got %d)" % k)
    _req(cand_ids.is_cuda and cand_ids.dtype == torch.int64 and tuple(cand_ids.shape) == (Q, N)
         and cand_ids.is_contiguous(), "cand_ids: int64 [Q, N]")
    _req(cand_dist.is_cuda and cand_dist.dtype == torch.float32 and tuple(cand_dist.shape) == (Q, N)
         and cand_dist.is_contiguous(), "cand_dist: fp32 [Q, N]")
    _req(n_valid.is_cuda and n_valid.dtype == torch.int32 and n_valid.numel() == Q and n_valid.is_contiguous(),
         "n_valid: int32 [Q]")
    if out is None:
        out = (torch.empty((Q, k), dtype=torch.int64, device=scores.device),
               torch.empty((Q, k), dtype=torch.float32, device=scores.device),
               torch.empty((Q, k), dtype=torch.float32, device=scores.device))
    oi, od, os_ = out
    _req(oi.dtype == torch.int64 and od.dtype == torch.float32 and os_.dtype == torch.float32, "out dtypes")
    for t in out:
        _req(t.is_contiguous() and t.numel() >= Q * k, "out: [Q, k]")
    check(_lib.lib().ragk_rerank_select(scores.data_ptr(), cand_ids.data_ptr(), cand_dist.data_ptr(),
                                        n_valid.data_ptr(), oi.data_ptr(), od.data_ptr(), os_.data_ptr(), Q, N, k,
                                        stream_ptr()), "ragk_rerank_select")
    return out


def rope_kv(qkv, positions, cos_t, sin_t, slots, k_cache, v_cache, Hq, Hkv, D, apply_rope=True):
    _bf16_2d(qkv, "qkv")
    T = qkv.shape[0]
    _req(qkv.shape[1] >= (Hq + 2 * Hkv) * D, "qkv width")
    _req(positions.dtype == torch.int32 and positions.numel() == T, "positions")
    if isinstance(k_cache, Fp8KV) or isinstance(v_cache, Fp8KV):
        _req(apply_rope, "fp8 KV cache: rope_kv without RoPE is not built")
        _req(slots is not None and slots.dtype == torch.int32 and slots.numel() == T, "slots")
        _req(cos_t is not None and sin_t is not None, "rope tables")
        _kv8(k_cache, v_cache, Hkv, D, qkv.device)
        check(_lib.lib().ragk_rope_kv_fp8(qkv.data_ptr(), qkv.stride(0), positions.data_ptr(), cos_t.data_ptr(),
                                          sin_t.data_ptr(), slots.data_ptr(), k_cache.data.data_ptr(),
                                          v_cache.data.data_ptr(), k_cache.scale.data_ptr(), v_cache.scale.data_ptr(),
                                          T, Hq, Hkv, D, 64, stream_ptr()), "ragk_rope_kv_fp8")
        return
    if slots is not None:
        _req(slots.dtype == torch.int32 and slots.numel() == T, "slots")
        _req(k_cache.dim() == 4 and k_cache.shape[1] == Hkv and k_cache.shape[3] == D, "cache layout")
    BS = k_cache.shape[2] if k_cache is not None else 64
    check(_lib.lib().ragk_rope_kv(qkv.data_ptr(), qkv.stride(0), positions.data_ptr(), ptr(cos_t), ptr(sin_t),
                                  ptr(slots), ptr(k_cache), ptr(v_cache), T, Hq, Hkv, D, BS, int(apply_rope),
                                  stream_ptr()), "ragk_rope_kv")


def add_partials_rmsnorm(P, h, w, eps, out=None):
    _bf16_2d(h, "h")
    M, H = h.shape
    _req(P.dtype == torch.float32 and P.is_contiguous() and P.dim() == 3 and P.shape[1:] == (M, H), "partials shape")
    _req(w.is_cuda and w.dtype == torch.bfloat16 and w.numel() == H, "norm weight")
    out = torch.empty_like(h) if out is None else out
    _req(out.shape == (M, H) and out.stride(1) == 1, "out")
    for t, name in ((P, "partials"), (h, "h"), (w, "norm weight"), (out, "out")):
        _al16(t, name)
    check(_lib.lib().ragk_add_partials_rmsnorm(P.data_ptr(), P.shape[0], M, h.data_ptr(), h.stride(0), w.data_ptr(),
                                               out.data_ptr(), out.stride(0), H, float(eps), stream_ptr()),
          "ragk_add_partials_rmsnorm")
    return out


def rope_kv_partials(P, q_out, positions, cos_t, sin_t, slots, k_cache, v_cache, Hq, Hkv, D):
    _req(P.dtype == torch.float32 and P.is_contiguous() and P.dim() == 3, "partials")
    S, T, ldp = P.shape
    _req(ldp >= (Hq + 2 * Hkv) * D, "qkv width")
    _bf16_2d(q_out, "q_out")
    _req(q_out.shape[0] == T and q_out.shape[1] >= Hq * D, "q_out shape")
    _req(positions.dtype == torch.int32 and positions.numel() == T, "positions")
    _req(slots is not None and slots.dtype == torch.int32 and slots.numel() == T, "slots")
    _req(P.data_ptr() % 16 == 0 and ldp % 4 == 0, "partials: 16-byte aligned rows")
    _al16(q_out, "q_out")
    if isinstance(k_cache, Fp8KV) or isinstance(v_cache, Fp8KV):
        _kv8(k_cache, v_cache, Hkv, D, P.device)
        check(_lib.lib().ragk_rope_kv_partials_fp8(P.data_ptr(), S, T, ldp, q_out.data_ptr(), q_out.stride(0),
                                                   positions.data_ptr(), ptr(cos_t), ptr(sin_t), slots.data_ptr(),
                                                   k_cache.data.data_ptr(), v_cache.data.data_ptr(),
                                                   k_cache.scale.data_ptr(), v_cache.scale.data_ptr(), Hq, Hkv, D, 64,
                                                   stream_ptr()), "ragk_rope_kv_partials_fp8")
        return
    _req(k_cache.dim() == 4 and k_cache.shape[1] == Hkv and k_cache.shape[3] == D, "cache layout")
    check(_lib.lib().ragk_rope_kv_partials(P.data_ptr(), S, T, ldp, q_out.data_ptr(), q_out.stride(0),
                                           positions.data_ptr(), ptr(cos_t), ptr(sin_t), slots.data_ptr(),
                                           k_cache.data_ptr(), v_cache.data_ptr(), Hq, Hkv, D, k_cache.shape[2],
                                           stream_ptr()), "ragk_rope_kv_partials")


def pool_l2norm(hidden, cu, mode="cls", normalize=True, out=None):
    _bf16_2d(hidden, "hidden")
    B = cu.numel() - 1
    H = hidden.shape[1]
    _req(H <= 2048, "H <= 2048")
    m = {"cls": 0, "mean": 1, "last": 2}[mode]
    out = torch.empty((B, H), dtype=torch.float32, device=hidden.device) if out is None else out
    check(_lib.lib().ragk_pool_l2norm(hidden.data_ptr(), hidden.stride(0), cu.data_ptr(), out.data_ptr(), B, H, m,
                                      int(normalize), stream_ptr()), "ragk_pool_l2norm")
    return out


def silu_mul(x, out=None):
    _bf16_2d(x, "x")
    T, I2 = x.shape
    I = I2 // 2
    out = torch.empty((T, I), dtype=x.dtype, device=x.device) if out is None else out
    check(_lib.lib().ragk_silu_mul(x.data_ptr(), x.stride(0), out.data_ptr(), out.stride(0), T, I, stream_ptr()),
          "ragk_silu_mul")
    return out


def gather_rows(x, idx, out=None):
    _bf16_2d(x, "x")
    _req(idx.dtype == torch.int32 and idx.is_cuda, "idx int32")
    n = idx.numel()
    out = torch.empty((n, x.shape[1]), dtype=x.dtype, device=x.device) if out is None else out
    check(_lib.lib().ragk_gather_rows(x.data_ptr(), x.stride(0), idx.data_ptr(), out.data_ptr(), out.stride(0), n,
                                      x.shape[1], stream_ptr()), "ragk_gather_rows")
    return out


def prefill_qtile(Hq, Hkv):
    G = Hq // Hkv
    GB = 4 if G % 4 == 0 else (2 if G % 2 == 0 else 1)
    return 32 * ((8 if GB == 4 else 4) // GB)


def build_prefill_tiles(q_lens, Hq, Hkv):
    import numpy as np

    qt = prefill_qtile(Hq, Hkv)
    ql = np.asarray(q_lens, dtype=np.int64)
    nt = (ql + qt - 1) // qt
    seq = np.repeat(np.arange(len(ql)), nt)
    first = np.repeat(np.cumsum(nt) - nt, nt)
    q0 = (np.arange(int(nt.sum())) - first) * qt
    order = np.argsort(-q0, kind="stable")
    return torch.from_numpy(np.stack([seq[order], q0[order]], 1).astype(np.int32)).reshape(-1, 2)


M_TILE_ROWS = 256


def build_last_rows_lists(q_lens, rows, Hq, Hkv, tiles=None):
    import numpy as np

    qt = prefill_qtile(Hq, Hkv)
    if tiles is None:
        tiles = build_prefill_tiles(q_lens, Hq, Hkv)
    t = tiles.numpy().reshape(-1, 2).astype(np.int64)
    ql = np.asarray(q_lens, dtype=np.int64)
    cu = np.concatenate([[0], np.cumsum(ql)])
    r = np.unique(np.asarray(rows, dtype=np.int64).reshape(-1))
    if r.size and (r[0] < 0 or r[-1] >= cu[-1]):
        raise ValueError("build_last_rows_lists: row outside the packed step")
    lo = cu[t[:, 0]] + t[:, 1]
    hi = np.minimum(lo + qt, cu[t[:, 0] + 1])
    keep = np.searchsorted(r, lo, side="left") < np.searchsorted(r, hi, side="left")
    tiles_last = torch.from_numpy(np.ascontiguousarray(t[keep]).astype(np.int32)).reshape(-1, 2)
    m_tiles = torch.from_numpy(np.unique(r // M_TILE_ROWS).astype(np.int32))
    return tiles_last, m_tiles


def attn_prefill(q, k, v, cu_q, kv_lens, tiles, out, Hq, Hkv, D, causal=True, paged=True, block_tables=None,
                 cu_kv=None, kv_stride=0, scale=None):
    _req(q.dtype == torch.bfloat16 and q.stride(-1) == 1, "q")
    _req(tiles.dtype == torch.int32 and tiles.is_cuda and tiles.is_contiguous(), "tiles int32 on GPU")
    _req(D in (32, 64, 128), "head_dim must be 32/64/128")
    f8 = isinstance(k, Fp8KV) or isinstance(v, Fp8KV)
    if f8:
        _req(paged and causal, "fp8 KV cache: paged causal attention only")
        _kv8(k, v, Hkv, D, q.device)
    if paged:
        _req(len(k.shape) == 4 and k.shape[2] == 64 and k.shape[1] == Hkv and k.shape[3] == D, "paged cache [nb,Hkv,64,D]")
        _req(v.shape == k.shape, "paged k/v caches differ in shape")
        _req(block_tables is not None and block_tables.dtype == torch.int32, "block_tables int32")
        _req(block_tables.stride(0) <= 2048, "prefill block tables wider than 2048 blocks (128k tokens)")
        kv_stride = k.shape[0]
    scale = 1.0 / math.sqrt(D) if scale is None else scale
    kd, vd, ks, vs = (k.data, v.data, k.scale, v.scale) if f8 else (k, v, None, None)
    check(_lib.lib().ragk_attn_prefill(
        q.data_ptr(), q.stride(0), kd.data_ptr(), vd.data_ptr(), ptr(ks), ptr(vs), kv_stride, ptr(block_tables),
        block_tables.stride(0) if block_tables is not None else 0, cu_q.data_ptr(), ptr(cu_kv), kv_lens.data_ptr(),
        tiles.data_ptr(), tiles.shape[0], out.data_ptr(), out.stride(0), Hq, Hkv, D, int(causal), int(paged),
        float(scale), stream_ptr()), "ragk_attn_prefill")
    return out


DECODE_TARGET_BLOCKS = 512
DECODE_MIN_TILES = 4


def _decode_single(batch, Hkv):
    return DECODE_NW8_MIN_PAIRS > 0 and batch * Hkv >= DECODE_NW8_MIN_PAIRS


def decode_partitions(max_kv_len, batch, Hkv, target_blocks=None, min_tiles=None):
    target_blocks = DECODE_TARGET_BLOCKS if target_blocks is None else target_blocks
    min_tiles = DECODE_MIN_TILES if min_tiles is None else min_tiles
    max_kt = max(1, (max_kv_len + 63) // 64)
    if _decode_single(batch, Hkv):
        return min_tiles, 1
    mp = max(1, min(-(-target_blocks // (batch * Hkv)), -(-max_kt // min_tiles)))
    return min_tiles, mp


DECODE_NW8_MIN_PAIRS = 256


DECODE_NT_MIN_BH = 64


DECODE_KL = os.environ.get("RAGK_DECODE_KL", "1") != "0"

DECODE_DIAG = 0

DEC_NT, DEC_SINGLE, DEC_KL, DEC_DEFER_MERGE, DEC_DIAG_SHIFT = 1, 2, 4, 8, 4

# ... 366 lines not shown
```

Before: 1728 generated tokens/s (aggregate over all GPUs).

## Trim prefill QKV work to needed rows and skip K/V output stores

During prefill, the fused QKV+RoPE GEMM can now skip writing K/V columns to the qkv output, writing them only to the KV cache. In the last layer it computes Q only for M-tiles listed as needed, through a tile list that covers all rows for K/V but only selected tiles for Q. The post-attention rmsnorm also runs only on the listed row tiles. The aim is to cut redundant GEMM tiles, global stores and norm work in prefill. It depends on the attention kernels reading K/V only from the cache, and a debug option that poisons the trimmed columns is added to check this.

```diff
diff --git a/csrc/kernels/gemm_w4.hip b/csrc/kernels/gemm_w4.hip
--- a/csrc/kernels/gemm_w4.hip
+++ b/csrc/kernels/gemm_w4.hip
@@ -196,17 +196,83 @@
   bf16_t* kc;
   bf16_t* vc;
   int Hq, Hkv, BS;
+  int kv_only;
 };
 
+template <bool FULL, bool CSTORE>
+__device__ __forceinline__ void w4_epilogue_rope_rows(const f32x4 (&acc)[8][8], int row0, int d0, bf16_t* Ccol, int ldc,
+                                                      const RopeKV& rk, int M, const int (&pos)[8],
+                                                      const int (&slot)[8], bool rot, bool isq, int kvh,
+                                                      bf16_t* cache) {
+#pragma unroll
+  for (int i2 = 0; i2 < 8; i2 += 2) {
+    u32x4 cv[2][2][2], sv[2][2][2];
+    if (rot) {
+#pragma unroll
+      for (int u = 0; u < 2; ++u)
+#pragma unroll
+        for (int p = 0; p < 2; ++p) {
+          const float* ct = rk.cos_t + (size_t)pos[i2 + u] * 64 + d0 + 32 * p;
+          const float* st = rk.sin_t + (size_t)pos[i2 + u] * 64 + d0 + 32 * p;
+          cv[u][p][0] = *reinterpret_cast<const u32x4*>(ct);
+          cv[u][p][1] = *reinterpret_cast<const u32x4*>(ct + 4);
+          sv[u][p][0] = *reinterpret_cast<const u32x4*>(st);
+          sv[u][p][1] = *reinterpret_cast<const u32x4*>(st + 4);
+        }
+    }
+#pragma unroll
+    for (int u = 0; u < 2; ++u) {
+      const int i = i2 + u;
+      const int gr = row0 + 16 * i;
+      float o[4][8];
+#pragma unroll
+      for (int p = 0; p < 4; ++p)
+#pragma unroll
+        for (int k = 0; k < 4; ++k) {
+          o[p][k] = bf2f(f2bf(acc[i][2 * p][k]));
+          o[p][4 + k] = bf2f(f2bf(acc[i][2 * p + 1][k]));
+        }
+      if (rot) {
+#pragma unroll
+        for (int p = 0; p < 2; ++p)
+#pragma unroll
+          for (int k = 0; k < 8; ++k) {
+            const float c = __uint_as_float(cv[u][p][k >> 2][k & 3]), sn = __uint_as_float(sv[u][p][k >> 2][k & 3]);
+            const float x1 = o[p][k], x2 = o[p + 2][k];
+            o[p][k] = bf2f(f2bf(bf2f(f2bf(x1 * c)) + bf2f(f2bf(-x2 * sn))));
+            o[p + 2][k] = bf2f(f2bf(bf2f(f2bf(x2 * c)) + bf2f(f2bf(x1 * sn))));
+          }
+      }
+      if (FULL || gr < M) {
+        if constexpr (CSTORE) {
+          bf16_t* crow = Ccol + (size_t)gr * ldc + d0;
+#pragma unroll
+          for (int p = 0; p < 4; ++p) *reinterpret_cast<u32x4*>(crow + 32 * p) = pack8(o[p]);
+        }
+        const int sl = slot[i];
+        if (!isq && sl >= 0) {
+          bf16_t* dst = cache + (((size_t)(sl / rk.BS) * rk.Hkv + kvh) * rk.BS + (sl % rk.BS)) * 128 + d0;
+#pragma unroll
+          for (int p = 0; p < 4; ++p) *reinterpret_cast<u32x4*>(dst + 32 * p) = pack8(o[p]);
+        }
+      }
+    }
+  }
+}
+
 template <bool FULL>
-__device__ __forceinline__ void w4_epilogue_rope(const f32x4 (&acc)[8][8], int wr, int wc, int fr, int fh, int m0,
-                                                 int n0, bf16_t* C, int ldc, const RopeKV& rk, int M) {
+__device__ __forceinline__ void w4_epilogue_rope(const f32x4 (&acc)[8][8], int wr, int wc, int m0, int n0, bf16_t* C,
+                                                 int ldc, const RopeKV& rk, int M) {
+  int ln;
+  asm volatile("v_mbcnt_lo_u32_b32 %0, -1, 0\n\tv_mbcnt_hi_u32_b32 %0, -1, %0" : "=v"(ln));
+  const int fr = ln & 15, fh = ln >> 4;
   const int row0 = m0 + wr * 128 + fr;
   const int hd = (n0 + wc * 128) >> 7;
   const int d0 = 8 * fh;
   const bool isq = hd < rk.Hq, isk = !isq && hd < rk.Hq + rk.Hkv, rot = hd < rk.Hq + rk.Hkv;
   const int kvh = isk ? hd - rk.Hq : hd - rk.Hq - rk.Hkv;
   bf16_t* cache = isk ? rk.kc : rk.vc;
+  bf16_t* Ccol = C + n0 + wc * 128;
   int pos[8], slot[8];
 #pragma unroll
   for (int i = 0; i < 8; ++i) {
@@ -214,56 +280,10 @@
     pos[i] = rk.pos[r];
     slot[i] = rk.slot[r];
   }
-#pragma unroll
-  for (int i2 = 0; i2 < 8; i2 += 2) {
-    u32x4 cv[2][2][2], sv[2][2][2];
-#pragma unroll
-    for (int u = 0; u < 2; ++u)
-#pragma unroll
-      for (int p = 0; p < 2; ++p) {
-        const float* ct = rk.cos_t + (size_t)pos[i2 + u] * 64 + d0 + 32 * p;
-        const float* st = rk.sin_t + (size_t)pos[i2 + u] * 64 + d0 + 32 * p;
-        cv[u][p][0] = *reinterpret_cast<const u32x4*>(ct);
-        cv[u][p][1] = *reinterpret_cast<const u32x4*>(ct + 4);
-        sv[u][p][0] = *reinterpret_cast<const u32x4*>(st);
-        sv[u][p][1] = *reinterpret_cast<const u32x4*>(st + 4);
-      }
-#pragma unroll
-    for (int u = 0; u < 2; ++u) {
-      const int i = i2 + u;
-      const int gr = row0 + 16 * i;
-      float o[4][8];
-#pragma unroll
-      for (int p = 0; p < 4; ++p)
-#pragma unroll
-        for (int k = 0; k < 4; ++k) {
-          o[p][k] = bf2f(f2bf(acc[i][2 * p][k]));
-          o[p][4 + k] = bf2f(f2bf(acc[i][2 * p + 1][k]));
-        }
-      if (rot) {
-#pragma unroll
-        for (int p = 0; p < 2; ++p)
-#pragma unroll
-          for (int k = 0; k < 8; ++k) {
-            const float c = __uint_as_float(cv[u][p][k >> 2][k & 3]), sn = __uint_as_float(sv[u][p][k >> 2][k & 3]);
-            const float x1 = o[p][k], x2 = o[p + 2][k];
-            o[p][k] = bf2f(f2bf(bf2f(f2bf(x1 * c)) + bf2f(f2bf(-x2 * sn))));
-            o[p + 2][k] = bf2f(f2bf(bf2f(f2bf(x2 * c)) + bf2f(f2bf(x1 * sn))));
-          }
-      }
-      if (FULL || gr < M) {
-        bf16_t* crow = C + (size_t)gr * ldc + n0 + wc * 128 + d0;
-#pragma unroll
-        for (int p = 0; p < 4; ++p) *reinterpret_cast<u32x4*>(crow + 32 * p) = pack8(o[p]);
-        const int sl = slot[i];
-        if (!isq && sl >= 0) {
-          bf16_t* dst = cache + (((size_t)(sl / rk.BS) * rk.Hkv + kvh) * rk.BS + (sl % rk.BS)) * 128 + d0;
-#pragma unroll
-          for (int p = 0; p < 4; ++p) *reinterpret_cast<u32x4*>(dst + 32 * p) = pack8(o[p]);
-        }
-      }
-    }
-  }
+  if (isq || !rk.kv_only)
+    w4_epilogue_rope_rows<FULL, true>(acc, row0, d0, Ccol, ldc, rk, M, pos, slot, rot, isq, kvh, cache);
+  else
+    w4_epilogue_rope_rows<FULL, false>(acc, row0, d0, Ccol, ldc, rk, M, pos, slot, rot, false, kvh, cache);
 }
 
 template <int EPI, bool OUT_F32, bool FULL>
@@ -442,6 +462,23 @@
   n0 = (in_group / gm) * WBN;
 }
 
+__device__ __forceinline__ void w4_origin_qlist(int tile, int nwt, int tiles_m, int n_q, int tn_q, int tn_kv, int& m0,
+                                                int& n0, const int* __restrict__ mt, int mt_max) {
+  int logical = xcd_remap(tile, nwt);
+  const int nkv = tiles_m * tn_kv;
+  const bool q = logical >= nkv;
+  if (q) logical -= nkv;
+  const int tm = q ? n_q : tiles_m, tn = q ? tn_q : tn_kv;
+  const int group = logical / (WGROUP_M * tn);
+  const int first_m = group * WGROUP_M;
+  const int gm = min(tm - first_m, WGROUP_M);
+  const int in_group = logical % (WGROUP_M * tn);
+  int mi = first_m + in_group % gm;
+  if (q) mi = (int)min((unsigned)mt[__builtin_amdgcn_readfirstlane(mi)], (unsigned)mt_max);
+  m0 = mi * WBM;
+  n0 = ((q ? 0 : tn_q) + in_group / gm) * WBN;
+}
+
 template <int EPI, bool OUT_F32, bool KSPLIT = false, bool MT = false>
 __global__ __launch_bounds__(W4_THREADS, 1) void gemm_w4_kernel(const bf16_t* __restrict__ A, int lda,
                                                                 const bf16_t* __restrict__ B, int ldb, void* C,
@@ -454,9 +491,11 @@
   const int wid = __builtin_amdgcn_readfirstlane(tid >> 6);
   const int wr = wid >> 1, wc = wid & 1;
   const int fr = lane & 15, fh = lane >> 4;
-  const int tiles_m = MT ? n_m_tiles : (M + WBM - 1) / WBM, tiles_n = (N + WBN - 1) / WBN;
+  constexpr bool QLIST = MT && EPI == EPI_ROPE_KV;
+  const int tiles_m = MT && !QLIST ? n_m_tiles : (M + WBM - 1) / WBM, tiles_n = (N + WBN - 1) / WBN;
   const int mt_max = (M + WBM - 1) / WBM - 1;
-  const int nwg = tiles_m * tiles_n;
+  const int tn_q = QLIST ? rk.Hq * 128 / WBN : 0;
+  const int nwg = QLIST ? tiles_m * (tiles_n - tn_q) + n_m_tiles * tn_q : tiles_m * tiles_n;
   const int nwt = KSPLIT ? nwg * nsplit : nwg;
   const int nk = K / WBK;
   const int Nout = EPI == EPI_SILU_MUL ? N / 2 : N;
@@ -467,13 +506,15 @@
   constexpr int VMH0 = H_VM + EV > 63 ? 63 : H_VM + EV;
   constexpr bool LATE_F0 = !(EPI == EPI_NONE || EPI == EPI_SILU_MUL || (EPI == EPI_RESID && !OUT_F32));
   static_assert(EPI != EPI_ROPE_KV || (!OUT_F32 && !KSPLIT), "rope epilogue: bf16 output, no split-K");
-  static_assert(!MT || EPI == EPI_NONE || ((EPI == EPI_RESID || EPI == EPI_SILU_MUL) && !OUT_F32 && !KSPLIT),
-                "M-tile list: none / residual / SiLU*up epilogues and the split-K slabs");
+  static_assert(!MT || EPI == EPI_NONE ||
+                    ((EPI == EPI_RESID || EPI == EPI_SILU_MUL || EPI == EPI_ROPE_KV) && !OUT_F32 && !KSPLIT),
+                "M-tile list: none / residual / SiLU*up / rope epilogues and the split-K slabs");
 
   int tile = blockIdx.x;
   int z = KSPLIT ? tile / nwg : 0;
   int m0, n0;
-  w4_origin<MT>(tile - z * nwg, nwg, tiles_m, tiles_n, m0, n0, m_tiles, mt_max);
+  if constexpr (QLIST) w4_origin_qlist(tile, nwg, tiles_m, n_m_tiles, tn_q, tiles_n - tn_q, m0, n0, m_tiles, mt_max);
+  else w4_origin<MT>(tile - z * nwg, nwg, tiles_m, tiles_n, m0, n0, m_tiles, mt_max);
   int off_a[8], off_b[8];
   w4_offsets<false>(lda, m0, M, wid, lane, off_a);
   w4_offsets<true>(ldb, n0, N, wid, lane, off_b);
@@ -518,7 +559,8 @@
     int nm0, nn0;
     const int ntile = has_next ? next : tile;
     const int nz = KSPLIT ? ntile / nwg : 0;
-    w4_origin<MT>(ntile - nz * nwg, nwg, tiles_m, tiles_n, nm0, nn0, m_tiles, mt_max);
+    if constexpr (QLIST) w4_origin_qlist(ntile, nwg, tiles_m, n_m_tiles, tn_q, tiles_n - tn_q, nm0, nn0, m_tiles, mt_max);
+    else w4_origin<MT>(ntile - nz * nwg, nwg, tiles_m, tiles_n, nm0, nn0, m_tiles, mt_max);
     {
       int ln;
       asm volatile("v_mbcnt_lo_u32_b32 %0, -1, 0\n\tv_mbcnt_hi_u32_b32 %0, -1, %0" : "=v"(ln));
@@ -541,9 +583,9 @@
     void* Cz = KSPLIT ? (void*)(reinterpret_cast<float*>(C) + (size_t)z * M * ldc) : C;
     if constexpr (EPI == EPI_ROPE_KV) {
       if (m0 + WBM <= M) {
-        w4_epilogue_rope<true>(acc, wr, wc, fr, fh, m0, n0, reinterpret_cast<bf16_t*>(Cz), ldc, rk, M);
+        w4_epilogue_rope<true>(acc, wr, wc, m0, n0, reinterpret_cast<bf16_t*>(Cz), ldc, rk, M);
       } else {
-        w4_epilogue_rope<false>(acc, wr, wc, fr, fh, m0, n0, reinterpret_cast<bf16_t*>(Cz), ldc, rk, M);
+        w4_epilogue_rope<false>(acc, wr, wc, m0, n0, reinterpret_cast<bf16_t*>(Cz), ldc, rk, M);
         __builtin_amdgcn_s_waitcnt(0x0F70);
       }
     } else if (m0 + WBM <= M && n0 + WBN <= N) {
@@ -671,14 +713,25 @@
 
 RAGK_API int ragk_gemm_w4_rope_kv(const void* A, int lda, const void* B, int ldb, void* C, int ldc, int M, int K,
                                   const int* pos, const int* slot, const float* cos_t, const float* sin_t, void* kc,
-                                  void* vc, int Hq, int Hkv, int BS, hipStream_t st) {
+                                  void* vc, int Hq, int Hkv, int BS, int kv_cache_only, const int* q_m_tiles,
+                                  int n_q_tiles, hipStream_t st) {
   if (M <= 0) return 0;
   const int N = (Hq + 2 * Hkv) * 128;
   if (K % WBK != 0 || K / WBK < W4_MIN_KT || Hq < 1 || Hkv < 1 || BS < 1 || N % WBN != 0) return (int)hipErrorInvalidValue;
   if (!pos || !slot || !cos_t || !sin_t || !kc || !vc || ldc % 8 != 0) return (int)hipErrorInvalidValue;
   if ((long long)M * lda * 2 >= (1LL << 31) || (long long)N * ldb * 2 >= (1LL << 31)) return (int)hipErrorInvalidValue;
-  const int nwg = ((M + WBM - 1) / WBM) * (N / WBN);
-  const RopeKV rk{pos, slot, cos_t, sin_t, (bf16_t*)kc, (bf16_t*)vc, Hq, Hkv, BS};
+  const int tiles_m = (M + WBM - 1) / WBM;
+  const RopeKV rk{pos, slot, cos_t, sin_t, (bf16_t*)kc, (bf16_t*)vc, Hq, Hkv, BS, kv_cache_only ? 1 : 0};
+  if (n_q_tiles >= 0) {
+    if ((Hq * 128) % WBN != 0 || n_q_tiles > tiles_m || (n_q_tiles > 0 && !q_m_tiles)) return (int)hipErrorInvalidValue;
+    const int tn_q = Hq * 128 / WBN;
+    const int nwt = tiles_m * (N / WBN - tn_q) + n_q_tiles * tn_q;
+    hipLaunchKernelGGL((gemm_w4_kernel<EPI_ROPE_KV, false, false, true>), dim3(w4_grid(nwt)), dim3(W4_THREADS), 0, st,
+                       (const bf16_t*)A, lda, (const bf16_t*)B, ldb, C, ldc, nullptr, nullptr, 0, M, N, K, 1, rk,
+                       q_m_tiles, n_q_tiles);
+    return (int)hipGetLastError();
+  }
+  const int nwg = tiles_m * (N / WBN);
   hipLaunchKernelGGL((gemm_w4_kernel<EPI_ROPE_KV, false>), dim3(w4_grid(nwg)), dim3(W4_THREADS), 0, st,
                      (const bf16_t*)A, lda, (const bf16_t*)B, ldb, C, ldc, nullptr, nullptr, 0, M, N, K, 1, rk, nullptr, 0);
   return (int)hipGetLastError();
diff --git a/csrc/kernels/norm.hip b/csrc/kernels/norm.hip
--- a/csrc/kernels/norm.hip
+++ b/csrc/kernels/norm.hip
@@ -8,11 +8,9 @@
 
 constexpr int NT = 256;
 
-__global__ __launch_bounds__(NT) void rmsnorm_kernel(const bf16_t* x, int ldx, bf16_t* resid, int ldr,
-                                                     const bf16_t* __restrict__ w, bf16_t* out, int ldo,
-                                                     int H, float eps) {
+__device__ __forceinline__ void rmsnorm_row(int row, const bf16_t* x, int ldx, bf16_t* resid, int ldr,
+                                            const bf16_t* __restrict__ w, bf16_t* out, int ldo, int H, float eps) {
   __shared__ float red[NT / 64];
-  const int row = blockIdx.x;
   const bf16_t* xr = x + (size_t)row * ldx;
   bf16_t* rr = resid ? resid + (size_t)row * ldr : nullptr;
   bf16_t* orow = out + (size_t)row * ldo;
@@ -49,6 +47,22 @@
       *reinterpret_cast<u32x4*>(orow + vi * 8) = pack8(o);
     }
   }
+}
+
+__global__ __launch_bounds__(NT) void rmsnorm_kernel(const bf16_t* x, int ldx, bf16_t* resid, int ldr,
+                                                     const bf16_t* __restrict__ w, bf16_t* out, int ldo,
+                                                     int H, float eps) {
+  rmsnorm_row(blockIdx.x, x, ldx, resid, ldr, w, out, ldo, H, eps);
+}
+
+__global__ __launch_bounds__(NT) void rmsnorm_tiles_kernel(const bf16_t* x, int ldx, bf16_t* resid, int ldr,
+                                                           const bf16_t* __restrict__ w, bf16_t* out, int ldo,
+                                                           int H, float eps, const int* __restrict__ m_tiles,
+                                                           int rows) {
+  const int t = m_tiles[blockIdx.x >> 8];
+  const int row = t * 256 + (blockIdx.x & 255);
+  if (t < 0 || row >= rows) return;
+  rmsnorm_row(row, x, ldx, resid, ldr, w, out, ldo, H, eps);
 }
 
 __global__ __launch_bounds__(NT) void layernorm_kernel(const bf16_t* x, int ldx, const bf16_t* resid, int ldr,
@@ -503,6 +517,15 @@
   return (int)hipGetLastError();
 }
 
+RAGK_API int ragk_rmsnorm_tiles(const void* x, int ldx, void* resid, int ldr, const void* w, void* out, int ldo,
+                                int rows, int H, float eps, const int* m_tiles, int n_m_tiles, hipStream_t st) {
+  if (rows <= 0 || n_m_tiles <= 0) return 0;
+  if (H % 8 || H > 8 * NT * 4 || !m_tiles || n_m_tiles > (rows + 255) / 256) return (int)hipErrorInvalidValue;
+  hipLaunchKernelGGL(rmsnorm_tiles_kernel, dim3(n_m_tiles * 256), dim3(NT), 0, st, (const bf16_t*)x, ldx,
+                     (bf16_t*)resid, ldr, (const bf16_t*)w, (bf16_t*)out, ldo, H, eps, m_tiles, rows);
+  return (int)hipGetLastError();
+}
+
 RAGK_API int ragk_layernorm(const void* x, int ldx, const void* resid, int ldr, const void* g, const void* b,
                             void* out, int ldo, int rows, int H, float eps, hipStream_t st) {
   if (rows <= 0) return 0;
diff --git a/rag_llm_k8s_amd/models/llama.py b/rag_llm_k8s_amd/models/llama.py
--- a/rag_llm_k8s_amd/models/llama.py
+++ b/rag_llm_k8s_amd/models/llama.py
@@ -263,7 +263,8 @@
         Hq, Hkv, D = self.Hq, self.Hkv, self.D
         kc, vc = self.kv_cache[li]
         xn = be.rmsnorm(h, L["ln_in"], c.rms_norm_eps)
-        qkv = be.gemm_rope_kv(xn, L["wqkv"], inp.positions, self.cos, self.sin, inp.slots, kc, vc, Hq, Hkv, D)
+        qkv = be.gemm_rope_kv(xn, L["wqkv"], inp.positions, self.cos, self.sin, inp.slots, kc, vc, Hq, Hkv, D,
+                              kv_cache_only=self._qkv_trim(inp))
         if inp.meta.kind == "decode":
             be.attn_decode(qkv, kc, vc, inp.meta, attn, Hq, Hkv, D)
         else:
@@ -292,6 +293,14 @@
     @staticmethod
     def prefill_last_rows_enabled():
         return os.environ.get("RAGK_PREFILL_LAST_ROWS", "1") != "0"
+
+    @staticmethod
+    def prefill_qkv_trim_enabled():
+        return os.environ.get("RAGK_PREFILL_QKV_TRIM", "1") != "0"
+
+    def _qkv_trim(self, inp: StepInput):
+        return (self.comm is None and inp.meta is not None and inp.meta.kind != "decode"
+                and self.prefill_qkv_trim_enabled())
 
     def _last_rows(self, inp: StepInput, M):
         if (self.comm is not None or inp.meta is None or inp.meta.kind == "decode" or inp.logits_idx is None
@@ -392,15 +401,25 @@
         Hq, Hkv, D = self.Hq, self.Hkv, self.D
         kc, vc = self.kv_cache[li]
         xn = be.rmsnorm(h, L["ln_in"], c.rms_norm_eps)
-        qkv = be.gemm_rope_kv(xn, L["wqkv"], inp.positions, self.cos, self.sin, inp.slots, kc, vc, Hq, Hkv, D)
+        qkv = be.gemm_rope_kv(xn, L["wqkv"], inp.positions, self.cos, self.sin, inp.slots, kc, vc, Hq, Hkv, D,
+                              **self._last_qkv_args(inp, mode))
         if mode == "skip":
             return
         mt = inp.m_tiles
         be.attn_prefill(qkv, kc, vc, inp.meta, attn, Hq, Hkv, D, tiles=inp.meta.tiles_last)
         be.gemm(attn, L["wo"], resid=h, epi="resid", out=h, m_tiles=mt)
-        xn = be.rmsnorm(h, L["ln_post"], c.rms_norm_eps)
+        xn = be.rmsnorm(h, L["ln_post"], c.rms_norm_eps, m_tiles=mt if self._qkv_trim(inp) else None)
         a = be.gemm(xn, L["wgu"], epi="silu_mul", m_tiles=mt)
         be.gemm(a, L["wdown"], resid=h, epi="resid", out=h, m_tiles=mt)
+
+    def _last_qkv_args(self, inp: StepInput, mode):
+        if not self._qkv_trim(inp):
+            return {}
+        if mode == "tiles":
+            return {"kv_cache_only": True, "q_m_tiles": inp.m_tiles}
+        if mode == "skip":
+            return {"kv_cache_only": True, "q_m_tiles": inp.logits_idx.new_empty(0, dtype=torch.int32)}
+        return {"kv_cache_only": True}
 
     def hidden_states_splitk(self, inp: StepInput, h, attn, ns_o, ns_d):
         be, w, c = self.be, self.w, self.cfg
@@ -413,7 +432,8 @@
             cut = last if li + 1 == len(layers) else None
             rows = {"m_tiles": inp.m_tiles} if cut == "tiles" else {}
             blocks = {"tiles": inp.meta.tiles_last} if cut == "tiles" else {}
-            qkv = be.gemm_rope_kv(xn, L["wqkv"], inp.positions, self.cos, self.sin, inp.slots, kc, vc, Hq, Hkv, D)
+            qkv = be.gemm_rope_kv(xn, L["wqkv"], inp.positions, self.cos, self.sin, inp.slots, kc, vc, Hq, Hkv, D,
+                                  **self._last_qkv_args(inp, cut))
             if cut == "skip":
                 return h.new_empty((0, h.shape[1]))
             be.attn_prefill(qkv, kc, vc, inp.meta, attn, Hq, Hkv, D, **blocks)
@@ -422,7 +442,7 @@
                                              c.rms_norm_eps)
             else:
                 be.gemm(attn, L["wo"], resid=h, epi="resid", out=h, **rows)
-                xn = be.rmsnorm(h, L["ln_post"], c.rms_norm_eps)
+                xn = be.rmsnorm(h, L["ln_post"], c.rms_norm_eps, **(rows if self._qkv_trim(inp) else {}))
             a = be.gemm(xn, L["wgu"], epi="silu_mul", **rows)
             nxt = layers[li + 1]["ln_in"] if li + 1 < len(layers) else w.norm
             if ns_d > 1:
diff --git a/rag_llm_k8s_amd/ops/_lib.py b/rag_llm_k8s_amd/ops/_lib.py
--- a/rag_llm_k8s_amd/ops/_lib.py
+++ b/rag_llm_k8s_amd/ops/_lib.py
@@ -19,7 +19,7 @@
     "ragk_gemm_stream_set_diag": [I],
     "ragk_gemm_stream_set_pair_rows": [I],
     "ragk_gemm_w4": [P, I, P, I, P, I, P, P, I, I, I, I, I, I, P, I, S],
-    "ragk_gemm_w4_rope_kv": [P, I, P, I, P, I, I, I, P, P, P, P, P, P, I, I, I, S],
+    "ragk_gemm_w4_rope_kv": [P, I, P, I, P, I, I, I, P, P, P, P, P, P, I, I, I, I, P, I, S],
     "ragk_gemm_w4_splitk": [P, I, P, I, P, I, I, I, I, P, I, S],
     "ragk_gemm_part": [P, I, P, I, P, I, I, I, I, S],
     "ragk_gemm_part_norm": [P, I, P, F, P, I, P, I, I, I, I, S],
@@ -45,6 +45,7 @@
     "ragk_gemm_dec": [P, I, P, I, P, I, P, P, I, I, I, I, I, I, I, P, P, S],
     "ragk_gemm_dec_splits": [I, I, I],
     "ragk_rmsnorm": [P, I, P, I, P, P, I, I, I, F, S],
+    "ragk_rmsnorm_tiles": [P, I, P, I, P, P, I, I, I, F, P, I, S],
     "ragk_layernorm": [P, I, P, I, P, P, P, I, I, I, F, S],
     "ragk_embed": [P, P, P, I, I, I, S],
     "ragk_embed_carry": [P, P, P, P, P, I, I, I, S],
diff --git a/rag_llm_k8s_amd/ops/backend.py b/rag_llm_k8s_amd/ops/backend.py
--- a/rag_llm_k8s_amd/ops/backend.py
+++ b/rag_llm_k8s_amd/ops/backend.py
@@ -49,7 +49,7 @@
             return out
         return y
 
-    def rmsnorm(self, x, w, eps, out=None):
+    def rmsnorm(self, x, w, eps, out=None, m_tiles=None):
         y = R.rmsnorm(x, w, eps)
         if out is not None:
             out.copy_(y)
@@ -107,9 +107,14 @@
                 else:
                     cache[s // KV_BLOCK, :, s % KV_BLOCK] = rows
 
-    def gemm_rope_kv(self, x, w, positions, cos_t, sin_t, slots, kc, vc, Hq, Hkv, D):
+    poison_trimmed_kv = False
+
+    def gemm_rope_kv(self, x, w, positions, cos_t, sin_t, slots, kc, vc, Hq, Hkv, D, kv_cache_only=False,
+                     q_m_tiles=None):
         qkv = self.gemm(x, w)
         self.rope_kv(qkv, positions, cos_t, sin_t, slots, kc, vc, Hq, Hkv, D)
+        if kv_cache_only and self.poison_trimmed_kv:
+            qkv[:, Hq * D:] = float("nan")
         return qkv
 
 
@@ -291,8 +296,8 @@
         N = w.shape[0] // 2 if epi == "silu_mul" else w.shape[0]
         return self.n.gemm_m_tiles_ok(M, N, w.shape[1], epi, ldb=w.stride(0))
 
-    def rmsnorm(self, x, w, eps, out=None):
-        return self.n.rmsnorm(x, w, eps, out=out)
+    def rmsnorm(self, x, w, eps, out=None, m_tiles=None):
+        return self.n.rmsnorm(x, w, eps, out=out, m_tiles=m_tiles)
 
     def layernorm(self, x, g, b, eps, out=None, resid=None):
         return self.n.layernorm(x, g, b, eps, out=out, resid=resid)
@@ -312,9 +317,15 @@
     def rope_kv(self, qkv, positions, cos_t, sin_t, slots, kc, vc, Hq, Hkv, D, apply_rope=True):
         self.n.rope_kv(qkv, positions, cos_t, sin_t, slots, kc, vc, Hq, Hkv, D, apply_rope=apply_rope)
 
-    def gemm_rope_kv(self, x, w, positions, cos_t, sin_t, slots, kc, vc, Hq, Hkv, D):
-        if self.n.gemm_rope_kv_ok(x, w, positions, cos_t, sin_t, slots, kc, vc, Hq, Hkv, D):
-            return self.n.gemm_rope_kv(x, w, positions, cos_t, sin_t, slots, kc, vc, Hq, Hkv, D)
+    def gemm_rope_kv(self, x, w, positions, cos_t, sin_t, slots, kc, vc, Hq, Hkv, D, kv_cache_only=False,
+                     q_m_tiles=None):
+        ok = self.n.gemm_rope_kv_ok
+        if ok(x, w, positions, cos_t, sin_t, slots, kc, vc, Hq, Hkv, D, q_m_tiles=q_m_tiles is not None):
+            return self.n.gemm_rope_kv(x, w, positions, cos_t, sin_t, slots, kc, vc, Hq, Hkv, D,
+                                       kv_cache_only=kv_cache_only, q_m_tiles=q_m_tiles)
+        if ok(x, w, positions, cos_t, sin_t, slots, kc, vc, Hq, Hkv, D):
+            return self.n.gemm_rope_kv(x, w, positions, cos_t, sin_t, slots, kc, vc, Hq, Hkv, D,
+                                       kv_cache_only=kv_cache_only)
         qkv = self.gemm(x, w)
         self.rope_kv(qkv, positions, cos_t, sin_t, slots, kc, vc, Hq, Hkv, D)
         return qkv
diff --git a/rag_llm_k8s_amd/ops/native.py b/rag_llm_k8s_amd/ops/native.py
--- a/rag_llm_k8s_amd/ops/native.py
+++ b/rag_llm_k8s_amd/ops/native.py
@@ -96,7 +96,9 @@
 PREFILL_ROPE_FUSED = os.environ.get("RAGK_PREFILL_ROPE", "1") != "0"
 
 
-def gemm_rope_kv_ok(x, w, positions, cos_t, sin_t, slots, k_cache, v_cache, Hq, Hkv, D):
+def gemm_rope_kv_ok(x, w, positions, cos_t, sin_t, slots, k_cache, v_cache, Hq, Hkv, D, q_m_tiles=False):
+    if q_m_tiles and (Hq * D) % 256:
+        return False
     if not PREFILL_ROPE_FUSED or D != 128 or slots is None or k_cache is None or v_cache is None:
         return False
     if isinstance(k_cache, Fp8KV) or isinstance(v_cache, Fp8KV):
@@ -123,17 +125,24 @@
             and slots.is_contiguous() and positions.numel() == M and slots.numel() == M)
 
 
-def gemm_rope_kv(x, w, positions, cos_t, sin_t, slots, k_cache, v_cache, Hq, Hkv, D, out=None):
-    _req(gemm_rope_kv_ok(x, w, positions, cos_t, sin_t, slots, k_cache, v_cache, Hq, Hkv, D), "gemm_rope_kv operands")
+def gemm_rope_kv(x, w, positions, cos_t, sin_t, slots, k_cache, v_cache, Hq, Hkv, D, out=None, kv_cache_only=False,
+                 q_m_tiles=None):
+    _req(gemm_rope_kv_ok(x, w, positions, cos_t, sin_t, slots, k_cache, v_cache, Hq, Hkv, D,
+                         q_m_tiles=q_m_tiles is not None), "gemm_rope_kv operands")
     M, K = x.shape
     N = w.shape[0]
     if out is None:
         out = torch.empty((M, N), dtype=torch.bfloat16, device=x.device)
     _req(out.shape == (M, N) and out.stride(1) == 1 and out.stride(0) % 8 == 0, "gemm_rope_kv out")
+    qt_ptr, qt_n = None, -1
+    if q_m_tiles is not None:
+        qt_ptr, qt_n = _m_tiles_arg(q_m_tiles, M, x.device)
+        qt_ptr = qt_ptr if qt_n else None
     check(_lib.lib().ragk_gemm_w4_rope_kv(x.data_ptr(), x.stride(0), w.data_ptr(), w.stride(0), out.data_ptr(),
                                           out.stride(0), M, K, positions.data_ptr(), slots.data_ptr(),
                                           cos_t.data_ptr(), sin_t.data_ptr(), k_cache.data_ptr(), v_cache.data_ptr(),
-                                          Hq, Hkv, k_cache.shape[2], stream_ptr()), "ragk_gemm_w4_rope_kv")
+                                          Hq, Hkv, k_cache.shape[2], int(bool(kv_cache_only)), qt_ptr, qt_n,
+                                          stream_ptr()), "ragk_gemm_w4_rope_kv")
     return out
 
 
@@ -765,7 +774,7 @@
     return out
 
 
-def rmsnorm(x, w, eps, out=None, resid=None):
+def rmsnorm(x, w, eps, out=None, resid=None, m_tiles=None):
     _bf16_2d(x, "x")
     T, H = x.shape
     _req(w.numel() == H and w.dtype == torch.bfloat16, "weight")
@@ -779,9 +788,16 @@
     _al16(resid, "resid")
     _al16(w, "weight")
     _al16(out, "out")
-    check(_lib.lib().ragk_rmsnorm(x.data_ptr(), x.stride(0), ptr(resid), resid.stride(0) if resid is not None else 0,
-                                  w.data_ptr(), out.data_ptr(), out.stride(0), T, H, float(eps), stream_ptr()),
-          "ragk_rmsnorm")
+    ldr = resid.stride(0) if resid is not None else 0
+    if m_tiles is not None:
+        mt_ptr, mt_n = _m_tiles_arg(m_tiles, T, x.device)
+        if mt_n:
+            check(_lib.lib().ragk_rmsnorm_tiles(x.data_ptr(), x.stride(0), ptr(resid), ldr, w.data_ptr(), out.data_ptr(),
+                                                out.stride(0), T, H, float(eps), mt_ptr, mt_n, stream_ptr()),
+                  "ragk_rmsnorm_tiles")
+        return out
+    check(_lib.lib().ragk_rmsnorm(x.data_ptr(), x.stride(0), ptr(resid), ldr, w.data_ptr(), out.data_ptr(),
+                                  out.stride(0), T, H, float(eps), stream_ptr()), "ragk_rmsnorm")
     return out
 
 
```

Result: no change. 1735 generated tokens/s (aggregate over all GPUs) (median of 6 runs) (+0.4%).
